# ArroyoSystems/arroyo

Measured on NVIDIA H100. Metric: rows/sec sliding-window SUM (1M keys), higher is better.
Workload: dtype int64

## Files before the change

arroyo_b200/csrc/abi.cu:

```cuda
#include <algorithm>
#include <chrono>
#include <memory>
#include <new>

#include "op.h"
#include "planner.h"

using namespace ab;

struct ArroyoB200Op {
  OpBase* impl;
  double host_process_ms = 0, host_watermark_ms = 0;
};

namespace {
struct WallTimer {
  double& acc;
  std::chrono::steady_clock::time_point t0 = std::chrono::steady_clock::now();
  explicit WallTimer(double& a) : acc(a) {}
  ~WallTimer() { acc += std::chrono::duration<double, std::milli>(std::chrono::steady_clock::now() - t0).count(); }
};
}

namespace {

template <class F>
int32_t guarded(ArroyoB200Op* op, F&& f) {
  if (!op || !op->impl) return ARROYO_B200_INVALID_ARGUMENT;
  try {
    f(op->impl);
    return ARROYO_B200_OK;
  } catch (const Error& e) {
    op->impl->last_error = e.what();
    return e.status;
  } catch (const std::bad_alloc&) {
    op->impl->last_error = "out of host memory";
    return ARROYO_B200_RUNTIME;
  } catch (const std::exception& e) {
    op->impl->last_error = e.what();
    return ARROYO_B200_RUNTIME;
  } catch (...) {
    op->impl->last_error = "unknown C++ exception";
    return ARROYO_B200_RUNTIME;
  }
}

template <class F>
int32_t emit_batches(ArroyoB200Op* op, ArroyoB200Batches* out, F&& f, double ArroyoB200Op::*timer = nullptr,
                     bool null_out_ok = false) {
  if (out) memset(out, 0, sizeof *out);
  if (!op) return ARROYO_B200_INVALID_ARGUMENT;
  double untimed = 0;
  WallTimer wt(timer ? op->*timer : untimed);
  return guarded(op, [&](OpBase* o) {
    AB_REQUIRE(out != nullptr || null_out_ok, ARROYO_B200_INVALID_ARGUMENT, "null out");
    std::unique_ptr<BatchesPriv, void (*)(BatchesPriv*)> priv(new BatchesPriv(), discard);
    f(o, priv.get());
    if (out) batches_finish(priv.release(), out);
  });
}

void begin_emission(OpBase* o, int64_t watermark_ns) {
  o->pending_out = new BatchesPriv();
  try {
    o->begin_watermark(watermark_ns);
  } catch (...) {
    o->poll_watermark(true);
    discard(o->pending_out);
    o->pending_out = nullptr;
    throw;
  }
}

void set_err(char* err, uint64_t len, const char* msg) {
  if (err && len) {
    snprintf(err, (size_t)len, "%s", msg);
  }
}

int64_t hand_out(OpBase* o, std::vector<ArroyoB200DeviceBatch>& v, ArroyoB200DeviceBatch* out, int64_t max_out) {
  const size_t n = (size_t)std::min<int64_t>((int64_t)v.size(), std::max<int64_t>(max_out, 0));
  for (size_t i = 0; i < n; ++i) out[i] = v[i];
  o->pending_dev.assign(v.begin() + n, v.end());
  return (int64_t)n;
}

}

extern "C" {

int32_t arroyo_b200_abi_version(void) { return 1; }

int32_t arroyo_b200_device_count(void) {
  int n = 0;
  if (cudaGetDeviceCount(&n) != cudaSuccess) {
    cudaGetLastError();
    return 0;
  }
  return n;
}

void* arroyo_b200_host_alloc(uint64_t bytes) {
  void* p = nullptr;
  if (cudaHostAlloc(&p, (size_t)bytes, cudaHostAllocDefault) != cudaSuccess) {
    cudaGetLastError();
    return nullptr;
  }
  return p;
}

void arroyo_b200_host_free(void* p) {
  if (p) cudaFreeHost(p);
}

int32_t arroyo_b200_op_create(const ArroyoB200OpConfig* config, ArroyoB200Op** out, char* err, uint64_t err_len) {
  if (!config || !out) {
    set_err(err, err_len, "null config or out pointer");
    return ARROYO_B200_INVALID_ARGUMENT;
  }
  *out = nullptr;
  try {
    OpBase* impl = nullptr;
    switch (config->kind) {
      case ARROYO_B200_TUMBLING_AGGREGATE:
      case ARROYO_B200_SLIDING_AGGREGATE:
        impl = make_window_agg_op(*config);
        break;
      case ARROYO_B200_SESSION_AGGREGATE:
        impl = make_session_op(*config);
        break;
      case ARROYO_B200_INSTANT_JOIN:
        impl = make_instant_join_op(*config);
        break;
      case ARROYO_B200_UPDATING_AGGREGATE:
        impl = make_updating_agg_op(*config);
        break;
      case ARROYO_B200_TTL_JOIN:
        impl = make_ttl_join_op(*config);
        break;
      case ARROYO_B200_INSTANT_AGGREGATE:
        impl = make_instant_agg_op(*config);
        break;
      case ARROYO_B200_WINDOW_FUNCTION:
        impl = make_window_fn_op(*config);
        break;
      default:
        set_err(err, err_len, "unknown operator kind");
        return ARROYO_B200_INVALID_ARGUMENT;
    }
    auto* h = new ArroyoB200Op();
    h->impl = impl;
    *out = h;
    return ARROYO_B200_OK;
  } catch (const Error& e) {
    set_err(err, err_len, e.what());
    return e.status;
  } catch (const std::exception& e) {
    set_err(err, err_len, e.what());
    return ARROYO_B200_RUNTIME;
  } catch (...) {
    set_err(err, err_len, "unknown C++ exception");
    return ARROYO_B200_RUNTIME;
  }
}

void arroyo_b200_op_destroy(ArroyoB200Op* op) {
  if (!op) return;
  try {
    if (op->impl && op->impl->pending_out) {
      op->impl->poll_watermark(true);
      discard(op->impl->pending_out);
      op->impl->pending_out = nullptr;
    }
    delete op->impl;
  } catch (...) {
  }
  delete op;
}

const char* arroyo_b200_op_last_error(const ArroyoB200Op* op) {
  if (!op || !op->impl) return "invalid handle";
  return op->impl->last_error.c_str();
}

const char* arroyo_b200_op_name(const ArroyoB200Op* op) {
  if (!op || !op->impl) return "";
  return op->impl->name.c_str();
}

int32_t arroyo_b200_op_on_start(ArroyoB200Op* op, struct ArrowArray* state, struct ArrowSchema* schemas, int64_t n,
                                int64_t watermark_ns, int64_t table_min_time_ns) {
  return guarded(op, [&](OpBase* o) { o->on_start(state, schemas, n, watermark_ns, table_min_time_ns); });
}

int32_t arroyo_b200_op_process_batch(ArroyoB200Op* op, uint32_t input_index, uint32_t in_partitions,
                                     struct ArrowArray* batch, const struct ArrowSchema* schema) {
  if (!op) return ARROYO_B200_INVALID_ARGUMENT;
  WallTimer wt(op->host_process_ms);
  return guarded(op, [&](OpBase* o) { o->process_batch(input_index, in_partitions, batch, schema); });
}

int32_t arroyo_b200_op_process_batch_emit(ArroyoB200Op* op, uint32_t input_index, uint32_t in_partitions,
                                          struct ArrowArray* batch, const struct ArrowSchema* schema, ArroyoB200Batches* out) {
  return emit_batches(
      op, out, [&](OpBase* o, BatchesPriv* b) { o->process_batch_emit(input_index, in_partitions, batch, schema, b); },
      &ArroyoB200Op::host_process_ms);
}

int32_t arroyo_b200_op_process_device_batch(ArroyoB200Op* op, uint32_t input_index, uint32_t in_partitions,
                                            const uint64_t* cols, int32_t n_cols, int64_t n_rows) {
  return guarded(op, [&](OpBase* o) {
    AB_REQUIRE(cols != nullptr && n_cols > 0, ARROYO_B200_INVALID_ARGUMENT, "null column list");
    o->process_device_batch(input_index, in_partitions, cols, n_cols, n_rows);
  });
}

int32_t arroyo_b200_op_process_device_batches(ArroyoB200Op* op, uint32_t input_index, uint32_t in_partitions,
                                              const uint64_t* cols, int32_t n_cols, const int64_t* n_rows,
                                              int64_t n_batches) {
  if (!op) return ARROYO_B200_INVALID_ARGUMENT;
  WallTimer wt(op->host_process_ms);
  return guarded(op, [&](OpBase* o) {
    AB_REQUIRE(cols != nullptr && n_rows != nullptr && n_cols > 0 && n_batches >= 0, ARROYO_B200_INVALID_ARGUMENT,
               "null batch list");
    for (int64_t b = 0; b < n_batches; ++b)
      o->process_device_batch(input_index, in_partitions, cols + b * n_cols, n_cols, n_rows[b]);
  });
}

int32_t arroyo_b200_op_handle_watermark(ArroyoB200Op* op, int64_t watermark_ns, ArroyoB200Batches* out) {
  return emit_batches(
      op, out, [&](OpBase* o, BatchesPriv* b) { o->handle_watermark(watermark_ns, b, nullptr); },
      &ArroyoB200Op::host_watermark_ms);
}

int32_t arroyo_b200_op_handle_tick(ArroyoB200Op* op, ArroyoB200Batches* out) {
  return emit_batches(op, out, [&](OpBase* o, BatchesPriv* b) { o->handle_tick(b); });
}

int32_t arroyo_b200_op_handle_watermark_begin(ArroyoB200Op* op, int64_t watermark_ns) {
  if (!op) return ARROYO_B200_INVALID_ARGUMENT;
  WallTimer wt(op->host_watermark_ms);
  return guarded(op, [&](OpBase* o) {
    AB_REQUIRE(o->pending_out == nullptr, ARROYO_B200_INVALID_ARGUMENT,
               "the previous emission has not been collected (handle_watermark_poll)");
    begin_emission(o, watermark_ns);
  });
}

int32_t arroyo_b200_op_handle_watermark_poll(ArroyoB200Op* op, int32_t block, ArroyoB200Batches* out, int32_t* ready) {
  if (out) memset(out, 0, sizeof *out);
  if (ready) *ready = 0;
  if (!op) return ARROYO_B200_INVALID_ARGUMENT;
  WallTimer wt(op->host_watermark_ms);
  return guarded(op, [&](OpBase* o) {
    AB_REQUIRE(out != nullptr && ready != nullptr, ARROYO_B200_INVALID_ARGUMENT, "null out");
    if (!o->pending_out) {
      *ready = 1;
      return;
    }
    if (!o->poll_watermark(block != 0)) return;
    batches_finish(o->pending_out, out);
    o->pending_out = nullptr;
    *ready = 1;
  });
}

int32_t arroyo_b200_op_run_batches(ArroyoB200Op* op, struct ArrowArray* batches, const struct ArrowSchema* schema,
                                    int64_t n_batches, const int64_t* watermarks, int32_t async_emit,
                                    ArroyoB200Batches* out, int64_t* n_consumed) {
  if (out) memset(out, 0, sizeof *out);
  if (n_consumed) *n_consumed = 0;
  if (!op) return ARROYO_B200_INVALID_ARGUMENT;
  auto* acc = new BatchesPriv();
  int32_t st = guarded(op, [&](OpBase* o) {
    AB_REQUIRE(out != nullptr && n_consumed != nullptr && (n_batches == 0 || (batches != nullptr && schema != nullptr)),
               ARROYO_B200_INVALID_ARGUMENT, "null argument");
    auto collect = [&](bool block) {
      if (!o->pending_out || !o->poll_watermark(block)) return;
      for (auto& a : o->pending_out->arrays) acc->arrays.push_back(a);
      for (auto& s : o->pending_out->schemas) acc->schemas.push_back(s);
      delete o->pending_out;
      o->pending_out = nullptr;
    };
    for (int64_t i = 0; i < n_batches; ++i) {
      {
        WallTimer wt(op->host_process_ms);
        o->process_batch(0, 1, &batches[i], schema);
      }
      ++*n_consumed;
      const int64_t wm = watermarks ? watermarks[i] : INT64_MIN;
      WallTimer wt(op->host_watermark_ms);
      if (wm == INT64_MIN) {
        if (async_emit && (i & 7) == 0) collect(false);
        continue;
      }
      if (async_emit) {
        collect(true);
        begin_emission(o, wm);
      } else {
        o->handle_watermark(wm, acc, nullptr);
      }
    }
    if (async_emit) collect(false);
  });
  if (out) batches_finish(acc, out);
  else discard(acc);
  return st;
}

int32_t arroyo_b200_op_handle_watermark_device(ArroyoB200Op* op, int64_t watermark_ns, ArroyoB200DeviceBatch* out,
                                               int64_t max_out, int64_t* n_out) {
  if (n_out) *n_out = 0;
  if (!op) return ARROYO_B200_INVALID_ARGUMENT;
  WallTimer wt(op->host_watermark_ms);
  return guarded(op, [&](OpBase* o) {
    AB_REQUIRE(n_out != nullptr && (out != nullptr || max_out <= 0), ARROYO_B200_INVALID_ARGUMENT, "null out");
    AB_REQUIRE(o->pending_dev.empty(), ARROYO_B200_INVALID_ARGUMENT,
               "windows of the previous emission are still queued (handle_watermark_device_poll)");
    std::vector<ArroyoB200DeviceBatch> v;
    o->handle_watermark(watermark_ns, nullptr, &v);
    *n_out = hand_out(o, v, out, max_out);
  });
}

int32_t arroyo_b200_op_handle_watermark_device_begin(ArroyoB200Op* op, int64_t watermark_ns) {
  if (!op) return ARROYO_B200_INVALID_ARGUMENT;
  WallTimer wt(op->host_watermark_ms);
  return guarded(op, [&](OpBase* o) {
    AB_REQUIRE(o->pending_dev.empty(), ARROYO_B200_INVALID_ARGUMENT,
               "windows of the previous emission are still queued (handle_watermark_device_poll)");
    o->begin_watermark_device(watermark_ns);
  });
}

int32_t arroyo_b200_op_handle_watermark_device_poll(ArroyoB200Op* op, ArroyoB200DeviceBatch* out, int64_t max_out,
                                                    int64_t* n_out) {
  if (n_out) *n_out = 0;
  if (!op) return ARROYO_B200_INVALID_ARGUMENT;
  WallTimer wt(op->host_watermark_ms);
  return guarded(op, [&](OpBase* o) {
    AB_REQUIRE(n_out != nullptr && (out != nullptr || max_out <= 0), ARROYO_B200_INVALID_ARGUMENT, "null out");
    std::vector<ArroyoB200DeviceBatch> v;
    o->poll_watermark_device(&v);
    *n_out = hand_out(o, v, out, max_out);
  });
}

int32_t arroyo_b200_op_handle_checkpoint(ArroyoB200Op* op, int64_t watermark_ns, ArroyoB200Batches* state_out) {
  return emit_batches(op, state_out, [&](OpBase* o, BatchesPriv* b) { o->handle_checkpoint(watermark_ns, b); });
}

int32_t arroyo_b200_op_checkpoint_state(ArroyoB200Op* op, ArroyoB200Batches* state_out) {
  return emit_batches(op, state_out, [&](OpBase* o, BatchesPriv* b) { o->checkpoint_state(b); });
}

int32_t arroyo_b200_op_restore_side(ArroyoB200Op* op, uint32_t side, struct ArrowArray* batches,
                                    struct ArrowSchema* schemas, int64_t n) {
  return guarded(op, [&](OpBase* o) { o->restore_side(side, batches, schemas, n); });
}

int32_t arroyo_b200_op_set_clock(ArroyoB200Op* op, int64_t now_ns) {
  return guarded(op, [&](OpBase* o) { o->set_clock(now_ns); });
}

int32_t arroyo_b200_op_on_close(ArroyoB200Op* op, int32_t end_of_data, ArroyoB200Batches* out) {
  return emit_batches(op, out, [&](OpBase* o, BatchesPriv* b) { o->on_close(end_of_data, b); }, nullptr, true);
}

int32_t arroyo_b200_op_flush(ArroyoB200Op* op) {
  return guarded(op, [&](OpBase* o) { o->flush(); });
}

int32_t arroyo_b200_op_submit(ArroyoB200Op* op) {
  return guarded(op, [&](OpBase* o) { o->submit(); });
}

void arroyo_b200_release_batches(ArroyoB200Batches* batches) { batches_release(batches); }

int32_t arroyo_b200_op_stats(ArroyoB200Op* op, ArroyoB200Stats* out) {
  return guarded(op, [&](OpBase* o) {
    AB_REQUIRE(out != nullptr, ARROYO_B200_INVALID_ARGUMENT, "null out");
    o->stats(out);
    out->host_process_ms = op->host_process_ms;
    out->host_watermark_ms = op->host_watermark_ms;
  });
}

uint64_t arroyo_b200_hash_key(int64_t key) { return mix64((uint64_t)key); }

uint32_t arroyo_b200_server_for_hash(uint64_t h, uint32_t n) {
  if (n == 0) return 0;
  uint64_t range = UINT64_MAX / (uint64_t)n;
  return (uint32_t)((h / range) % (uint64_t)n);
}

int64_t arroyo_b200_bin_start(int64_t ts_ns, int64_t width_ns) {
  if (width_ns < 2 || ts_ns < 0) return width_ns <= 0 ? ts_ns : ts_ns - ts_ns % width_ns;
  FastDivU64 d = FastDivU64::make((uint64_t)width_ns);
  return (int64_t)(d.div_host((uint64_t)ts_ns) * (uint64_t)width_ns);
}

static int64_t write_steps(const std::vector<PlanStep>& steps, int64_t* out, int64_t cap) {
  if ((int64_t)steps.size() * 4 > cap) return -1;
  for (size_t i = 0; i < steps.size(); ++i) {
    out[4 * i + 0] = steps[i].kind;
    out[4 * i + 1] = steps[i].a;
    out[4 * i + 2] = steps[i].b;
    out[4 * i + 3] = steps[i].c;
  }
  return (int64_t)steps.size();
}

int64_t arroyo_b200_plan_sliding(int64_t width_ns, int64_t slide_ns, const int64_t* events, int64_t n_events,
                                 int64_t* out, int64_t out_cap) {
  if (slide_ns <= 0 || width_ns <= 0 || width_ns % slide_ns) return -2;
  SlidingPlanner pl(width_ns, slide_ns);
  std::vector<PlanStep> steps;
  bool has_wm = false;
  int64_t wm = 0;
  for (int64_t i = 0; i < n_events; ++i) {
    int64_t kind = events[2 * i], v = events[2 * i + 1];
    if (kind == 0) {
      if (has_wm && v < bin_start(wm, slide_ns)) continue;
      pl.touch(v);
    } else if (kind == 1) {
      has_wm = true;
      wm = v;
      pl.watermark(v, steps);
    } else if (kind == 2) {
      pl.checkpoint(has_wm, wm, steps);
    }
  }
  return write_steps(steps, out, out_cap);
}

int64_t arroyo_b200_plan_tumbling(int64_t width_ns, const int64_t* events, int64_t n_events, int64_t* out,
                                  int64_t out_cap) {
  if (width_ns <= 0) return -2;
  TumblingPlanner pl(width_ns);
  std::vector<PlanStep> steps;
  bool has_wm = false;
  int64_t wm = 0;
  for (int64_t i = 0; i < n_events; ++i) {
    int64_t kind = events[2 * i], v = events[2 * i + 1];
    if (kind == 0) {
      if (has_wm && v < bin_start(wm, width_ns)) continue;
      pl.touch(v);
    } else if (kind == 1) {
      has_wm = true;
      wm = v;
      pl.watermark(v, steps);
    } else if (kind == 2) {
      pl.checkpoint(steps);
    }
  }
  return write_steps(steps, out, out_cap);
}

}
```

arroyo_b200/csrc/op.h:

```cpp
#pragma once

#include <string>
#include <vector>

#include "arrow_io.h"
#include "common.cuh"

namespace ab {

class OpBase {
 public:
  ArroyoB200OpConfig cfg{};
  std::string last_error;
  std::string name;

  virtual ~OpBase() {
    if (own_stream_) cudaStreamDestroy(stream_);
  }
  virtual void on_start(ArrowArray* state, ArrowSchema* schemas, int64_t n, int64_t watermark, int64_t table_min) = 0;
  virtual void process_batch(uint32_t index, uint32_t in_partitions, ArrowArray* batch, const ArrowSchema* schema) = 0;
  virtual void process_batch_emit(uint32_t index, uint32_t in_partitions, ArrowArray* batch, const ArrowSchema* schema,
                                  BatchesPriv* ) {
    process_batch(index, in_partitions, batch, schema);
  }
  virtual void process_device_batch(uint32_t index, uint32_t in_partitions, const uint64_t* cols, int32_t n_cols,
                                    int64_t n_rows) = 0;
  virtual void handle_watermark(int64_t watermark, BatchesPriv* out_host, std::vector<ArroyoB200DeviceBatch>* out_dev) = 0;
  virtual void handle_checkpoint(int64_t watermark, BatchesPriv* out) = 0;
  virtual void on_close(int end_of_data, BatchesPriv* out) = 0;
  virtual void handle_tick(BatchesPriv* ) {}
  virtual void checkpoint_state(BatchesPriv* ) {}
  virtual void restore_side(uint32_t , ArrowArray* , ArrowSchema* , int64_t ) {
    throw Error(ARROYO_B200_UNSUPPORTED, name + ": restore_side is only for the join with expiration");
  }
  virtual void set_clock(int64_t ) {
    throw Error(ARROYO_B200_UNSUPPORTED, name + ": set_clock is only for the updating aggregate");
  }
  virtual void flush() = 0;
  virtual void submit() {}
  BatchesPriv* pending_out = nullptr;
  virtual void begin_watermark(int64_t watermark) { handle_watermark(watermark, pending_out, nullptr); }
  virtual bool poll_watermark(bool ) { return true; }
  std::vector<ArroyoB200DeviceBatch> pending_dev;
  virtual void begin_watermark_device(int64_t watermark) {
    pending_dev.clear();
    handle_watermark(watermark, nullptr, &pending_dev);
  }
  virtual void poll_watermark_device(std::vector<ArroyoB200DeviceBatch>* out) {
    out->swap(pending_dev);
    pending_dev.clear();
  }
  virtual void stats(ArroyoB200Stats* out) = 0;

 protected:
  int device_ = 0;
  cudaStream_t stream_ = nullptr;
  bool own_stream_ = false;
  int num_sms_ = 132;

  void open_device(const ArroyoB200OpConfig& c) {
    int count = 0;
    if (cudaGetDeviceCount(&count) != cudaSuccess || count <= 0)
      throw Error(ARROYO_B200_FATAL, "no CUDA device available: libarroyo_b200 has no CPU fallback");
    AB_REQUIRE(c.device >= 0 && c.device < count, ARROYO_B200_INVALID_ARGUMENT, "bad device ordinal");
    device_ = c.device;
    set_device();
    cudaDeviceProp prop{};
    AB_CUDA(cudaGetDeviceProperties(&prop, device_));
    num_sms_ = prop.multiProcessorCount;
    if (c.stream) {
      stream_ = (cudaStream_t)c.stream;
    } else {
      AB_CUDA(cudaStreamCreateWithFlags(&stream_, cudaStreamNonBlocking));
      own_stream_ = true;
    }
  }
  void set_device() const { AB_CUDA(cudaSetDevice(device_)); }
  void drain_stream() const {
    cudaSetDevice(device_);
    cudaStreamSynchronize(stream_);
  }
};

OpBase* make_window_agg_op(const ArroyoB200OpConfig& cfg);
OpBase* make_instant_join_op(const ArroyoB200OpConfig& cfg);
OpBase* make_session_op(const ArroyoB200OpConfig& cfg);
OpBase* make_updating_agg_op(const ArroyoB200OpConfig& cfg);
OpBase* make_ttl_join_op(const ArroyoB200OpConfig& cfg);
OpBase* make_instant_agg_op(const ArroyoB200OpConfig& cfg);
OpBase* make_window_fn_op(const ArroyoB200OpConfig& cfg);

}
```

arroyo_b200/csrc/window_agg.cu:

```cuda
#include <algorithm>
#include <climits>
#include <deque>
#include <map>
#include <memory>
#include <set>

#include "agg_plan.h"
#include "bdict.cuh"
#include "op.h"
#include "planner.h"

namespace ab {
namespace {

constexpr int MAX_SEGS = 512;
constexpr int MAX_RING = 4096;
constexpr int RING_INLINE = 64;
constexpr int MAX_MERGE = 4096;
constexpr long long FREE_BIN = LLONG_MIN;

constexpr int THREADS = 256;
constexpr int PAIRS = 2;
constexpr int TILE = THREADS * PAIRS * 2;

struct Counters {
  unsigned long long late_rows;
  unsigned long long deferred;
  unsigned long long lost;
  unsigned long long neg_ts;
  unsigned long long max_q;
  unsigned long long big_vals;
  unsigned int n_keys;
  unsigned int dict_full;
  unsigned long long part_overflow;
};

struct Segment {
  const long long* key;
  const long long* ts;
  const long long* val[MAX_VALS];
  long long n;
  long long tile_start;
  int vec_ok;
  int pad;
};

struct IngestParams {
  const Segment* segs;
  int n_segs;
  int keyed;
  long long n_tiles;
  BDict dict;
  FastDivU64 slide_div;
  long long slide;
  long long late_bin;
  unsigned long long late_q;
  unsigned int guard_vals;
  int combine;
  int rows_slot;
  int pad2;
  uint32_t ring_mask;
  int n_acc;
  const long long* pane_bins;
  unsigned long long* const* pane_ptrs;
  unsigned long long id_cap;
  int ring_inline;
  int pad1;
  long long ring_bins[RING_INLINE];
  unsigned long long* ring_ptrs[RING_INLINE];
  int acc_kind[MAX_ACC];
  int acc_val[MAX_ACC];
  Counters* counters;
  unsigned long long* slot_rows;
  long long* d_key;
  long long* d_ts;
  long long* d_val[MAX_VALS];
  unsigned long long defer_cap;
};

struct InitParams {
  unsigned long long* pane;
  unsigned long long id_cap;
  unsigned long long n;
  int n_acc;
  int acc_kind[MAX_ACC];
};

__global__ void pane_init_kernel(const __grid_constant__ InitParams p) {
  uint64_t i = (uint64_t)blockIdx.x * blockDim.x + threadIdx.x;
  uint64_t stride = (uint64_t)gridDim.x * blockDim.x;
  for (; i < p.n; i += stride) {
    for (int a = 0; a < p.n_acc; ++a) p.pane[a * p.id_cap + i] = acc_identity(p.acc_kind[a]);
  }
}

__device__ __forceinline__ const long long* ldg_ptr(const long long* const* pp) {
  return reinterpret_cast<const long long*>(__ldg(reinterpret_cast<const unsigned long long*>(pp)));
}

__device__ __forceinline__ void red_add_u64(unsigned long long* a, unsigned long long v) {
  asm volatile("red.global.add.u64 [%0], %1;" ::"l"(__cvta_generic_to_global(a)), "l"(v) : "memory");
}
__device__ __forceinline__ void red_add_f64(unsigned long long* a, double v) {
  asm volatile("red.global.add.f64 [%0], %1;" ::"l"(__cvta_generic_to_global(a)), "d"(v) : "memory");
}
__device__ __forceinline__ void red_min_s64(unsigned long long* a, long long v) {
  asm volatile("red.global.min.s64 [%0], %1;" ::"l"(__cvta_generic_to_global(a)), "l"(v) : "memory");
}
__device__ __forceinline__ void red_max_s64(unsigned long long* a, long long v) {
  asm volatile("red.global.max.s64 [%0], %1;" ::"l"(__cvta_generic_to_global(a)), "l"(v) : "memory");
}

__device__ __forceinline__ long long ring_bin(const IngestParams& p, uint32_t slot) {
  return p.ring_inline ? p.ring_bins[slot] : __ldg(p.pane_bins + slot);
}
__device__ __forceinline__ unsigned long long* ring_ptr(const IngestParams& p, uint32_t slot) {
  return p.ring_inline ? p.ring_ptrs[slot]
                       : reinterpret_cast<unsigned long long*>(__ldg(reinterpret_cast<const unsigned long long*>(p.pane_ptrs + slot)));
}

struct Vals {
  long long v0, v1, v2, v3;
};
template <int NV>
__device__ __forceinline__ Vals pack_vals(const long long (&v)[NV > 0 ? NV : 1]) {
  Vals o{0, 0, 0, 0};
  if (NV > 0) o.v0 = v[0];
  if (NV > 1) o.v1 = v[NV > 1 ? 1 : 0];
  if (NV > 2) o.v2 = v[NV > 2 ? 2 : 0];
  if (NV > 3) o.v3 = v[NV > 3 ? 3 : 0];
  return o;
}

__device__ __noinline__ void defer_row(const IngestParams& p, long long key, long long ts, long long v0, long long v1,
                                       long long v2, long long v3) {
  unsigned long long idx = atomicAdd(&p.counters->deferred, 1ull);
  if (idx < p.defer_cap) {
    p.d_key[idx] = key;
    p.d_ts[idx] = ts;
    if (p.d_val[0]) p.d_val[0][idx] = v0;
    if (p.d_val[1]) p.d_val[1][idx] = v1;
    if (p.d_val[2]) p.d_val[2][idx] = v2;
    if (p.d_val[3]) p.d_val[3][idx] = v3;
  } else {
    atomicAdd(&p.counters->lost, 1ull);
  }
}

constexpr int GENERIC_SIG = -1;
constexpr int sig_of(int k1, int k2 = 0, int k3 = 0) { return k1 | (k2 << 3) | (k3 << 6); }

__device__ __forceinline__ void red_kind(int kind, unsigned long long* dst, long long v) {
  switch (kind) {
    case ACC_SUM_I64: red_add_u64(dst, (unsigned long long)v); break;
    case ACC_SUM_F64: red_add_f64(dst, (double)v); break;
    case ACC_MIN_I64: red_min_s64(dst, v); break;
    case ACC_MAX_I64: red_max_s64(dst, v); break;
    default: break;
  }
}

__device__ __forceinline__ unsigned long long rows_of(const IngestParams& p, const Vals& v) {
  const int x = p.rows_slot;
  if (x < 0) return 1ull;
  return (unsigned long long)(x == 0 ? v.v0 : x == 1 ? v.v1 : x == 2 ? v.v2 : v.v3);
}

template <int NV, int SIG>
__device__ __forceinline__ void accumulate(const IngestParams& p, const Vals& v, unsigned long long* pane, uint32_t id) {
  red_add_u64(pane + id, rows_of(p, v));
  if (SIG == GENERIC_SIG) {
#pragma unroll
    for (int a = 1; a < MAX_ACC; ++a) {
      if (a < p.n_acc) {
        const int x = p.acc_val[a];
        const long long val = x == 0 ? v.v0 : x == 1 ? v.v1 : x == 2 ? v.v2 : v.v3;
        red_kind(p.acc_kind[a], pane + (unsigned long long)a * p.id_cap + id, val);
      }
    }
  } else {
    constexpr int k1 = SIG & 7, k2 = (SIG >> 3) & 7, k3 = (SIG >> 6) & 7;
    if (k1) red_kind(k1, pane + p.id_cap + id, v.v0);
    if (k2) red_kind(k2, pane + 2 * p.id_cap + id, v.v0);
    if (k3) red_kind(k3, pane + 3 * p.id_cap + id, v.v0);
  }
}

__device__ __forceinline__ bool big_one(long long v) { return (unsigned long long)(v + (1ll << 31)) >= (1ull << 32); }
__device__ __forceinline__ bool big_value(unsigned int mask, const Vals& v) {
  return ((mask & 1u) && big_one(v.v0)) || ((mask & 2u) && big_one(v.v1)) || ((mask & 4u) && big_one(v.v2)) ||
         ((mask & 8u) && big_one(v.v3));
}

template <int NV, int SIG>
__device__ __noinline__ void slow_row(const IngestParams& p, long long key, long long ts, uint64_t q, long long v0,
                                      long long v1, long long v2, long long v3) {
  const uint32_t slot = (uint32_t)q & p.ring_mask;
  uint32_t id = 0;
  bool ok = ring_bin(p, slot) == (long long)(q * (uint64_t)p.slide);
  if (ok && p.keyed) {
    const uint64_t h = bd_hash(key);
    const ulonglong2* hp = reinterpret_cast<const ulonglong2*>(bd_home(p.dict, key, h));
    const ulonglong2 raw = __ldcg(hp), raw1 = __ldcg(hp + 1);
    id = bd_resolve(p.dict, key, h, raw.x, (uint32_t)raw.y, raw1.x, (uint32_t)raw1.y);
    ok = id < ID_OVERFLOW;
    if (!ok) atomicAdd(&p.counters->dict_full, 1u);
  }
  const Vals v{v0, v1, v2, v3};
  if (ok && NV > 0 && p.guard_vals && big_value(p.guard_vals, v)) {
    atomicAdd(&p.counters->big_vals, 1ull);
    ok = false;
  }
  if (!ok) {
    defer_row(p, key, ts, v0, v1, v2, v3);
    return;
  }
  unsigned long long* pane = ring_ptr(p, slot);
  atomicAdd(p.slot_rows + slot, 1ull);
  accumulate<NV, SIG>(p, v, pane, id);
}

struct PaneCache {
  uint64_t q = ~0ull;
  unsigned long long* ptr = nullptr;
  uint32_t cnt = 0;
};

__device__ __forceinline__ void flush_counts(const IngestParams& p, PaneCache& pc, int lane) {
  const unsigned int peers = __match_any_sync(0xffffffffu, pc.q);
  const unsigned int total = __reduce_add_sync(peers, pc.cnt);
  if (total && (__ffs(peers) - 1) == lane)
    atomicAdd(p.slot_rows + ((uint32_t)pc.q & p.ring_mask), (unsigned long long)total);
  pc.cnt = 0;
}

template <int NV, int SIG>
__device__ __forceinline__ uint32_t hot_resolve(const IngestParams& p, const PaneCache& pc, uint64_t& maxq, bool keyed,
                                                long long key, long long ts, uint64_t q, const Vals& v, uint64_t h,
                                                unsigned long long k0, uint32_t id0, unsigned long long k1, uint32_t id1) {
  uint32_t id = ID_OVERFLOW;
  if (q == pc.q && pc.ptr != nullptr) id = keyed ? bd_resolve(p.dict, key, h, k0, id0, k1, id1) : 0u;
  if (NV > 0 && p.guard_vals && big_value(p.guard_vals, v)) {
    atomicAdd(&p.counters->big_vals, 1ull);
    defer_row(p, key, ts, v.v0, v.v1, v.v2, v.v3);
    return ID_OVERFLOW;
  }
  if (id >= ID_OVERFLOW) {
    maxq = max(maxq, q);
    slow_row<NV, SIG>(p, key, ts, q, v.v0, v.v1, v.v2, v.v3);
  }
  return id;
}

__device__ __forceinline__ long long shfl_ll(unsigned mask, long long v, int src) {
  return (long long)__shfl_sync(mask, (unsigned long long)v, src);
}

__device__ __forceinline__ long long group_reduce(int kind, unsigned peers, long long v) {
  long long r = v;
  bool first = true;
  for (unsigned m = peers; m; m &= m - 1) {
    const long long x = shfl_ll(peers, v, __ffs(m) - 1);
    if (first) {
      r = x;
      first = false;
      continue;
    }
    switch (kind) {
      case ACC_SUM_I64: r = (long long)((unsigned long long)r + (unsigned long long)x); break;
      case ACC_SUM_F64: r = __double_as_longlong(__longlong_as_double(r) + __longlong_as_double(x)); break;
      case ACC_MIN_I64: r = min(r, x); break;
      case ACC_MAX_I64: r = max(r, x); break;
      default: break;
    }
  }
  return r;
}

__device__ __forceinline__ void red_kind_combined(int kind, unsigned long long* dst, long long v) {
  if (kind == ACC_SUM_F64) red_add_f64(dst, __longlong_as_double(v));
  else red_kind(kind, dst, v);
}

template <int NV, int SIG>
__device__ __forceinline__ void combine_accumulate(const IngestParams& p, const PaneCache& pc, bool fast, uint32_t id,
                                                   const Vals& v, int lane) {
  const unsigned long long gkey = fast ? ((unsigned long long)id | (pc.q << 32)) : (0xFFFFFFFF00000000ull | (unsigned)lane);
  const unsigned long long nb = __shfl_xor_sync(0xffffffffu, gkey, 1);
  if (!__any_sync(0xffffffffu, fast && nb == gkey)) {
    if (fast) accumulate<NV, SIG>(p, v, pc.ptr, id);
    return;
  }
  const unsigned peers = __match_any_sync(0xffffffffu, gkey);
  const bool leader = (__ffs(peers) - 1) == lane;
  unsigned long long* pane = pc.ptr;
  if (p.rows_slot < 0) {
    if (fast && leader) red_add_u64(pane + id, (unsigned long long)__popc(peers));
  } else {
    const long long r = group_reduce(ACC_SUM_I64, peers, (long long)rows_of(p, v));
    if (fast && leader) red_add_u64(pane + id, (unsigned long long)r);
  }
  if (SIG == GENERIC_SIG) {
#pragma unroll
    for (int a = 1; a < MAX_ACC; ++a) {
      if (a < p.n_acc) {
        const int x = p.acc_val[a];
        long long val = x == 0 ? v.v0 : x == 1 ? v.v1 : x == 2 ? v.v2 : v.v3;
        const int kind = p.acc_kind[a];
        if (kind == ACC_SUM_F64) val = __double_as_longlong((double)val);
        const long long r = group_reduce(kind, peers, val);
        if (fast && leader) red_kind_combined(kind, pane + (unsigned long long)a * p.id_cap + id, r);
      }
    }
  } else {
    constexpr int k1 = SIG & 7, k2 = (SIG >> 3) & 7, k3 = (SIG >> 6) & 7;
    if (k1) {
      const long long r = group_reduce(k1, peers, k1 == ACC_SUM_F64 ? __double_as_longlong((double)v.v0) : v.v0);
      if (fast && leader) red_kind_combined(k1, pane + p.id_cap + id, r);
    }
    if (k2) {
      const long long r = group_reduce(k2, peers, k2 == ACC_SUM_F64 ? __double_as_longlong((double)v.v0) : v.v0);
      if (fast && leader) red_kind_combined(k2, pane + 2 * p.id_cap + id, r);
    }
    if (k3) {
      const long long r = group_reduce(k3, peers, k3 == ACC_SUM_F64 ? __double_as_longlong((double)v.v0) : v.v0);
      if (fast && leader) red_kind_combined(k3, pane + 3 * p.id_cap + id, r);
    }
  }
}

#ifndef AB_INGEST_PREFETCH
#define AB_INGEST_PREFETCH 1
#endif
#ifndef AB_INGEST_MIN_BLOCKS
#define AB_INGEST_MIN_BLOCKS 4
#endif
template <int NV, int SIG>
__global__ void __launch_bounds__(THREADS, AB_INGEST_MIN_BLOCKS) ingest_kernel(const __grid_constant__ IngestParams p) {
  __shared__ unsigned long long s_late, s_maxq;
  __shared__ unsigned int s_done;
  const int tid = threadIdx.x;
  const int lane = tid & 31;
  if (tid == 0) {
    s_late = 0;
    s_maxq = 0;
    s_done = 0;
  }
  __syncthreads();

  PaneCache pc;
  uint32_t late = 0;
  uint64_t maxq = 0;
  const FastDivU64 sd = p.slide_div;
  const bool keyed = p.keyed != 0;

  for (long long tile = blockIdx.x; tile < p.n_tiles; tile += gridDim.x) {
    int lo = 0, hi = p.n_segs - 1;
    while (lo < hi) {
      int mid = (lo + hi + 1) >> 1;
      if (__ldg(&p.segs[mid].tile_start) <= tile) lo = mid; else hi = mid - 1;
    }
    const Segment* sg = p.segs + lo;
    const long long base = (tile - __ldg(&sg->tile_start)) * TILE;
    const long long nrem = __ldg(&sg->n) - base;
    const int cnt = nrem < TILE ? (int)nrem : TILE;

    long long nkey = 0, nts = 0;
    long long nv[NV > 0 ? NV : 1] = {0};
    if (tid < cnt) {
      if (keyed) nkey = __ldcs(ldg_ptr(&sg->key) + base + tid);
      nts = __ldcs(ldg_ptr(&sg->ts) + base + tid);
#pragma unroll
      for (int x = 0; x < NV; ++x) nv[x] = __ldcs(ldg_ptr(&sg->val[x]) + base + tid);
    }
#pragma unroll 1
    for (int i = tid; i < TILE; i += THREADS) {
      const bool valid = i < cnt;
      const long long key = nkey, ts = nts;
      long long v[NV > 0 ? NV : 1];
#pragma unroll
      for (int x = 0; x < (NV > 0 ? NV : 1); ++x) v[x] = nv[x];
      ulonglong2 raw = {0, 0}, raw1 = {0, 0};
      const uint64_t h = keyed ? bd_hash(key) : 0ull;
      if (valid && keyed) {
        const ulonglong2* hp = reinterpret_cast<const ulonglong2*>(bd_home(p.dict, key, h));
        raw = __ldcg(hp);
        raw1 = __ldcg(hp + 1);
      }
#if AB_INGEST_PREFETCH
      if (i + THREADS < cnt) {
        if (keyed) nkey = __ldcs(ldg_ptr(&sg->key) + base + i + THREADS);
        nts = __ldcs(ldg_ptr(&sg->ts) + base + i + THREADS);
#pragma unroll
        for (int x = 0; x < NV; ++x) nv[x] = __ldcs(ldg_ptr(&sg->val[x]) + base + i + THREADS);
      }
#endif
      const uint64_t q = sd.div((uint64_t)ts);
      if (valid && ts < 0) atomicAdd(&p.counters->neg_ts, 1ull);
      const bool live = valid && ts >= 0 && q >= p.late_q;
      late += (valid && !live) ? 1u : 0u;
      if (__any_sync(0xffffffffu, live && q != pc.q)) {
        flush_counts(p, pc, lane);
        if (live) {
          const uint32_t slot = (uint32_t)q & p.ring_mask;
          const bool resident = ring_bin(p, slot) == (long long)(q * (uint64_t)p.slide);
          pc.q = q;
          pc.ptr = resident ? ring_ptr(p, slot) : nullptr;
          maxq = max(maxq, q);
        }
      }
      const Vals pv = pack_vals<NV>(v);
      uint32_t id = ID_OVERFLOW;
      if (live) id = hot_resolve<NV, SIG>(p, pc, maxq, keyed, key, ts, q, pv, h, raw.x, (uint32_t)raw.y, raw1.x, (uint32_t)raw1.y);
      const bool fast = id < ID_OVERFLOW;
      if (fast) ++pc.cnt;
      if (p.combine) combine_accumulate<NV, SIG>(p, pc, fast, id, pv, lane);
      else if (fast) accumulate<NV, SIG>(p, pv, pc.ptr, id);
#if !AB_INGEST_PREFETCH
      if (i + THREADS < cnt) {
        if (keyed) nkey = __ldcs(ldg_ptr(&sg->key) + base + i + THREADS);
        nts = __ldcs(ldg_ptr(&sg->ts) + base + i + THREADS);
#pragma unroll
        for (int x = 0; x < NV; ++x) nv[x] = __ldcs(ldg_ptr(&sg->val[x]) + base + i + THREADS);
      }
#endif
    }
  }

  __syncwarp();
  flush_counts(p, pc, lane);
  unsigned long long wl = late;
#pragma unroll
  for (int o = 16; o > 0; o >>= 1) {
    wl += __shfl_xor_sync(0xffffffffu, wl, o);
    maxq = max(maxq, __shfl_xor_sync(0xffffffffu, maxq, o));
  }
  if (lane == 0) {
    if (wl) atomicAdd(&s_late, wl);
    if (maxq) atomicMax(&s_maxq, (unsigned long long)maxq);
    __threadfence_block();
    if (atomicAdd(&s_done, 1u) == THREADS / 32 - 1) {
      __threadfence_block();
      const unsigned long long bl = *(volatile unsigned long long*)&s_late;
      const unsigned long long mq = *(volatile unsigned long long*)&s_maxq;
      if (bl) atomicAdd(&p.counters->late_rows, bl);
      if (mq) atomicMax(&p.counters->max_q, mq);
    }
  }
}

#include "ingest_two_pass.cuh"

struct PartialParams {
  const uint32_t* ids;
  const unsigned long long* state[MAX_ACC];
  long long n;
  int n_acc;
  int acc_kind[MAX_ACC];
  unsigned long long* pane;
  unsigned long long id_cap;
};

__global__ void ingest_partial_kernel(const __grid_constant__ PartialParams p) {
  long long i = (long long)blockIdx.x * blockDim.x + threadIdx.x;
  long long stride = (long long)gridDim.x * blockDim.x;
  for (; i < p.n; i += stride) {
    const uint32_t id = p.ids[i];
    for (int a = 0; a < p.n_acc; ++a)
      acc_atomic_merge(p.acc_kind[a], p.pane + (unsigned long long)a * p.id_cap + id, p.state[a] ? p.state[a][i] : 1ull);
  }
}

constexpr int EMIT_INLINE = 16;
struct EmitParams {
  const unsigned long long* const* panes;
  const unsigned long long* inline_panes[EMIT_INLINE];
  int panes_inline;
  int n_panes;
  int n_acc;
  unsigned long long id_cap;
  uint32_t n_ids;
  int keyed;
  int acc_kind[MAX_ACC];
  unsigned long long* out_raw[MAX_ACC];
  unsigned long long* out_avg[MAX_ACC];
  const long long* id_keys;
  long long* out_key;
  long long* out_wstart;
  long long* out_wend;
  long long* out_ts;
  long long wstart, wend, ts;
  unsigned int* out_count;
  unsigned int out_base;
  unsigned long long* running;
  int n_add;
  int partial;
  unsigned long long* out_state[MAX_ACC];
};

constexpr int EMIT_THREADS = 256;

__device__ __forceinline__ unsigned long long unmerge_acc(int kind, unsigned long long a, unsigned long long v) {
  if (kind == ACC_SUM_F64)
    return (unsigned long long)__double_as_longlong(__longlong_as_double((long long)a) - __longlong_as_double((long long)v));
  return a - v;
}

template <int NACC>
__device__ __forceinline__ void emit_row(const EmitParams& p, unsigned int o, const unsigned long long (&acc)[NACC],
                                         long long key) {
  const unsigned long long rows = acc[0];
  if (p.keyed) p.out_key[o] = key;
  if (p.partial) {
#pragma unroll
    for (int a = 0; a < NACC; ++a)
      p.out_state[a][o] = acc[a];
    p.out_ts[o] = p.ts;
    return;
  }
#pragma unroll
  for (int a = 0; a < NACC; ++a) {
    if (p.out_raw[a]) p.out_raw[a][o] = acc[a];
    if (p.out_avg[a]) {
      const double num = p.acc_kind[a] == ACC_SUM_F64 ? __longlong_as_double((long long)acc[a]) : (double)(long long)acc[a];
      p.out_avg[a][o] = (unsigned long long)__double_as_longlong(num / (double)rows);
    }
  }
  if (p.out_wstart) {
    p.out_wstart[o] = p.wstart;
    p.out_wend[o] = p.wend;
  }
  p.out_ts[o] = p.ts;
}

template <bool RUNNING, int NACC>
__global__ void __launch_bounds__(EMIT_THREADS) emit_kernel(const __grid_constant__ EmitParams p) {
  __shared__ unsigned int s_warp[EMIT_THREADS / 32];
  __shared__ unsigned int s_base;
  const int tid = threadIdx.x;
  const int lane = tid & 31, w = tid >> 5;
  const uint32_t n_pairs = (p.n_ids + 1) / 2;
  const uint32_t n_iter = (n_pairs + EMIT_THREADS - 1) / EMIT_THREADS;
  for (uint32_t it = blockIdx.x; it < n_iter; it += gridDim.x) {
    const uint32_t pair = it * EMIT_THREADS + tid;
    const uint32_t id = pair * 2;
    unsigned long long acc0[NACC], acc1[NACC];
#pragma unroll
    for (int a = 0; a < NACC; ++a) {
      acc0[a] = 0;
      acc1[a] = 0;
    }
    const bool in0 = id < p.n_ids, in1 = id + 1 < p.n_ids;
    if (in0) {
      if (RUNNING) {
#pragma unroll
        for (int a = 0; a < NACC; ++a)
          {
            const ulonglong2 v = *reinterpret_cast<const ulonglong2*>(p.running + (unsigned long long)a * p.id_cap + id);
            acc0[a] = v.x;
            acc1[a] = v.y;
          }
        for (int k = 0; k < p.n_panes; ++k) {
          const unsigned long long* pane = p.panes_inline ? p.inline_panes[k] : p.panes[k];
          const bool add = k < p.n_add;
#pragma unroll
          for (int a = 0; a < NACC; ++a)
            {
              const ulonglong2 v = __ldcs(reinterpret_cast<const ulonglong2*>(pane + (unsigned long long)a * p.id_cap + id));
              const int kind = p.acc_kind[a];
              acc0[a] = add ? acc_merge(kind, acc0[a], v.x) : unmerge_acc(kind, acc0[a], v.x);
              acc1[a] = add ? acc_merge(kind, acc1[a], v.y) : unmerge_acc(kind, acc1[a], v.y);
            }
        }
        const bool z0 = acc0[0] == 0, z1 = acc1[0] == 0;
#pragma unroll
        for (int a = 0; a < NACC; ++a)
          {
            if (z0) acc0[a] = 0;
            if (z1) acc1[a] = 0;
            *reinterpret_cast<ulonglong2*>(p.running + (unsigned long long)a * p.id_cap + id) = make_ulonglong2(acc0[a], acc1[a]);
          }
      } else {
#pragma unroll
        for (int a = 0; a < NACC; ++a)
          {
            const unsigned long long ident = acc_identity(p.acc_kind[a]);
            acc0[a] = ident;
            acc1[a] = ident;
          }
        for (int k = 0; k < p.n_panes; ++k) {
          const unsigned long long* pane = p.panes_inline ? p.inline_panes[k] : p.panes[k];
#pragma unroll
          for (int a = 0; a < NACC; ++a)
            {
              const ulonglong2 v = __ldcs(reinterpret_cast<const ulonglong2*>(pane + (unsigned long long)a * p.id_cap + id));
              const int kind = p.acc_kind[a];
              acc0[a] = acc_merge(kind, acc0[a], v.x);
              acc1[a] = acc_merge(kind, acc1[a], v.y);
            }
        }
      }
    }
    const bool v0 = in0 && acc0[0] != 0, v1 = in1 && acc1[0] != 0;
    const unsigned int b0 = __ballot_sync(0xffffffffu, v0), b1 = __ballot_sync(0xffffffffu, v1);
    if (lane == 0) s_warp[w] = __popc(b0) + __popc(b1);
    __syncthreads();
    if (tid == 0) {
      unsigned int total = 0;
      for (int i = 0; i < EMIT_THREADS / 32; ++i) {
        unsigned int c = s_warp[i];
        s_warp[i] = total;
        total += c;
      }
      s_base = total ? atomicAdd(p.out_count, total) - p.out_base : 0u;
    }
    __syncthreads();
    const unsigned int lt = (1u << lane) - 1u;
    const unsigned int o0 = s_base + s_warp[w] + __popc(b0 & lt) + __popc(b1 & lt);
    ulonglong2 keys = make_ulonglong2(0, 0);
    if ((v0 || v1) && p.keyed) keys = *reinterpret_cast<const ulonglong2*>(p.id_keys + id);
    if (v0) emit_row<NACC>(p, o0, acc0, (long long)keys.x);
    if (v1) emit_row<NACC>(p, o0 + (v0 ? 1u : 0u), acc1, (long long)keys.y);
    __syncthreads();
  }
}

struct Pane {
  int64_t bin = 0;
  unsigned long long* dev = nullptr;
  unsigned long long* frozen = nullptr;
  int slot = -1;
  bool in_tier = false;
  uint64_t rows = 0;
  bool exported = false;
  bool delta_exported = false;
};

struct LaunchRec {
  cudaEvent_t done = nullptr;
  cudaEvent_t t0 = nullptr, t1 = nullptr;
  Counters* h_counters = nullptr;
  unsigned long long* h_slot_rows = nullptr;
  uint64_t rows = 0;
  bool in_flight = false;
  int chunk = -1;
};

constexpr size_t RELEASE_GROUP = 16;
struct PendingRelease {
  cudaEvent_t ev;
  std::vector<ArrowArray> arrs;
};

class WindowAggOp final : public OpBase {
 public:
  explicit WindowAggOp(const ArroyoB200OpConfig& c);
  ~WindowAggOp() override;

  void on_start(ArrowArray* state, ArrowSchema* schemas, int64_t n, int64_t watermark, int64_t table_min) override;
  void process_batch(uint32_t, uint32_t, ArrowArray* batch, const ArrowSchema* schema) override;
  void process_device_batch(uint32_t, uint32_t, const uint64_t* cols, int32_t n_cols, int64_t n_rows) override;
  void handle_watermark(int64_t wm, BatchesPriv* out_host, std::vector<ArroyoB200DeviceBatch>* out_dev) override;
  void handle_checkpoint(int64_t wm, BatchesPriv* out) override;
  void on_close(int, BatchesPriv*) override { flush(); }
  void flush() override;
  void submit() override;
  void begin_watermark(int64_t wm) override;
  bool poll_watermark(bool block) override;
  void begin_watermark_device(int64_t wm) override;
  void poll_watermark_device(std::vector<ArroyoB200DeviceBatch>* out) override;
  void stats(ArroyoB200Stats* out) override;

 private:
  bool sliding_;
  int64_t width_, slide_;
  AggPlan plan_;
  bool invertible_ = true;
  bool avg_exact_ = true;
  unsigned int guard_vals_ = 0;
  int rows_slot_ = -1;
  bool running_mode_ = false;
  bool profile_;
  std::string key_format_ = "l";

  BucketDict dict_;
  DevBuf book_;
  static constexpr size_t BOOK_SLOT_OFF = (sizeof(Counters) + 15) / 16 * 16;
  Counters* d_counters() const { return reinterpret_cast<Counters*>(book_.p); }
  unsigned long long* d_slot_rows() const { return reinterpret_cast<unsigned long long*>((char*)book_.p + BOOK_SLOT_OFF); }
  std::vector<unsigned long long> slot_rows_seen_;
  uint32_t total_keys_host_ = 0;
  uint32_t dict_full_seen_ = 0;
  DevBuf part_, part_cursor_;
  uint32_t part_cap_ = 0;
  int part_flip_ = 0;
  bool two_pass_attr_set_ = false;
  bool two_pass_enabled_ = true;
  uint64_t part_overflow_seen_ = 0;
  mutable int two_pass_pause_ = 0;
  bool two_pass_eligible(uint64_t rows) const;
  void launch_two_pass(IngestParams& p, uint64_t rows, long long tiles_direct);
  cudaStream_t out_stream_ = nullptr;
  cudaEvent_t emit_done_ = nullptr, out_done_ = nullptr;
  bool async_out_ = false, out_inflight_ = false;
  void wait_outputs();
  static constexpr size_t COPY_GROUP = 48;
  std::vector<void*> copy_dst_, copy_src_;
  std::vector<size_t> copy_size_;
  bool batch_copy_ok_ = true;
  void queue_copy(void* dst, const void* src, size_t bytes);
  void flush_copies();
  std::vector<ArrowArray> open_release_;
  std::vector<cudaEvent_t> ev_pool_;
  void seal_release();

  uint32_t ring_ = 16;
  std::vector<long long> h_pane_bins_;
  std::vector<unsigned long long*> h_pane_ptrs_;
  DevBuf d_pane_bins_, d_pane_ptrs_;
  bool ring_dirty_ = true;
  std::map<int64_t, Pane> panes_;
  std::vector<std::pair<unsigned long long*, uint64_t>> free_panes_;
  std::vector<DevBuf> pane_storage_;
  int64_t late_bin_ = LLONG_MIN;
  int64_t max_bin_seen_ = LLONG_MIN;

  unsigned long long* running_ = nullptr;
  std::set<int64_t> in_running_;
  std::map<int64_t, Pane> zombies_;

  std::unique_ptr<TumblingPlanner> tumbling_;
  std::unique_ptr<SlidingPlanner> sliding_planner_;

  static constexpr int NCHUNK = 3;
  static constexpr int NLAUNCH = 3;
  int64_t chunk_rows_ = 1 << 24;
  int64_t launch_rows_ = (1 << 24) + (1 << 22);
  DevBuf chunk_[NCHUNK];
  cudaEvent_t chunk_free_[NCHUNK] = {nullptr, nullptr, nullptr};
  cudaStream_t copy_stream_ = nullptr;
  cudaEvent_t copied_ = nullptr;
  int cur_chunk_ = 0;
  int64_t cur_rows_ = 0;
  std::vector<Segment> segs_;
  int64_t pending_rows_ = 0;
  bool pending_uses_chunk_ = false;
  PinnedBuf h_segs_[NLAUNCH];
  DevBuf d_segs_[NLAUNCH];
  LaunchRec launches_[NLAUNCH];
  PinnedBuf h_book_[NLAUNCH];
  int next_launch_ = 0;
  std::deque<int> in_flight_;
  std::deque<PendingRelease> releases_;
  std::vector<ArrowArray> zero_copy_inputs_;

  uint64_t defer_cap_ = 0;
  DevBuf defer_[2][2 + MAX_VALS];
  int defer_cur_ = 0;
  Counters last_counters_{};
  bool have_counters_ = false;
  bool draining_ = false;
  bool need_promote_ = false;

  struct OutSet {
    DevBuf key, wstart, wend, ts;
    DevBuf agg[ARROYO_B200_MAX_AGGS];
    DevBuf state[MAX_ACC];
    uint64_t cap = 0;
  };
  std::vector<std::unique_ptr<OutSet>> out_sets_;
  DevBuf d_emit_panes_, d_out_count_;
  unsigned int out_count_base_ = 0;
  PinnedBuf h_out_count_;
  static constexpr int COUNT_SLOTS = 64;
  PinnedBuf h_out_counts_;
  bool defer_counts_ = false;
  int count_slots_used_ = 0;
  int last_count_slot_ = -1;
  bool counts_pending_ = false;
  cudaEvent_t counts_done_ = nullptr;
  void resolve_deferred();

  ArroyoB200Stats st_{};
  std::vector<std::pair<cudaEvent_t, cudaEvent_t>> emit_events_;
  size_t emit_events_used_ = 0;

  void preallocate();
  template <class Fill>
  void rebuild_blocks(Fill fill);
  void grow_ids();
  void promote_avg();
  unsigned long long* acquire_block();
  void release_block(unsigned long long* blk);
  void init_block(unsigned long long* blk, uint64_t n_ids);
  void ensure_pane(int64_t bin);
  void drop_pane(int64_t bin);
  void upload_ring();
  void add_segment(const long long* key, const long long* ts, const long long* const* vals, int64_t n);
  void launch_pending();
  void launch_segments(const std::vector<Segment>& segs, int chunk);
  void absorb(int li);
  void sync_all();
  void drain_deferred();
  void poll_releases(bool wait);
  void rotate_chunk();
  void touch(int64_t bin);
  OutSet* out_set(size_t i, uint64_t cap);
  int64_t run_emit(const std::vector<const unsigned long long*>& blocks, int n_add, bool use_running, bool partial,
                   int64_t wstart, int64_t wend, int64_t ts, OutSet* os);
  void emit_window(int64_t a, int64_t b, size_t out_index, BatchesPriv* out_host,
                   std::vector<ArroyoB200DeviceBatch>* out_dev);
  void export_window(OutSet* os, int64_t n, BatchesPriv* out_host);
  void export_partial(OutSet* os, int64_t n, BatchesPriv* out);
  void collect_emit_times();
  void lookahead();
};

WindowAggOp::WindowAggOp(const ArroyoB200OpConfig& c) {
  cfg = c;
  sliding_ = c.kind == ARROYO_B200_SLIDING_AGGREGATE;
  name = sliding_ ? "sliding_window" : "tumbling_window";
  AB_REQUIRE(c.width_ns > 0, ARROYO_B200_UNSUPPORTED, "width_micros == 0 (instant window) is not supported");
  width_ = c.width_ns;
  slide_ = sliding_ ? c.slide_ns : c.width_ns;
  AB_REQUIRE(slide_ >= 2, ARROYO_B200_INVALID_ARGUMENT, "slide must be >= 2 ns");
  if (sliding_)
    AB_REQUIRE(width_ % slide_ == 0, ARROYO_B200_INVALID_ARGUMENT,
               "hop width must be a multiple of the slide (arroyo-planner/src/lib.rs:640-655)");
  plan_ = AggPlan(c, ACC_SUM_I64);
  std::set<int> avg_slots;
  for (int g = 0; g < plan_.n_aggs; ++g)
    if (plan_.agg_kind[g] == ARROYO_B200_AGG_AVG_I64) avg_slots.insert(plan_.acc_val[plan_.agg_acc[g]]);
  avg_exact_ = !(c.flags & ARROYO_B200_FLAG_AVG_F64) && plan_.n_acc + avg_slots.size() <= (size_t)MAX_ACC;
  if (!avg_exact_) plan_ = AggPlan(c, ACC_SUM_F64);
  if (avg_exact_)
    for (int v : avg_slots) guard_vals_ |= 1u << v;
  for (int g = 0; g < plan_.n_aggs; ++g)
    if (plan_.agg_kind[g] == ARROYO_B200_AGG_MIN_I64 || plan_.agg_kind[g] == ARROYO_B200_AGG_MAX_I64) invertible_ = false;
  if (c.partial_count_col_plus1 > 0) {
    const int col = c.partial_count_col_plus1 - 1;
    AB_REQUIRE(col < c.n_cols, ARROYO_B200_INVALID_ARGUMENT, "partial count column out of range");
    rows_slot_ = plan_.value_slot(col);
    guard_vals_ = 0;
  }
  profile_ = (c.flags & ARROYO_B200_FLAG_PROFILE) != 0;
  bool has_f64 = false;
  for (int a = 1; a < plan_.n_acc; ++a) has_f64 = has_f64 || plan_.acc_kind[a] == ACC_SUM_F64;
  running_mode_ = sliding_ && invertible_ && !has_f64 && !(c.flags & ARROYO_B200_FLAG_REMERGE_ONLY) && width_ > slide_;

  open_device(c);

  if (sliding_) sliding_planner_.reset(new SlidingPlanner(width_, slide_));
  else tumbling_.reset(new TumblingPlanner(width_));

  book_.alloc(BOOK_SLOT_OFF + MAX_RING * sizeof(unsigned long long));
  AB_CUDA(cudaMemsetAsync(book_.p, 0, book_.bytes, stream_));
  slot_rows_seen_.assign(MAX_RING, 0);
  Counters init{};
  init.max_q = 0;
  init.n_keys = 0;
  AB_CUDA(cudaMemcpyAsync(book_.p, &init, sizeof init, cudaMemcpyHostToDevice, stream_));
  last_counters_ = init;

  uint64_t want = c.expected_keys ? c.expected_keys : (1ull << 16);
  dict_.init(stream_, num_sms_, plan_.keyed, (unsigned int*)((char*)book_.p + offsetof(Counters, n_keys)),
             &st_.kernel_launches);
  dict_.alloc(plan_.keyed ? bd_buckets_for(want) : 1);
  {
    const char* e = getenv("ARROYO_B200_NO_TWO_PASS");
    two_pass_enabled_ = !(e && atoi(e) != 0) && !(c.flags & ARROYO_B200_FLAG_NO_TWO_PASS);
  }

  h_pane_bins_.assign(MAX_RING, FREE_BIN);
  h_pane_ptrs_.assign(MAX_RING, nullptr);
  d_pane_bins_.alloc(MAX_RING * sizeof(long long));
  d_pane_ptrs_.alloc(MAX_RING * sizeof(void*));
  if (sliding_) {
    uint64_t need = (uint64_t)(width_ / slide_) + 8;
    while (ring_ < need && ring_ < MAX_RING) ring_ <<= 1;
  }

  const int n_used = 2 + plan_.n_vals;
  for (int i = 0; i < NCHUNK; ++i) {
    AB_CUDA(cudaEventCreateWithFlags(&chunk_free_[i], cudaEventDisableTiming));
    if (i == 0) {
      AB_CUDA(cudaStreamCreateWithFlags(&copy_stream_, cudaStreamNonBlocking));
      AB_CUDA(cudaEventCreateWithFlags(&copied_, cudaEventDisableTiming));
    }
  }
  (void)n_used;
  for (int i = 0; i < NLAUNCH; ++i) {
    h_segs_[i].alloc(MAX_SEGS * sizeof(Segment));
    d_segs_[i].alloc(MAX_SEGS * sizeof(Segment));
    h_book_[i].alloc(BOOK_SLOT_OFF + MAX_RING * sizeof(unsigned long long));
    launches_[i].h_counters = h_book_[i].as<Counters>();
    launches_[i].h_slot_rows = reinterpret_cast<unsigned long long*>((char*)h_book_[i].p + BOOK_SLOT_OFF);
    AB_CUDA(cudaEventCreateWithFlags(&launches_[i].done, cudaEventDisableTiming));
    if (profile_) {
      AB_CUDA(cudaEventCreate(&launches_[i].t0));
      AB_CUDA(cudaEventCreate(&launches_[i].t1));
    }
  }
  if (c.reserved >= 16 && c.reserved <= 26) chunk_rows_ = 1ll << c.reserved;
  launch_rows_ = chunk_rows_ + chunk_rows_ / 4;
  defer_cap_ = (uint64_t)launch_rows_ * 2;
  d_emit_panes_.alloc(MAX_MERGE * sizeof(void*));
  d_out_count_.alloc(sizeof(unsigned int));
  AB_CUDA(cudaMemsetAsync(d_out_count_.p, 0, sizeof(unsigned int), stream_));
  h_out_count_.alloc(sizeof(unsigned int));
  h_out_counts_.alloc(COUNT_SLOTS * sizeof(unsigned int));
  preallocate();
  AB_CUDA(cudaStreamSynchronize(stream_));
}

void WindowAggOp::preallocate() {
  const size_t block_bytes = (size_t)plan_.n_acc * dict_.id_cap() * sizeof(unsigned long long);
  size_t want = (sliding_ ? (size_t)(width_ / slide_) : 1) + 4 + (running_mode_ ? 1 : 0);
  const size_t budget = (size_t)4 << 30;
  want = std::min<size_t>(std::min<size_t>(want, 64), std::max<size_t>(budget / std::max<size_t>(block_bytes, 1), 4));
  for (size_t i = 0; i < want; ++i) {
    pane_storage_.emplace_back(block_bytes);
    auto* blk = pane_storage_.back().as<unsigned long long>();
    init_block(blk, dict_.id_cap());
    free_panes_.emplace_back(blk, 0);
  }
  for (int c = 0; c < 2 + plan_.n_vals; ++c) defer_[0][c].alloc(defer_cap_ * 8);
  out_set(0, dict_.id_cap());
  out_set(1, dict_.id_cap());
}

WindowAggOp::~WindowAggOp() {
  cudaSetDevice(device_);
  if (counts_done_) cudaEventDestroy(counts_done_);
  if (copy_stream_) cudaStreamSynchronize(copy_stream_);
  if (out_stream_) cudaStreamSynchronize(out_stream_);
  cudaStreamSynchronize(stream_);
  for (auto& r : releases_) {
    for (auto& a : r.arrs)
      if (a.release) a.release(&a);
    cudaEventDestroy(r.ev);
  }
  for (auto& a : zero_copy_inputs_)
    if (a.release) a.release(&a);
  for (auto& a : open_release_)
    if (a.release) a.release(&a);
  for (auto e : ev_pool_) cudaEventDestroy(e);
  for (int i = 0; i < NCHUNK; ++i)
    if (chunk_free_[i]) cudaEventDestroy(chunk_free_[i]);
  if (copy_stream_) {
    cudaStreamSynchronize(copy_stream_);
    cudaStreamDestroy(copy_stream_);
    cudaEventDestroy(copied_);
  }
  for (int i = 0; i < NLAUNCH; ++i) {
    if (launches_[i].done) cudaEventDestroy(launches_[i].done);
    if (launches_[i].t0) cudaEventDestroy(launches_[i].t0);
    if (launches_[i].t1) cudaEventDestroy(launches_[i].t1);
  }
  for (auto& e : emit_events_) {
    cudaEventDestroy(e.first);
    cudaEventDestroy(e.second);
  }
  if (out_stream_) {
    cudaStreamSynchronize(out_stream_);
    cudaStreamDestroy(out_stream_);
    cudaEventDestroy(emit_done_);
    cudaEventDestroy(out_done_);
  }
}

void WindowAggOp::init_block(unsigned long long* blk, uint64_t n_ids) {
  if (n_ids == 0) return;
  InitParams ip{};
  ip.pane = blk;
  ip.id_cap = dict_.id_cap();
  ip.n = n_ids;
  ip.n_acc = plan_.n_acc;
  for (int a = 0; a < plan_.n_acc; ++a) ip.acc_kind[a] = plan_.acc_kind[a];
  int blocks = (int)std::min<uint64_t>((n_ids + 255) / 256, (uint64_t)num_sms_ * 8);
  pane_init_kernel<<<blocks, 256, 0, stream_>>>(ip);
  AB_CUDA(cudaGetLastError());
  ++st_.kernel_launches;
}

unsigned long long* WindowAggOp::acquire_block() {
  if (!free_panes_.empty()) {
    auto pr = free_panes_.back();
    free_panes_.pop_back();
    init_block(pr.first, pr.second);
    return pr.first;
  }
  pane_storage_.emplace_back((size_t)plan_.n_acc * dict_.id_cap() * sizeof(unsigned long long));
  auto* blk = pane_storage_.back().as<unsigned long long>();
  init_block(blk, dict_.id_cap());
  return blk;
}

void WindowAggOp::release_block(unsigned long long* blk) {
  if (!blk) return;
  free_panes_.emplace_back(blk, std::min<uint64_t>(dict_.id_cap(), (uint64_t)dict_.n_ids() + 1));
}

__global__ void permute_block_kernel(const unsigned long long* __restrict__ old_blk, unsigned long long* __restrict__ new_blk,
                                     const uint32_t* __restrict__ map, uint32_t old_ids, uint64_t old_cap, uint64_t new_cap,
                                     int n_acc) {
  uint32_t i = blockIdx.x * blockDim.x + threadIdx.x;
  const uint32_t stride = gridDim.x * blockDim.x;
  for (; i < old_ids; i += stride) {
    const uint32_t m = map[i];
    if (m == ID_UNSET || m >= ID_OVERFLOW) continue;
    for (int a = 0; a < n_acc; ++a) new_blk[(uint64_t)a * new_cap + m] = old_blk[(uint64_t)a * old_cap + i];
  }
}

template <class Fill>
void WindowAggOp::rebuild_blocks(Fill fill) {
  std::vector<DevBuf> new_storage;
  auto rebuild = [&](unsigned long long*& blk) {
    if (!blk) return;
    new_storage.emplace_back((size_t)plan_.n_acc * dict_.id_cap() * sizeof(unsigned long long));
    auto* nb = new_storage.back().as<unsigned long long>();
    init_block(nb, dict_.id_cap());
    fill(blk, nb);
    blk = nb;
  };
  for (auto& kv : panes_) {
    rebuild(kv.second.dev);
    rebuild(kv.second.frozen);
    if (kv.second.slot >= 0) h_pane_ptrs_[kv.second.slot] = kv.second.dev;
  }
  for (auto& kv : zombies_) {
    rebuild(kv.second.dev);
    rebuild(kv.second.frozen);
  }
  rebuild(running_);
  AB_CUDA(cudaStreamSynchronize(stream_));
  free_panes_.clear();
  pane_storage_ = std::move(new_storage);
  ring_dirty_ = true;
}

void WindowAggOp::grow_ids() {
  const BdGrowth g = dict_.grow();
  const uint64_t new_cap = dict_.id_cap();
  const int grid = (int)std::min<uint64_t>((g.old_ids + 255) / 256, (uint64_t)num_sms_ * 8);
  rebuild_blocks([&](const unsigned long long* old_blk, unsigned long long* nb) {
    permute_block_kernel<<<std::max(grid, 1), 256, 0, stream_>>>(old_blk, nb, g.map.as<uint32_t>(), g.old_ids, g.old_cap,
                                                               new_cap, plan_.n_acc);
    AB_CUDA(cudaGetLastError());
    ++st_.kernel_launches;
  });
  Counters c{};
  AB_CUDA(cudaMemcpyAsync(&c, book_.p, sizeof c, cudaMemcpyDeviceToHost, stream_));
  AB_CUDA(cudaStreamSynchronize(stream_));
  total_keys_host_ = c.n_keys;
  part_cap_ = 0;
}

__global__ void i64_to_f64_kernel(const unsigned long long* __restrict__ src, unsigned long long* __restrict__ dst, uint64_t n) {
  uint64_t i = (uint64_t)blockIdx.x * blockDim.x + threadIdx.x;
  uint64_t stride = (uint64_t)gridDim.x * blockDim.x;
  for (; i < n; i += stride) dst[i] = (unsigned long long)__double_as_longlong((double)(long long)src[i]);
}

void WindowAggOp::promote_avg() {
  if (!avg_exact_) return;
  AB_REQUIRE(in_flight_.empty(), ARROYO_B200_RUNTIME, "promote with launches in flight");
  const int old_n_acc = plan_.n_acc;
  std::set<int> avg_srcs;
  for (int g = 0; g < plan_.n_aggs; ++g)
    if (plan_.agg_kind[g] == ARROYO_B200_AGG_AVG_I64) avg_srcs.insert(plan_.agg_acc[g]);
  AB_REQUIRE(old_n_acc + (int)avg_srcs.size() <= MAX_ACC, ARROYO_B200_RUNTIME, "too many accumulators after AVG promotion");
  std::vector<std::pair<int, int>> f64_from;
  for (int g = 0; g < plan_.n_aggs; ++g) {
    if (plan_.agg_kind[g] != ARROYO_B200_AGG_AVG_I64) continue;
    const int src = plan_.agg_acc[g];
    int found = -1;
    for (auto& pr : f64_from)
      if (pr.second == src) found = pr.first;
    if (found < 0) {
      found = plan_.n_acc;
      plan_.acc_kind[plan_.n_acc] = ACC_SUM_F64;
      plan_.acc_val[plan_.n_acc] = plan_.acc_val[src];
      ++plan_.n_acc;
      f64_from.emplace_back(found, src);
    }
    plan_.agg_acc[g] = found;
  }
  avg_exact_ = false;
  if (running_mode_) {
    running_mode_ = false;
    in_running_.clear();
    for (auto& z : zombies_) {
      release_block(z.second.dev);
      release_block(z.second.frozen);
    }
    zombies_.clear();
    release_block(running_);
    running_ = nullptr;
  }
  const uint64_t cap = dict_.id_cap();
  const uint32_t n_valid = (uint32_t)std::min<uint64_t>(dict_.n_ids(), cap);
  rebuild_blocks([&](const unsigned long long* old_blk, unsigned long long* nb) {
    for (int a = 0; a < old_n_acc; ++a)
      AB_CUDA(cudaMemcpyAsync(nb + (size_t)a * cap, old_blk + (size_t)a * cap, (size_t)n_valid * sizeof(unsigned long long),
                              cudaMemcpyDeviceToDevice, stream_));
    for (auto& pr : f64_from) {
      const int grid = (int)std::min<uint64_t>((n_valid + 255) / 256 + 1, (uint64_t)num_sms_ * 8);
      i64_to_f64_kernel<<<grid, 256, 0, stream_>>>(old_blk + (size_t)pr.second * cap, nb + (size_t)pr.first * cap, n_valid);
      AB_CUDA(cudaGetLastError());
      ++st_.kernel_launches;
    }
  });
}

void WindowAggOp::ensure_pane(int64_t bin) {
  auto it = panes_.find(bin);
  if (it != panes_.end() && it->second.slot >= 0) return;
  const uint64_t q = (uint64_t)bin / (uint64_t)slide_;
  uint32_t slot;
  while (true) {
    slot = (uint32_t)q & (ring_ - 1);
    if (h_pane_bins_[slot] == FREE_BIN) break;
    if (ring_ == MAX_RING) {
      auto old = panes_.find(h_pane_bins_[slot]);
      AB_REQUIRE(old != panes_.end(), ARROYO_B200_RUNTIME, "ring slot of an unknown pane");
      old->second.slot = -1;
      h_pane_bins_[slot] = FREE_BIN;
      h_pane_ptrs_[slot] = nullptr;
      ring_dirty_ = true;
      break;
    }
    ring_ *= 2;
    std::fill(h_pane_bins_.begin(), h_pane_bins_.end(), FREE_BIN);
    std::fill(h_pane_ptrs_.begin(), h_pane_ptrs_.end(), nullptr);
    for (auto& kv : panes_) {
      if (kv.second.slot < 0) continue;
      uint32_t s = (uint32_t)((uint64_t)kv.first / (uint64_t)slide_) & (ring_ - 1);
      kv.second.slot = (int)s;
      h_pane_bins_[s] = kv.first;
      h_pane_ptrs_[s] = kv.second.dev;
    }
    ring_dirty_ = true;
  }
  if (it == panes_.end()) {
    Pane p;
    p.bin = bin;
    p.dev = acquire_block();
    it = panes_.emplace(bin, p).first;
  }
  it->second.slot = (int)slot;
  h_pane_bins_[slot] = bin;
  h_pane_ptrs_[slot] = it->second.dev;
  ring_dirty_ = true;
}

void WindowAggOp::drop_pane(int64_t bin) {
  auto it = panes_.find(bin);
  if (it == panes_.end()) return;
  Pane& p = it->second;
  if (p.slot >= 0) {
    h_pane_bins_[p.slot] = FREE_BIN;
    h_pane_ptrs_[p.slot] = nullptr;
    ring_dirty_ = true;
  }
  release_block(p.dev);
  release_block(p.frozen);
  panes_.erase(it);
}

void WindowAggOp::upload_ring() {
  if (!ring_dirty_) return;
  AB_CUDA(cudaMemcpyAsync(d_pane_bins_.p, h_pane_bins_.data(), ring_ * sizeof(long long), cudaMemcpyHostToDevice, stream_));
  AB_CUDA(cudaMemcpyAsync(d_pane_ptrs_.p, h_pane_ptrs_.data(), ring_ * sizeof(void*), cudaMemcpyHostToDevice, stream_));
  ring_dirty_ = false;
}

void WindowAggOp::queue_copy(void* dst, const void* src, size_t bytes) {
  if (bytes == 0) return;
  copy_dst_.push_back(dst);
  copy_src_.push_back(const_cast<void*>(src));
  copy_size_.push_back(bytes);
  if (copy_dst_.size() >= COPY_GROUP) flush_copies();
}

void WindowAggOp::flush_copies() {
  const size_t n = copy_dst_.size();
  if (n == 0) return;
  bool done = false;
#if CUDART_VERSION >= 12080 && CUDART_VERSION < 13000
  if (batch_copy_ok_ && n > 1) {
    cudaMemcpyAttributes at{};
    at.srcAccessOrder = cudaMemcpySrcAccessOrderStream;
    at.flags = cudaMemcpyFlagPreferOverlapWithCompute;
    size_t idx = 0, fail = 0;
    cudaError_t e = cudaMemcpyBatchAsync(copy_dst_.data(), copy_src_.data(), copy_size_.data(), n, &at, &idx, 1, &fail,
                                         copy_stream_);
    if (e == cudaSuccess) {
      done = true;
    } else if (e == cudaErrorNotSupported || e == cudaErrorInvalidValue) {
      cudaGetLastError();
      batch_copy_ok_ = false;
    } else {
      AB_CUDA(e);
    }
  }
#endif
  if (!done)
    for (size_t i = 0; i < n; ++i)
      AB_CUDA(cudaMemcpyAsync(copy_dst_[i], copy_src_[i], copy_size_[i], cudaMemcpyHostToDevice, copy_stream_));
  copy_dst_.clear();
  copy_src_.clear();
  copy_size_.clear();
}

void WindowAggOp::seal_release() {
  flush_copies();
  if (open_release_.empty()) return;
  PendingRelease r;
  if (!ev_pool_.empty()) {
    r.ev = ev_pool_.back();
    ev_pool_.pop_back();
  } else {
    AB_CUDA(cudaEventCreateWithFlags(&r.ev, cudaEventDisableTiming));
  }
  AB_CUDA(cudaEventRecord(r.ev, copy_stream_));
  r.arrs.swap(open_release_);
  releases_.push_back(std::move(r));
}

void WindowAggOp::poll_releases(bool wait) {
  if (wait) seal_release();
  while (!releases_.empty()) {
    PendingRelease& r = releases_.front();
    if (wait) {
      AB_CUDA(cudaEventSynchronize(r.ev));
    } else {
      cudaError_t e = cudaEventQuery(r.ev);
      if (e == cudaErrorNotReady) break;
      AB_CUDA(e);
    }
    for (auto& a : r.arrs)
      if (a.release) a.release(&a);
    ev_pool_.push_back(r.ev);
    releases_.pop_front();
  }
}

void WindowAggOp::add_segment(const long long* key, const long long* ts, const long long* const* vals, int64_t n) {
  if (n <= 0) return;
  if (!segs_.empty()) {
    Segment& l = segs_.back();
    bool contig = l.ts + l.n == ts && (!plan_.keyed || l.key + l.n == key);
    for (int v = 0; v < plan_.n_vals; ++v) contig = contig && (l.val[v] + l.n == vals[v]);
    if (contig) {
      l.n += n;
      pending_rows_ += n;
      return;
    }
  }
  if ((int)segs_.size() == MAX_SEGS) launch_pending();
  Segment s{};
  s.key = key;
  s.ts = ts;
  for (int v = 0; v < plan_.n_vals; ++v) s.val[v] = vals[v];
  s.n = n;
  segs_.push_back(s);
  pending_rows_ += n;
}

void WindowAggOp::rotate_chunk() {
  cur_chunk_ = (cur_chunk_ + 1) % NCHUNK;
  cur_rows_ = 0;
  AB_CUDA(cudaStreamWaitEvent(copy_stream_, chunk_free_[cur_chunk_], 0));
}

void WindowAggOp::process_batch(uint32_t, uint32_t, ArrowArray* batch, const ArrowSchema* schema) {
  set_device();
  int64_t n = 0;
  std::vector<InColumn> cols = import_batch(batch, schema, &n);
  AB_REQUIRE((int)cols.size() == cfg.n_cols, ARROYO_B200_INVALID_ARGUMENT, "batch has the wrong number of columns");
  require_aggregate_input_types(cols, plan_.keyed ? plan_.key_col : -1, plan_.val_cols, plan_.n_vals);
  if (plan_.keyed) key_format_ = cols[plan_.key_col].format;
  poll_releases(false);
  st_.rows_in += (uint64_t)n;
  if (n > 0 && panes_.empty() && max_bin_seen_ == LLONG_MIN) {
    int64_t b0 = bin_start((int64_t)cols[plan_.ts_col].data[0], slide_);
    if (b0 >= late_bin_) {
      ensure_pane(b0);
      max_bin_seen_ = b0;
      lookahead();
    }
  }
  if (n > 0 && (cfg.flags & ARROYO_B200_FLAG_ZERO_COPY)) {
    bool pinned = true;
    const uint64_t* devp[ARROYO_B200_MAX_COLS] = {nullptr};
    auto probe = [&](int c) {
      cudaPointerAttributes at{};
      if (cudaPointerGetAttributes(&at, cols[c].data) != cudaSuccess) {
        cudaGetLastError();
        pinned = false;
        return;
      }
      if (at.type != cudaMemoryTypeHost || at.devicePointer == nullptr) pinned = false;
      else devp[c] = (const uint64_t*)at.devicePointer;
    };
    if (plan_.keyed) probe(plan_.key_col);
    probe(plan_.ts_col);
    for (int v = 0; v < plan_.n_vals; ++v) probe(plan_.val_cols[v]);
    if (pinned) {
      int64_t done = 0;
      while (done < n) {
        int64_t take = std::min<int64_t>(n - done, launch_rows_ - pending_rows_);
        const long long* vals[MAX_VALS];
        for (int v = 0; v < plan_.n_vals; ++v) vals[v] = (const long long*)devp[plan_.val_cols[v]] + done;
        add_segment(plan_.keyed ? (const long long*)devp[plan_.key_col] + done : nullptr, (const long long*)devp[plan_.ts_col] + done,
                    vals, take);
        done += take;
        if (done < n && pending_rows_ >= launch_rows_) launch_pending();
      }
      st_.h2d_bytes += (uint64_t)n * 8 * (uint64_t)((plan_.keyed ? 1 : 0) + 1 + plan_.n_vals);
      zero_copy_inputs_.push_back(*batch);
      batch->release = nullptr;
      if (pending_rows_ >= launch_rows_) launch_pending();
      return;
    }
  }
  const int n_used = 2 + plan_.n_vals;
  int64_t done = 0;
  while (done < n) {
    if (!chunk_[cur_chunk_].p) chunk_[cur_chunk_].alloc((size_t)n_used * chunk_rows_ * 8);
    int64_t room = chunk_rows_ - cur_rows_;
    if (room == 0) {
      launch_pending();
      rotate_chunk();
      continue;
    }
    int64_t take = std::min(room, n - done);
    long long* base = chunk_[cur_chunk_].as<long long>();
    long long* d_key = base + 0 * chunk_rows_ + cur_rows_;
    long long* d_ts = base + 1 * chunk_rows_ + cur_rows_;
    const long long* d_vals[MAX_VALS];
    if (plan_.keyed) queue_copy(d_key, cols[plan_.key_col].data + done, (size_t)take * 8);
    queue_copy(d_ts, cols[plan_.ts_col].data + done, (size_t)take * 8);
    for (int v = 0; v < plan_.n_vals; ++v) {
      long long* dv = base + (size_t)(2 + v) * chunk_rows_ + cur_rows_;
      queue_copy(dv, cols[plan_.val_cols[v]].data + done, (size_t)take * 8);
      d_vals[v] = dv;
    }
    st_.h2d_bytes += (uint64_t)take * 8 * (uint64_t)((plan_.keyed ? 1 : 0) + 1 + plan_.n_vals);
    add_segment(d_key, d_ts, d_vals, take);
    pending_uses_chunk_ = true;
    cur_rows_ += take;
    done += take;
  }
  open_release_.push_back(*batch);
  batch->release = nullptr;
  if (open_release_.size() >= RELEASE_GROUP) seal_release();
  if (cur_rows_ == chunk_rows_) {
    launch_pending();
    rotate_chunk();
  }
}

void WindowAggOp::process_device_batch(uint32_t, uint32_t, const uint64_t* cols, int32_t n_cols, int64_t n_rows) {
  set_device();
  const AggCols d = plan_.columns(cols, n_cols);
  if (n_rows <= 0) return;
  st_.rows_in += (uint64_t)n_rows;
  int64_t done = 0;
  while (done < n_rows) {
    int64_t take = std::min<int64_t>(n_rows - done, launch_rows_ - pending_rows_);
    const long long* vals[MAX_VALS];
    for (int v = 0; v < plan_.n_vals; ++v) vals[v] = d.val[v] + done;
    add_segment(d.key ? d.key + done : nullptr, d.ts + done, vals, take);
    done += take;
    if (pending_rows_ >= launch_rows_) launch_pending();
  }
}

bool WindowAggOp::two_pass_eligible(uint64_t rows) const {
  if (!two_pass_enabled_ || !plan_.keyed || rows_slot_ >= 0 || plan_.n_vals > 1 || plan_.n_acc > 2) return false;
  if (plan_.n_acc == 2 && plan_.acc_kind[1] != ACC_SUM_I64) return false;
  if (dict_.n_buckets() > (uint64_t)P1_NR) return false;
  if (max_bin_seen_ == LLONG_MIN) return false;
  if (two_pass_pause_ > 0) {
    --two_pass_pause_;
    return false;
  }
  static const uint64_t min_rows = [] {
    const char* e = getenv("ARROYO_B200_TWO_PASS_MIN_ROWS");
    return e ? strtoull(e, nullptr, 10) : (1ull << 19);
  }();
  return rows >= min_rows || (cfg.flags & ARROYO_B200_FLAG_TWO_PASS_ALWAYS);
}

void WindowAggOp::launch_two_pass(IngestParams& p, uint64_t rows, long long tiles) {
  const uint64_t n_buckets = dict_.n_buckets();
  TwoPassParams tp{};
  int nf = 0;
  for (int k = 0; k < 3 && nf < TP_NP; ++k) {
    const int64_t b = max_bin_seen_ + (int64_t)(k == 2 ? -1 : k) * slide_;
    auto it = panes_.find(b);
    if (b < late_bin_ || it == panes_.end() || it->second.slot < 0) continue;
    tp.fast_q[nf] = (unsigned long long)b / (unsigned long long)slide_;
    tp.fast_ptr[nf] = it->second.dev;
    tp.fast_slot[nf] = (uint32_t)it->second.slot;
    ++nf;
  }
  for (int f = nf; f < TP_NP; ++f) {
    tp.fast_q[f] = ~0ull;
    tp.fast_ptr[f] = nullptr;
    tp.fast_slot[f] = 0;
  }
  const uint32_t n_regions = (uint32_t)(TP_NP * n_buckets);
  const uint64_t mean = (uint64_t)launch_rows_ / n_buckets + 1;
  const uint32_t cap = (uint32_t)std::min<uint64_t>(((mean + mean / 4 + 2048 + 63) / 64) * 64, 1u << 30);
  if (part_cap_ != cap || !part_.p) {
    AB_CUDA(cudaStreamSynchronize(stream_));
    part_.alloc((size_t)n_regions * cap * sizeof(Rec));
    part_cursor_.alloc((size_t)2 * n_regions * sizeof(unsigned int));
    AB_CUDA(cudaMemsetAsync(part_cursor_.p, 0, (size_t)2 * n_regions * sizeof(unsigned int), stream_));
    part_cap_ = cap;
  }
  tp.part = part_.as<Rec>();
  tp.cursor = part_cursor_.as<unsigned int>() + (size_t)part_flip_ * n_regions;
  tp.cursor_next = part_cursor_.as<unsigned int>() + (size_t)(part_flip_ ^ 1) * n_regions;
  part_flip_ ^= 1;
  tp.cap = cap;
  const uint32_t want_blocks = (uint32_t)num_sms_ * 2;
  tp.slices = (uint32_t)std::max<uint64_t>(1, std::min<uint64_t>((want_blocks + n_buckets - 1) / n_buckets,
                                                                 std::max<uint64_t>(1, rows / n_buckets / 4096)));
  if (!two_pass_attr_set_) {
    AB_CUDA(cudaFuncSetAttribute(part_kernel<0, 0>, cudaFuncAttributeMaxDynamicSharedMemorySize, (int)P1_SMEM));
    AB_CUDA(cudaFuncSetAttribute(part_kernel<1, sig_of(ACC_SUM_I64)>, cudaFuncAttributeMaxDynamicSharedMemorySize, (int)P1_SMEM));
    AB_CUDA(cudaFuncSetAttribute(agg_kernel<0>, cudaFuncAttributeMaxDynamicSharedMemorySize, (int)P2_SMEM));
    AB_CUDA(cudaFuncSetAttribute(agg_kernel<1>, cudaFuncAttributeMaxDynamicSharedMemorySize, (int)P2_SMEM));
    two_pass_attr_set_ = true;
  }
  const int grid1 = (int)std::max<long long>(1, std::min<long long>(tiles, (long long)num_sms_ * P1_BLOCKS_PER_SM));
  const uint32_t max_blocks = (uint32_t)num_sms_ * P2_BLOCKS_PER_SM;
  tp.tail_first = (uint32_t)n_buckets;
  tp.tail_slices = 1;
  if (tp.slices == 1 && n_buckets > max_blocks && rows / n_buckets >= 2048) {
    const uint32_t rest = (uint32_t)(n_buckets % max_blocks);
    if (rest && max_blocks / rest >= 2) {
      tp.tail_first = (uint32_t)n_buckets - rest;
      tp.tail_slices = std::min<uint32_t>(max_blocks / rest, 4);
    }
  }
  const uint32_t n_work = tp.tail_first * tp.slices + ((uint32_t)n_buckets - tp.tail_first) * tp.tail_slices;
  const int grid2 = (int)std::max<uint32_t>(1, std::min<uint32_t>(n_work, max_blocks));
  if (plan_.n_vals == 0) {
    part_kernel<0, 0><<<grid1, P1_THREADS, P1_SMEM, stream_>>>(p, tp);
    AB_CUDA(cudaGetLastError());
    agg_kernel<0><<<grid2, P2_NW * 32, P2_SMEM, stream_>>>(p, tp);
  } else {
    part_kernel<1, sig_of(ACC_SUM_I64)><<<grid1, P1_THREADS, P1_SMEM, stream_>>>(p, tp);
    AB_CUDA(cudaGetLastError());
    agg_kernel<1><<<grid2, P2_NW * 32, P2_SMEM, stream_>>>(p, tp);
  }
  ++st_.kernel_launches;
}

void WindowAggOp::launch_segments(const std::vector<Segment>& segs_in, int chunk) {
  while (in_flight_.size() >= 2) absorb(in_flight_.front());
  if (!draining_ && have_counters_ && last_counters_.deferred > 0) {
    while (!in_flight_.empty()) absorb(in_flight_.front());
    drain_deferred();
  }
  const int li = next_launch_;
  next_launch_ = (next_launch_ + 1) % NLAUNCH;
  LaunchRec& L = launches_[li];
  AB_REQUIRE(!L.in_flight, ARROYO_B200_RUNTIME, "launch record still in flight");
  Segment* hs = h_segs_[li].as<Segment>();
  long long tiles = 0;
  uint64_t rows = 0;
  for (size_t i = 0; i < segs_in.size(); ++i) {
    hs[i] = segs_in[i];
    hs[i].tile_start = tiles;
    uintptr_t al = (uintptr_t)hs[i].ts;
    if (plan_.keyed) al |= (uintptr_t)hs[i].key;
    for (int v = 0; v < plan_.n_vals; ++v) al |= (uintptr_t)hs[i].val[v];
    hs[i].vec_ok = (al & 15) == 0;
    tiles += (hs[i].n + TILE - 1) / TILE;
    rows += (uint64_t)hs[i].n;
  }
  AB_CUDA(cudaMemcpyAsync(d_segs_[li].p, hs, segs_in.size() * sizeof(Segment), cudaMemcpyHostToDevice, stream_));
  if (ring_ > RING_INLINE) upload_ring();
  if (!defer_[defer_cur_][0].p) {
    for (int c = 0; c < 2 + plan_.n_vals; ++c) defer_[defer_cur_][c].alloc(defer_cap_ * 8);
  }

  IngestParams p{};
  p.segs = d_segs_[li].as<Segment>();
  p.n_segs = (int)segs_in.size();
  p.keyed = plan_.keyed ? 1 : 0;
  p.n_tiles = tiles;
  p.dict = dict_.view();
  p.slide_div = FastDivU64::make((uint64_t)slide_);
  p.slide = slide_;
  p.late_bin = late_bin_;
  p.late_q = late_bin_ <= 0 ? 0ull : (unsigned long long)late_bin_ / (unsigned long long)slide_;
  p.guard_vals = avg_exact_ ? guard_vals_ : 0u;
  p.combine = (cfg.flags & ARROYO_B200_FLAG_NO_COMBINE) ? 0 : 1;
  p.rows_slot = rows_slot_;
  p.ring_mask = ring_ - 1;
  p.n_acc = plan_.n_acc;
  p.pane_bins = d_pane_bins_.as<long long>();
  p.pane_ptrs = d_pane_ptrs_.as<unsigned long long*>();
  p.id_cap = dict_.id_cap();
  p.ring_inline = ring_ <= RING_INLINE ? 1 : 0;
  if (p.ring_inline)
    for (uint32_t i = 0; i < ring_; ++i) {
      p.ring_bins[i] = h_pane_bins_[i];
      p.ring_ptrs[i] = h_pane_ptrs_[i];
    }
  for (int a = 0; a < plan_.n_acc; ++a) {
    p.acc_kind[a] = plan_.acc_kind[a];
    p.acc_val[a] = plan_.acc_val[a];
  }
  p.counters = d_counters();
  p.slot_rows = d_slot_rows();
  p.d_key = defer_[defer_cur_][0].as<long long>();
  p.d_ts = defer_[defer_cur_][1].as<long long>();
  for (int v = 0; v < plan_.n_vals; ++v) p.d_val[v] = defer_[defer_cur_][2 + v].as<long long>();
  p.defer_cap = defer_cap_;

  int grid = (int)std::min<long long>(tiles, (long long)num_sms_ * 8);
  if (grid < 1) grid = 1;
  if (profile_) AB_CUDA(cudaEventRecord(L.t0, stream_));
  const bool two_pass = two_pass_eligible(rows);
  if (two_pass) {
    long long t2 = 0;
    for (size_t i = 0; i < segs_in.size(); ++i) {
      hs[i].tile_start = t2;
      t2 += (hs[i].n + P1_TILE - 1) / P1_TILE;
    }
    AB_CUDA(cudaMemcpyAsync(d_segs_[li].p, hs, segs_in.size() * sizeof(Segment), cudaMemcpyHostToDevice, stream_));
    p.n_tiles = t2;
    launch_two_pass(p, rows, t2);
  }
  int sig = GENERIC_SIG;
  if (plan_.n_vals <= 1 && plan_.n_acc <= 4) {
    int k[3] = {0, 0, 0};
    for (int a = 1; a < plan_.n_acc; ++a) k[a - 1] = plan_.acc_kind[a];
    sig = sig_of(k[0], k[1], k[2]);
  }
#define AB_LAUNCH(NV, SIG) ingest_kernel<NV, SIG><<<grid, THREADS, 0, stream_>>>(p)
  if (two_pass) {
  } else if (plan_.n_vals == 0) AB_LAUNCH(0, 0);
  else if (plan_.n_vals == 1 && sig == sig_of(ACC_SUM_I64)) AB_LAUNCH(1, sig_of(ACC_SUM_I64));
  else if (plan_.n_vals == 1 && sig == sig_of(ACC_SUM_F64)) AB_LAUNCH(1, sig_of(ACC_SUM_F64));
  else if (plan_.n_vals == 1 && sig == sig_of(ACC_SUM_I64, ACC_SUM_F64)) AB_LAUNCH(1, sig_of(ACC_SUM_I64, ACC_SUM_F64));
  else if (plan_.n_vals == 1 && sig == sig_of(ACC_MIN_I64, ACC_MAX_I64)) AB_LAUNCH(1, sig_of(ACC_MIN_I64, ACC_MAX_I64));
  else if (plan_.n_vals == 1) AB_LAUNCH(1, GENERIC_SIG);
  else if (plan_.n_vals == 2) AB_LAUNCH(2, GENERIC_SIG);
  else if (plan_.n_vals == 3) AB_LAUNCH(3, GENERIC_SIG);
  else AB_LAUNCH(4, GENERIC_SIG);
#undef AB_LAUNCH
  AB_CUDA(cudaGetLastError());
  if (profile_) AB_CUDA(cudaEventRecord(L.t1, stream_));
  ++st_.kernel_launches;
  ++st_.ingest_launches;
  AB_CUDA(cudaMemcpyAsync(L.h_counters, book_.p, BOOK_SLOT_OFF + ring_ * sizeof(unsigned long long), cudaMemcpyDeviceToHost,
                          stream_));
  AB_CUDA(cudaEventRecord(L.done, stream_));
  if (chunk >= 0) AB_CUDA(cudaEventRecord(chunk_free_[chunk], stream_));
  L.rows = rows;
  L.in_flight = true;
  L.chunk = chunk;
  in_flight_.push_back(li);
}

void WindowAggOp::launch_pending() {
  seal_release();
  if (segs_.empty()) return;
  std::vector<Segment> segs;
  segs.swap(segs_);
  pending_rows_ = 0;
  int chunk = pending_uses_chunk_ ? cur_chunk_ : -1;
  pending_uses_chunk_ = false;
  if (chunk >= 0) {
    AB_CUDA(cudaEventRecord(copied_, copy_stream_));
    AB_CUDA(cudaStreamWaitEvent(stream_, copied_, 0));
  }
  launch_segments(segs, chunk);
  if (!zero_copy_inputs_.empty()) {
    PendingRelease r;
    if (!ev_pool_.empty()) {
      r.ev = ev_pool_.back();
      ev_pool_.pop_back();
    } else {
      AB_CUDA(cudaEventCreateWithFlags(&r.ev, cudaEventDisableTiming));
    }
    AB_CUDA(cudaEventRecord(r.ev, stream_));
    r.arrs.swap(zero_copy_inputs_);
    releases_.push_back(std::move(r));
  }
}

void WindowAggOp::touch(int64_t bin) {
  if (sliding_) sliding_planner_->touch(bin);
  else tumbling_->touch(bin);
}

void WindowAggOp::absorb(int li) {
  LaunchRec& L = launches_[li];
  AB_REQUIRE(L.in_flight, ARROYO_B200_RUNTIME, "absorb of an idle launch");
  AB_CUDA(cudaEventSynchronize(L.done));
  L.in_flight = false;
  AB_REQUIRE(!in_flight_.empty() && in_flight_.front() == li, ARROYO_B200_RUNTIME, "launch order violated");
  in_flight_.pop_front();
  if (profile_) {
    float ms = 0;
    AB_CUDA(cudaEventElapsedTime(&ms, L.t0, L.t1));
    st_.ingest_ms += ms;
    st_.ingest_rows_timed += L.rows;
  }
  const Counters& c = *L.h_counters;
  last_counters_ = c;
  have_counters_ = true;
  total_keys_host_ = c.n_keys;
  if (c.part_overflow != part_overflow_seen_) {
    if (c.part_overflow - part_overflow_seen_ > L.rows / 64) two_pass_pause_ = 64;
    part_overflow_seen_ = c.part_overflow;
  }
  if (c.max_q) max_bin_seen_ = std::max<int64_t>(max_bin_seen_, (int64_t)(c.max_q * (uint64_t)slide_));
  for (uint32_t s = 0; s < ring_; ++s) {
    const unsigned long long fresh = L.h_slot_rows[s] - slot_rows_seen_[s];
    slot_rows_seen_[s] = L.h_slot_rows[s];
    if (fresh) {
      AB_REQUIRE(h_pane_bins_[s] != FREE_BIN, ARROYO_B200_RUNTIME, "touched a free ring slot");
      Pane& tp = panes_.at(h_pane_bins_[s]);
      tp.rows += fresh;
      if (tp.rows >= (1ull << 31)) need_promote_ = true;
      touch(h_pane_bins_[s]);
    }
  }
  if (c.lost) throw Error(ARROYO_B200_RUNTIME, "deferred-row buffer overflowed; rows were lost");
  if (c.neg_ts)
    throw Error(ARROYO_B200_PANIC, "batch holds a negative _timestamp (before the Unix epoch): the reference panics on it");
  lookahead();
}

void WindowAggOp::lookahead() {
  if (max_bin_seen_ == LLONG_MIN) return;
  for (int k = 0; k <= 2; ++k) {
    int64_t b = max_bin_seen_ + (int64_t)k * slide_;
    if (b >= late_bin_ && !panes_.count(b)) {
      uint32_t slot = (uint32_t)((uint64_t)b / (uint64_t)slide_) & (ring_ - 1);
      if (h_pane_bins_[slot] == FREE_BIN) ensure_pane(b);
    }
  }
}

void WindowAggOp::sync_all() {
  while (!in_flight_.empty()) absorb(in_flight_.front());
  if (need_promote_ && avg_exact_) promote_avg();
  drain_deferred();
}

void WindowAggOp::drain_deferred() {
  struct Guard {
    bool& f;
    explicit Guard(bool& x) : f(x) { f = true; }
    ~Guard() { f = false; }
  } guard(draining_);
  uint64_t prev = UINT64_MAX;
  for (int stalls = 0; stalls < 64;) {
    if (!have_counters_ || last_counters_.deferred == 0) return;
    AB_REQUIRE(in_flight_.empty(), ARROYO_B200_RUNTIME, "drain with launches in flight");
    const uint64_t n = last_counters_.deferred;
    stalls = n < prev ? 0 : stalls + 1;
    prev = n;
    AB_REQUIRE(n <= defer_cap_, ARROYO_B200_RUNTIME, "deferred overflow");
    st_.rows_deferred += n;
    std::vector<long long> ts(n);
    AB_CUDA(cudaMemcpyAsync(ts.data(), defer_[defer_cur_][1].p, n * 8, cudaMemcpyDeviceToHost, stream_));
    AB_CUDA(cudaStreamSynchronize(stream_));
    std::set<int64_t> bins;
    for (uint64_t i = 0; i < n; ++i) {
      int64_t b = (int64_t)((uint64_t)ts[i] / (uint64_t)slide_ * (uint64_t)slide_);
      if (b >= late_bin_) bins.insert(b);
    }
    for (int64_t b : bins) ensure_pane(b);
    if (last_counters_.big_vals && avg_exact_) promote_avg();
    if (plan_.keyed && (last_counters_.dict_full != dict_full_seen_ ||
                   (uint64_t)last_counters_.n_keys > dict_.n_buckets() * (uint64_t)(BD_MEAN + BD_MEAN / 8))) {
      dict_full_seen_ = last_counters_.dict_full;
      grow_ids();
      last_counters_.n_keys = total_keys_host_;
    }
    const int full = defer_cur_;
    defer_cur_ ^= 1;
    unsigned long long zero = 0;
    AB_CUDA(cudaMemcpyAsync((char*)book_.p + offsetof(Counters, deferred), &zero, sizeof zero,
                            cudaMemcpyHostToDevice, stream_));
    Segment s{};
    s.key = defer_[full][0].as<long long>();
    s.ts = defer_[full][1].as<long long>();
    for (int v = 0; v < plan_.n_vals; ++v) s.val[v] = defer_[full][2 + v].as<long long>();
    s.n = (long long)n;
    launch_segments({s}, -1);
    while (!in_flight_.empty()) absorb(in_flight_.front());
  }
  throw Error(ARROYO_B200_RUNTIME, "deferred rows did not converge");
}

void WindowAggOp::flush() {
  set_device();
  resolve_deferred();
  launch_pending();
  sync_all();
  poll_releases(true);
}

void WindowAggOp::submit() {
  set_device();
  launch_pending();
}

void WindowAggOp::wait_outputs() {
  if (!out_inflight_) return;
  AB_CUDA(cudaEventSynchronize(out_done_));
  out_inflight_ = false;
}

void WindowAggOp::begin_watermark(int64_t wm) {
  set_device();
  if (!out_stream_) {
    AB_CUDA(cudaStreamCreateWithFlags(&out_stream_, cudaStreamNonBlocking));
    AB_CUDA(cudaEventCreateWithFlags(&emit_done_, cudaEventDisableTiming));
    AB_CUDA(cudaEventCreateWithFlags(&out_done_, cudaEventDisableTiming));
  }
  struct Flag {
    bool& f;
    explicit Flag(bool& x) : f(x) { f = true; }
    ~Flag() { f = false; }
  } flag(async_out_);
  handle_watermark(wm, pending_out, nullptr);
  AB_CUDA(cudaEventRecord(out_done_, out_stream_));
  out_inflight_ = true;
}

bool WindowAggOp::poll_watermark(bool block) {
  if (!out_inflight_) return true;
  set_device();
  if (block) {
    wait_outputs();
    return true;
  }
  cudaError_t e = cudaEventQuery(out_done_);
  if (e == cudaErrorNotReady) return false;
  AB_CUDA(e);
  out_inflight_ = false;
  return true;
}

WindowAggOp::OutSet* WindowAggOp::out_set(size_t i, uint64_t cap) {
  while (out_sets_.size() <= i) out_sets_.emplace_back(new OutSet());
  OutSet* os = out_sets_[i].get();
  if (os->cap < cap) {
    uint64_t c = std::max<uint64_t>(std::max<uint64_t>(cap, dict_.id_cap()), 1024);
    os->key.alloc(c * 8);
    os->wstart.alloc(c * 8);
    os->wend.alloc(c * 8);
    os->ts.alloc(c * 8);
    for (int g = 0; g < plan_.n_aggs; ++g) os->agg[g].alloc(c * 8);
    os->cap = c;
    for (int a = 0; a < MAX_ACC; ++a) os->state[a].release();
  }
  return os;
}

int64_t WindowAggOp::run_emit(const std::vector<const unsigned long long*>& blocks, int n_add, bool use_running,
                              bool partial, int64_t wstart, int64_t wend, int64_t ts, OutSet* os) {
  AB_REQUIRE(blocks.size() <= (size_t)INT_MAX, ARROYO_B200_RUNTIME, "too many panes in one window");
  const uint32_t n_ids = dict_.n_ids();
  EmitParams p{};
  p.panes_inline = blocks.size() <= (size_t)EMIT_INLINE ? 1 : 0;
  if (p.panes_inline) {
    for (size_t i = 0; i < blocks.size(); ++i) p.inline_panes[i] = blocks[i];
  } else {
    if (blocks.size() * sizeof(void*) > d_emit_panes_.bytes) {
      AB_CUDA(cudaStreamSynchronize(stream_));
      d_emit_panes_.alloc(std::max(blocks.size(), d_emit_panes_.bytes / sizeof(void*) * 2) * sizeof(void*));
    }
    AB_CUDA(cudaMemcpyAsync(d_emit_panes_.p, blocks.data(), blocks.size() * sizeof(void*), cudaMemcpyHostToDevice, stream_));
  }
  p.panes = d_emit_panes_.as<const unsigned long long*>();
  p.n_panes = (int)blocks.size();
  p.n_acc = plan_.n_acc;
  p.id_cap = dict_.id_cap();
  p.n_ids = n_ids;
  p.keyed = plan_.keyed ? 1 : 0;
  for (int a = 0; a < plan_.n_acc; ++a) p.acc_kind[a] = plan_.acc_kind[a];
  std::vector<std::pair<unsigned long long*, unsigned long long*>> dup_cols;
  for (int a = 0; a < MAX_ACC; ++a) {
    p.out_raw[a] = nullptr;
    p.out_avg[a] = nullptr;
  }
  if (!partial) {
    for (int g = 0; g < plan_.n_aggs; ++g) {
      unsigned long long* col = os->agg[g].as<unsigned long long>();
      const bool avg = plan_.agg_kind[g] == ARROYO_B200_AGG_AVG_I64;
      const int a = plan_.agg_kind[g] == ARROYO_B200_AGG_COUNT_STAR ? 0 : plan_.agg_acc[g];
      unsigned long long*& slot = avg ? p.out_avg[a] : p.out_raw[a];
      if (slot) dup_cols.emplace_back(slot, col);
      else slot = col;
    }
  }
  p.id_keys = dict_.id_keys();
  p.out_key = os->key.as<long long>();
  const bool proj = cfg.final_projection != 0 && !partial;
  p.out_wstart = proj ? os->wstart.as<long long>() : nullptr;
  p.out_wend = proj ? os->wend.as<long long>() : nullptr;
  p.out_ts = os->ts.as<long long>();
  p.wstart = wstart;
  p.wend = wend;
  p.ts = ts;
  p.out_count = d_out_count_.as<unsigned int>();
  const bool deferred = defer_counts_ && count_slots_used_ < COUNT_SLOTS;
  if (defer_counts_) {
    AB_CUDA(cudaMemsetAsync(d_out_count_.p, 0, sizeof(unsigned int), stream_));
    out_count_base_ = 0;
  }
  p.out_base = out_count_base_;
  p.running = use_running ? running_ : nullptr;
  p.n_add = n_add;
  p.partial = partial ? 1 : 0;
  if (partial) {
    for (int a = 0; a < plan_.n_acc; ++a) {
      if (!os->state[a].p) os->state[a].alloc(os->cap * 8);
      p.out_state[a] = os->state[a].as<unsigned long long>();
    }
  }
  const uint32_t n_iter = ((n_ids + 1) / 2 + EMIT_THREADS - 1) / EMIT_THREADS;
  int grid = (int)std::min<uint32_t>(std::max<uint32_t>(n_iter, 1u), (uint32_t)num_sms_ * 8);
  if (profile_) {
    if (emit_events_used_ == emit_events_.size()) {
      cudaEvent_t e0 = nullptr, e1 = nullptr;
      AB_CUDA(cudaEventCreate(&e0));
      AB_CUDA(cudaEventCreate(&e1));
      emit_events_.emplace_back(e0, e1);
    }
    AB_CUDA(cudaEventRecord(emit_events_[emit_events_used_].first, stream_));
  }
#define AB_EMIT(N)                                                               \
  do {                                                                          \
    if (use_running) emit_kernel<true, N><<<grid, EMIT_THREADS, 0, stream_>>>(p); \
    else emit_kernel<false, N><<<grid, EMIT_THREADS, 0, stream_>>>(p);            \
  } while (0)
  switch (plan_.n_acc) {
    case 1: AB_EMIT(1); break;
    case 2: AB_EMIT(2); break;
    case 3: AB_EMIT(3); break;
    case 4: AB_EMIT(4); break;
    case 5: AB_EMIT(5); break;
    case 6: AB_EMIT(6); break;
    case 7: AB_EMIT(7); break;
    case 8: AB_EMIT(8); break;
    default: AB_EMIT(9); break;
  }
  static_assert(MAX_ACC == 9, "emit_kernel instantiations cover 1..MAX_ACC accumulators");
#undef AB_EMIT
  AB_CUDA(cudaGetLastError());
  if (profile_) {
    AB_CUDA(cudaEventRecord(emit_events_[emit_events_used_].second, stream_));
    ++emit_events_used_;
    st_.emit_rows_timed += n_ids;
  }
  ++st_.kernel_launches;
  ++st_.emit_launches;
  if (deferred) {
    const int slot = count_slots_used_++;
    last_count_slot_ = slot;
    AB_CUDA(cudaMemcpyAsync(h_out_counts_.as<unsigned int>() + slot, d_out_count_.p, sizeof(unsigned int),
                            cudaMemcpyDeviceToHost, stream_));
    counts_pending_ = true;
    for (auto& d : dup_cols)
      if (n_ids) AB_CUDA(cudaMemcpyAsync(d.second, d.first, (size_t)n_ids * 8, cudaMemcpyDeviceToDevice, stream_));
    return -(int64_t)(slot + 1);
  }
  AB_CUDA(cudaMemcpyAsync(h_out_count_.p, d_out_count_.p, sizeof(unsigned int), cudaMemcpyDeviceToHost, stream_));
  AB_CUDA(cudaStreamSynchronize(stream_));
  const unsigned int out_now = *h_out_count_.as<unsigned int>();
  const int64_t n_out = (int64_t)(unsigned int)(out_now - out_count_base_);
  out_count_base_ = out_now;
  last_count_slot_ = -1;
  for (auto& d : dup_cols)
    if (n_out) AB_CUDA(cudaMemcpyAsync(d.second, d.first, (size_t)n_out * 8, cudaMemcpyDeviceToDevice, stream_));
  return n_out;
}

void WindowAggOp::export_window(OutSet* os, int64_t n, BatchesPriv* out_host) {
  cudaStream_t cs = stream_;
  if (async_out_) {
    AB_CUDA(cudaEventRecord(emit_done_, stream_));
    AB_CUDA(cudaStreamWaitEvent(out_stream_, emit_done_, 0));
    cs = out_stream_;
  }
  const int wi = std::min<int>(std::max<int>(cfg.window_index, 0), (plan_.keyed ? 1 : 0) + plan_.n_aggs);
  export_window_batch(out_host, n, cs, &st_.d2h_bytes, plan_.keyed ? os->key.p : nullptr, key_format_, os->agg,
                      plan_.agg_format, cfg.final_projection ? os->wstart.p : nullptr, os->wend.p, wi, os->ts.p);
  if (!async_out_) AB_CUDA(cudaStreamSynchronize(stream_));
}

void WindowAggOp::export_partial(OutSet* os, int64_t n, BatchesPriv* out) {
  const std::vector<StateCol> layout = plan_.state_layout(false);
  std::vector<OutColumn> cols = state_columns(layout, n, plan_.keyed ? os->key.p : nullptr, key_format_, os->state,
                                              os->ts.p, stream_, &st_.d2h_bytes);
  AB_CUDA(cudaStreamSynchronize(stream_));
  for (size_t j = 0; j < layout.size(); ++j) {
    if (layout[j].role != S_ACC || plan_.acc_kind[layout[j].acc] != ACC_SUM_I64 || strcmp(layout[j].format, "g")) continue;
    long long* raw = (long long*)cols[(plan_.keyed ? 1 : 0) + j].data;
    double* d = (double*)raw;
    for (int64_t i = 0; i < n; ++i) d[i] = (double)raw[i];
  }
  out->arrays.emplace_back();
  out->schemas.emplace_back();
  export_batch(cols, n, &out->arrays.back(), &out->schemas.back());
}

void WindowAggOp::emit_window(int64_t a, int64_t b, size_t out_index, BatchesPriv* out_host,
                              std::vector<ArroyoB200DeviceBatch>* out_dev) {
  std::vector<int64_t> members;
  for (auto it = panes_.lower_bound(a); it != panes_.end() && it->first < b; ++it)
    if (it->second.in_tier) members.push_back(it->first);
  if (avg_exact_ && guard_vals_) {
    uint64_t window_rows = 0;
    for (int64_t m : members) window_rows += panes_.at(m).rows;
    if (window_rows >= (1ull << 32)) promote_avg();
  }
  std::vector<const unsigned long long*> blocks;
  int n_add = 0;
  bool use_running = false;
  if (running_mode_) {
    if (!running_) {
      running_ = acquire_block();
    }
    std::set<int64_t> target(members.begin(), members.end());
    std::vector<const unsigned long long*> add, sub;
    for (int64_t m : target)
      if (!in_running_.count(m)) {
        const Pane& p = panes_.at(m);
        add.push_back(p.dev);
        if (p.frozen) add.push_back(p.frozen);
      }
    for (int64_t m : in_running_)
      if (!target.count(m)) {
        auto zi = zombies_.find(m);
        const Pane& p = zi != zombies_.end() ? zi->second : panes_.at(m);
        sub.push_back(p.dev);
        if (p.frozen) sub.push_back(p.frozen);
      }
    blocks = add;
    n_add = (int)add.size();
    blocks.insert(blocks.end(), sub.begin(), sub.end());
    in_running_ = target;
    use_running = true;
    if (target.empty()) {
      if (blocks.empty()) return;
    }
  } else {
    for (int64_t m : members) {
      const Pane& p = panes_.at(m);
      blocks.push_back(p.dev);
      if (p.frozen) blocks.push_back(p.frozen);
    }
    if (blocks.empty()) return;
  }
  OutSet* os = out_set(out_dev || async_out_ ? out_index : 0, std::max<uint64_t>(dict_.n_ids(), 1));
  const int64_t ts = cfg.final_projection ? b - 1 : a;
  int64_t n = run_emit(blocks, n_add, use_running, false, a, b, ts, os);
  for (auto& z : zombies_) {
    release_block(z.second.dev);
    release_block(z.second.frozen);
  }
  zombies_.clear();
  if (n == 0) return;
  if (n > 0) {
    st_.rows_out += (uint64_t)n;
    ++st_.windows_out;
  }
  if (out_host) {
    export_window(os, n, out_host);
  } else {
    ArroyoB200DeviceBatch d{};
    d.n_rows = n;
    int c = 0;
    std::vector<uint64_t> cols;
    if (plan_.keyed) cols.push_back((uint64_t)os->key.p);
    for (int g = 0; g < plan_.n_aggs; ++g) cols.push_back((uint64_t)os->agg[g].p);
    if (cfg.final_projection) {
      int wi = std::min<int>(std::max<int>(cfg.window_index, 0), (int)cols.size());
      cols.insert(cols.begin() + wi, (uint64_t)os->wend.p);
      cols.insert(cols.begin() + wi, (uint64_t)os->wstart.p);
    }
    cols.push_back((uint64_t)os->ts.p);
    for (uint64_t v : cols) d.cols[c++] = v;
    d.n_cols = c;
    out_dev->push_back(d);
  }
}

void WindowAggOp::handle_watermark(int64_t wm, BatchesPriv* out_host, std::vector<ArroyoB200DeviceBatch>* out_dev) {
  set_device();
  if (!defer_counts_) resolve_deferred();
  wait_outputs();
  launch_pending();
  sync_all();
  poll_releases(false);
  std::vector<PlanStep> steps;
  if (sliding_) sliding_planner_->watermark(wm, steps);
  else tumbling_->watermark(wm, steps);
  size_t out_index = 0;
  for (const PlanStep& s : steps) {
    switch (s.kind) {
      case PlanStep::JOIN: {
        auto it = panes_.find(s.a);
        AB_REQUIRE(it != panes_.end(), ARROYO_B200_RUNTIME, "closing a pane that is not resident");
        it->second.in_tier = true;
        break;
      }
      case PlanStep::EMIT: {
        if (!sliding_) {
          auto it = panes_.find(s.c);
          AB_REQUIRE(it != panes_.end(), ARROYO_B200_RUNTIME, "emitting a pane that is not resident");
          it->second.in_tier = true;
          emit_window(s.a, s.b, out_index++, out_host, out_dev);
          drop_pane(s.c);
        } else {
          emit_window(s.a, s.b, out_index++, out_host, out_dev);
        }
        break;
      }
      case PlanStep::LEAVE: {
        if (running_mode_ && in_running_.count(s.a)) {
          auto it = panes_.find(s.a);
          Pane z = it->second;
          it->second.dev = nullptr;
          it->second.frozen = nullptr;
          z.slot = -1;
          zombies_[s.a] = z;
        }
        drop_pane(s.a);
        break;
      }
      default:
        break;
    }
  }
  int64_t new_late = bin_start(wm, slide_);
  if (new_late > late_bin_) late_bin_ = new_late;
  std::vector<int64_t> dead;
  const auto& execs = sliding_ ? sliding_planner_->execs() : tumbling_->execs();
  for (auto& kv : panes_)
    if (kv.first < late_bin_ && !kv.second.in_tier && !execs.count(kv.first)) dead.push_back(kv.first);
  for (int64_t b : dead) drop_pane(b);
  for (auto& kv : panes_) {
    if (kv.first >= late_bin_) break;
    Pane& p = kv.second;
    if (p.slot < 0) continue;
    h_pane_bins_[p.slot] = FREE_BIN;
    h_pane_ptrs_[p.slot] = nullptr;
    p.slot = -1;
    ring_dirty_ = true;
  }
  if (wm != INT64_MAX && max_bin_seen_ != LLONG_MIN && late_bin_ >= 0) {
    if (!panes_.count(late_bin_)) {
      uint32_t slot = (uint32_t)((uint64_t)late_bin_ / (uint64_t)slide_) & (ring_ - 1);
      if (h_pane_bins_[slot] == FREE_BIN && late_bin_ <= max_bin_seen_ + 2 * slide_) ensure_pane(late_bin_);
    }
  }
  if (!defer_counts_) collect_emit_times();
}

void WindowAggOp::begin_watermark_device(int64_t wm) {
  set_device();
  resolve_deferred();
  AB_REQUIRE(pending_dev.empty(), ARROYO_B200_INVALID_ARGUMENT,
             "the previous emission has not been collected (handle_watermark_device_poll)");
  if (!counts_done_) AB_CUDA(cudaEventCreateWithFlags(&counts_done_, cudaEventDisableTiming));
  struct Flag {
    bool& f;
    explicit Flag(bool& x) : f(x) { f = true; }
    ~Flag() { f = false; }
  } flag(defer_counts_);
  count_slots_used_ = 0;
  try {
    handle_watermark(wm, nullptr, &pending_dev);
  } catch (...) {
    if (counts_pending_) cudaEventRecord(counts_done_, stream_);
    throw;
  }
  if (counts_pending_) AB_CUDA(cudaEventRecord(counts_done_, stream_));
}

void WindowAggOp::resolve_deferred() {
  if (!counts_pending_) return;
  AB_CUDA(cudaEventSynchronize(counts_done_));
  counts_pending_ = false;
  const unsigned int* h = h_out_counts_.as<unsigned int>();
  std::vector<ArroyoB200DeviceBatch> kept;
  for (ArroyoB200DeviceBatch& d : pending_dev) {
    if (d.n_rows < 0) {
      const int slot = (int)(-d.n_rows - 1);
      d.n_rows = (int64_t)h[slot];
      if (d.n_rows) {
        st_.rows_out += (uint64_t)d.n_rows;
        ++st_.windows_out;
      }
    }
    if (d.n_rows) kept.push_back(d);
  }
  pending_dev.swap(kept);
  if (last_count_slot_ >= 0) out_count_base_ = h[last_count_slot_];
  last_count_slot_ = -1;
  count_slots_used_ = 0;
  collect_emit_times();
}

void WindowAggOp::poll_watermark_device(std::vector<ArroyoB200DeviceBatch>* out) {
  set_device();
  resolve_deferred();
  out->swap(pending_dev);
  pending_dev.clear();
}

void WindowAggOp::collect_emit_times() {
  if (!profile_ || emit_events_used_ == 0) return;
  AB_CUDA(cudaEventSynchronize(emit_events_[emit_events_used_ - 1].second));
  for (size_t i = 0; i < emit_events_used_; ++i) {
    float ms = 0;
    AB_CUDA(cudaEventElapsedTime(&ms, emit_events_[i].first, emit_events_[i].second));
    st_.emit_ms += ms;
  }
  emit_events_used_ = 0;
}

void WindowAggOp::handle_checkpoint(int64_t wm, BatchesPriv* out) {
  set_device();
  resolve_deferred();
  wait_outputs();
  launch_pending();
  sync_all();
  std::vector<PlanStep> steps;
  if (sliding_) sliding_planner_->checkpoint(wm != INT64_MIN, wm, steps);
  else tumbling_->checkpoint(steps);
  for (const PlanStep& s : steps) {
    if (s.kind != PlanStep::CHECKPOINT_PANE) continue;
    auto it = panes_.find(s.a);
    AB_REQUIRE(it != panes_.end(), ARROYO_B200_RUNTIME, "checkpointing a pane that is not resident");
    Pane& p = it->second;
    OutSet* os = out_set(0, std::max<uint64_t>(dict_.n_ids(), 1));
    int64_t n = run_emit({p.dev}, 1, false, true, 0, 0, s.a, os);
    if (n > 0) export_partial(os, n, out);
    p.delta_exported = true;
    if (!p.frozen) p.frozen = acquire_block();
    FoldParams fp{};
    fp.base = p.frozen;
    fp.delta = p.dev;
    fp.cap = dict_.id_cap();
    fp.n = dict_.n_ids();
    fp.n_acc = plan_.n_acc;
    for (int a = 0; a < plan_.n_acc; ++a) fp.acc_kind[a] = plan_.acc_kind[a];
    int grid = (int)std::min<uint32_t>((dict_.n_ids() + 255) / 256, (uint32_t)num_sms_ * 8);
    acc_fold_kernel<<<std::max(grid, 1), 256, 0, stream_>>>(fp);
    AB_CUDA(cudaGetLastError());
    ++st_.kernel_launches;
  }
  for (auto& kv : panes_) {
    Pane& p = kv.second;
    if (!p.in_tier || p.exported) continue;
    std::vector<const unsigned long long*> blocks{p.dev};
    if (p.frozen && !p.delta_exported) blocks.push_back(p.frozen);
    OutSet* os = out_set(0, std::max<uint64_t>(dict_.n_ids(), 1));
    int64_t n = run_emit(blocks, (int)blocks.size(), false, true, 0, 0, kv.first, os);
    if (n > 0) export_partial(os, n, out);
    p.exported = true;
  }
  AB_CUDA(cudaStreamSynchronize(stream_));
  collect_emit_times();
}

void WindowAggOp::on_start(ArrowArray* state, ArrowSchema* schemas, int64_t n, int64_t watermark, int64_t table_min) {
  set_device();
  const StateBatches sb(plan_, false, state, schemas, n);
  const bool has_wm = watermark != INT64_MIN;
  if (has_wm) late_bin_ = std::max<int64_t>(late_bin_, bin_start(watermark, slide_));
  if (sliding_) sliding_planner_->restore_begin(has_wm, watermark);
  for (int64_t bi = 0; bi < n; ++bi) {
    const int64_t rows = sb.rows[bi];
    if (rows == 0) continue;
    const std::vector<InColumn>& cols = sb.cols[bi];
    if (plan_.keyed) key_format_ = cols[0].format;
    const int64_t ts = (int64_t)cols[sb.ts_col].data[0];
    const int64_t bin = bin_start(ts, slide_);
    ensure_pane(bin);
    Pane& p = panes_.at(bin);
    if (!p.frozen) p.frozen = acquire_block();
    bool to_tier = false;
    if (sliding_) to_tier = sliding_planner_->restore_pane(ts);
    else tumbling_->restore(bin);
    if (to_tier) p.in_tier = true;
    p.exported = to_tier;
    p.delta_exported = true;
    PartialParams pp{};
    pp.n = rows;
    pp.n_acc = plan_.n_acc;
    for (int a = 0; a < plan_.n_acc; ++a) pp.acc_kind[a] = plan_.acc_kind[a];
    DevBuf d_key, d_acc[MAX_ACC];
    std::vector<long long> conv[MAX_ACC];
    const long long* keys =
        plan_.keyed ? (const long long*)sb.upload(0, bi, bi + 1, d_key, stream_, &st_.h2d_bytes) : nullptr;
    for (int a = 0; a < plan_.n_acc; ++a) {
      const int c = sb.seed[a];
      if (c < 0) continue;
      if (plan_.acc_kind[a] == ACC_SUM_I64 && !strcmp(sb.layout[c - sb.kc].format, "g")) {
        conv[a].resize((size_t)rows);
        const double* d = (const double*)cols[c].data;
        for (int64_t i = 0; i < rows; ++i) conv[a][(size_t)i] = (long long)__builtin_llround(d[i]);
        d_acc[a].alloc((size_t)rows * 8);
        AB_CUDA(cudaMemcpyAsync(d_acc[a].p, conv[a].data(), (size_t)rows * 8, cudaMemcpyHostToDevice, stream_));
        st_.h2d_bytes += (uint64_t)rows * 8;
        pp.state[a] = d_acc[a].as<unsigned long long>();
      } else {
        pp.state[a] = sb.upload(c, bi, bi + 1, d_acc[a], stream_, &st_.h2d_bytes);
      }
    }
    while (plan_.keyed && (uint64_t)total_keys_host_ + (uint64_t)rows > dict_.n_buckets() * (uint64_t)BD_MEAN) {
      AB_CUDA(cudaStreamSynchronize(stream_));
      grow_ids();
    }
    DevBuf ids((size_t)rows * sizeof(uint32_t));
    dict_.place(keys, rows, ids.as<uint32_t>(), [&] { grow_ids(); });
    pp.ids = ids.as<uint32_t>();
    pp.pane = panes_.at(bin).frozen;
    pp.id_cap = dict_.id_cap();
    int grid = (int)std::min<int64_t>((rows + 255) / 256, (int64_t)num_sms_ * 8);
    ingest_partial_kernel<<<std::max(grid, 1), 256, 0, stream_>>>(pp);
    AB_CUDA(cudaGetLastError());
    ++st_.kernel_launches;
    Counters c{};
    AB_CUDA(cudaMemcpyAsync(&c, book_.p, sizeof c, cudaMemcpyDeviceToHost, stream_));
    AB_CUDA(cudaStreamSynchronize(stream_));
    total_keys_host_ = c.n_keys;
    last_counters_ = c;
    max_bin_seen_ = std::max<int64_t>(max_bin_seen_, bin);
  }
  if (sliding_) sliding_planner_->restore_end(table_min != INT64_MIN, table_min);
  AB_CUDA(cudaStreamSynchronize(stream_));
  take_batches(state, n);
}

void WindowAggOp::stats(ArroyoB200Stats* out) {
  set_device();
  resolve_deferred();
  st_.n_keys = plan_.keyed ? total_keys_host_ : 0;
  st_.rows_late = last_counters_.late_rows;
  *out = st_;
}

}

OpBase* make_window_agg_op(const ArroyoB200OpConfig& cfg) { return new WindowAggOp(cfg); }

}
```

arroyo_b200/ffi.py:

```python
import ctypes as C
import os

from . import build as _build

ABI_VERSION = 1
MAX_AGGS = 8
MAX_COLS = 16

OK, INVALID_ARGUMENT, UNSUPPORTED, RUNTIME, FATAL, PANIC = 0, 1, 2, 3, 4, 5
TUMBLING_AGGREGATE, SLIDING_AGGREGATE, SESSION_AGGREGATE, INSTANT_JOIN, UPDATING_AGGREGATE, TTL_JOIN = 1, 2, 3, 4, 5, 6
INSTANT_AGGREGATE = 7
WINDOW_FUNCTION = 8
FN_ROW_NUMBER, FN_RANK, FN_DENSE_RANK, FN_AGGREGATE = 1, 2, 3, 4
FN_LAG, FN_LEAD, FN_FIRST_VALUE, FN_LAST_VALUE, FN_NTH_VALUE, FN_PERCENT_RANK, FN_CUME_DIST = 5, 6, 7, 8, 9, 10, 11
ORDER_ASC, ORDER_DESC = 16, 17
FN_ARGUMENT = 18
MAX_ORDER_KEYS = 4
AGG_COUNT_STAR, AGG_SUM_I64, AGG_AVG_I64, AGG_MIN_I64, AGG_MAX_I64 = 1, 2, 3, 4, 5
JOIN_INNER, JOIN_LEFT, JOIN_RIGHT, JOIN_FULL = 0, 1, 2, 3
FLAG_PROFILE, FLAG_REMERGE_ONLY, FLAG_COMBINE, FLAG_AVG_F64, FLAG_NO_COMBINE, FLAG_ZERO_COPY = 1, 2, 4, 8, 16, 32
FLAG_NO_DIRECT = 64
FLAG_NO_TWO_PASS = 128
FLAG_TWO_PASS_ALWAYS = 256
FLAG_UPDATING_INPUT = 512
FLAG_FN_DEFAULT = 1024
NO_WATERMARK = -(1 << 63)
INT64_MIN = -(1 << 63)
INT64_MAX = (1 << 63) - 1


class ArrowSchema(C.Structure):
    pass


class ArrowArray(C.Structure):
    pass


ArrowSchema._fields_ = [
    ("format", C.c_char_p), ("name", C.c_char_p), ("metadata", C.c_char_p), ("flags", C.c_int64),
    ("n_children", C.c_int64), ("children", C.POINTER(C.POINTER(ArrowSchema))),
    ("dictionary", C.POINTER(ArrowSchema)), ("release", C.c_void_p), ("private_data", C.c_void_p),
]
ArrowArray._fields_ = [
    ("length", C.c_int64), ("null_count", C.c_int64), ("offset", C.c_int64), ("n_buffers", C.c_int64),
    ("n_children", C.c_int64), ("buffers", C.POINTER(C.c_void_p)),
    ("children", C.POINTER(C.POINTER(ArrowArray))), ("dictionary", C.POINTER(ArrowArray)),
    ("release", C.c_void_p), ("private_data", C.c_void_p),
]


class Agg(C.Structure):
    _fields_ = [("kind", C.c_int32), ("input_col", C.c_int32)]


class OpConfig(C.Structure):
    _fields_ = [
        ("kind", C.c_int32), ("device", C.c_int32), ("stream", C.c_uint64),
        ("task_index", C.c_uint32), ("parallelism", C.c_uint32),
        ("width_ns", C.c_int64), ("slide_ns", C.c_int64), ("gap_ns", C.c_int64),
        ("n_cols", C.c_int32), ("timestamp_col", C.c_int32), ("n_key_cols", C.c_int32), ("key_col", C.c_int32),
        ("n_aggs", C.c_int32), ("aggs", Agg * MAX_AGGS),
        ("final_projection", C.c_int32), ("window_index", C.c_int32),
        ("join_type", C.c_int32), ("right_n_cols", C.c_int32), ("right_timestamp_col", C.c_int32),
        ("left_key_col", C.c_int32), ("right_key_col", C.c_int32),
        ("left_n_routing", C.c_int32), ("right_n_routing", C.c_int32),
        ("partial_count_col_plus1", C.c_int32), ("window_fn", C.c_int32),
        ("expected_keys", C.c_uint64), ("flags", C.c_uint32), ("reserved", C.c_uint32),
    ]


class Batches(C.Structure):
    _fields_ = [("n_batches", C.c_int64), ("arrays", C.POINTER(ArrowArray)), ("schemas", C.POINTER(ArrowSchema)),
                ("private_data", C.c_void_p)]


class DeviceBatch(C.Structure):
    _fields_ = [("n_rows", C.c_int64), ("n_cols", C.c_int32), ("reserved", C.c_int32),
                ("cols", C.c_uint64 * MAX_COLS)]


class Stats(C.Structure):
    _fields_ = [
        ("rows_in", C.c_uint64), ("rows_late", C.c_uint64), ("rows_deferred", C.c_uint64), ("rows_out", C.c_uint64),
        ("windows_out", C.c_uint64), ("n_keys", C.c_uint64), ("kernel_launches", C.c_uint64),
        ("ingest_launches", C.c_uint64), ("emit_launches", C.c_uint64), ("h2d_bytes", C.c_uint64),
        ("d2h_bytes", C.c_uint64), ("ingest_ms", C.c_double), ("emit_ms", C.c_double),
        ("ingest_rows_timed", C.c_uint64), ("emit_rows_timed", C.c_uint64),
        ("host_process_ms", C.c_double), ("host_watermark_ms", C.c_double),
    ]

    def as_dict(self):
        return {f: getattr(self, f) for f, _ in self._fields_}


_VP = C.c_void_p
SYMBOLS = [
    ("arroyo_b200_abi_version", C.c_int32, []),
    ("arroyo_b200_device_count", C.c_int32, []),
    ("arroyo_b200_host_alloc", _VP, [C.c_uint64]),
    ("arroyo_b200_host_free", None, [_VP]),
    ("arroyo_b200_op_create", C.c_int32, [C.POINTER(OpConfig), C.POINTER(_VP), C.c_char_p, C.c_uint64]),
    ("arroyo_b200_op_destroy", None, [_VP]),
    ("arroyo_b200_op_last_error", C.c_char_p, [_VP]),
    ("arroyo_b200_op_name", C.c_char_p, [_VP]),
    ("arroyo_b200_op_on_start", C.c_int32, [_VP, C.POINTER(ArrowArray), C.POINTER(ArrowSchema), C.c_int64,
                                            C.c_int64, C.c_int64]),
    ("arroyo_b200_op_process_batch", C.c_int32, [_VP, C.c_uint32, C.c_uint32, C.POINTER(ArrowArray),
                                                 C.POINTER(ArrowSchema)]),
    ("arroyo_b200_op_process_device_batch", C.c_int32, [_VP, C.c_uint32, C.c_uint32, C.POINTER(C.c_uint64),
                                                        C.c_int32, C.c_int64]),
    ("arroyo_b200_op_process_device_batches", C.c_int32, [_VP, C.c_uint32, C.c_uint32, C.POINTER(C.c_uint64),
                                                          C.c_int32, C.POINTER(C.c_int64), C.c_int64]),
    ("arroyo_b200_op_handle_watermark", C.c_int32, [_VP, C.c_int64, C.POINTER(Batches)]),
    ("arroyo_b200_op_handle_watermark_begin", C.c_int32, [_VP, C.c_int64]),
    ("arroyo_b200_op_handle_watermark_poll", C.c_int32, [_VP, C.c_int32, C.POINTER(Batches), C.POINTER(C.c_int32)]),
    ("arroyo_b200_op_run_batches", C.c_int32, [_VP, C.c_void_p, C.c_void_p, C.c_int64, C.POINTER(C.c_int64), C.c_int32,
                                               C.POINTER(Batches), C.POINTER(C.c_int64)]),
    ("arroyo_b200_op_handle_watermark_device", C.c_int32, [_VP, C.c_int64, C.POINTER(DeviceBatch), C.c_int64,
                                                           C.POINTER(C.c_int64)]),
    ("arroyo_b200_op_handle_watermark_device_begin", C.c_int32, [_VP, C.c_int64]),
    ("arroyo_b200_op_handle_watermark_device_poll", C.c_int32, [_VP, C.POINTER(DeviceBatch), C.c_int64,
                                                                C.POINTER(C.c_int64)]),
    ("arroyo_b200_op_handle_checkpoint", C.c_int32, [_VP, C.c_int64, C.POINTER(Batches)]),
    ("arroyo_b200_op_checkpoint_state", C.c_int32, [_VP, C.POINTER(Batches)]),
    ("arroyo_b200_op_set_clock", C.c_int32, [_VP, C.c_int64]),
    ("arroyo_b200_op_on_close", C.c_int32, [_VP, C.c_int32, C.POINTER(Batches)]),
    ("arroyo_b200_op_handle_tick", C.c_int32, [_VP, C.POINTER(Batches)]),
    ("arroyo_b200_op_process_batch_emit", C.c_int32, [_VP, C.c_uint32, C.c_uint32, C.POINTER(ArrowArray), C.POINTER(ArrowSchema),
                                                      C.POINTER(Batches)]),
    ("arroyo_b200_op_restore_side", C.c_int32, [_VP, C.c_uint32, C.POINTER(ArrowArray), C.POINTER(ArrowSchema),
                                                C.c_int64]),
    ("arroyo_b200_op_flush", C.c_int32, [_VP]),
    ("arroyo_b200_op_submit", C.c_int32, [_VP]),
    ("arroyo_b200_release_batches", None, [C.POINTER(Batches)]),
    ("arroyo_b200_op_stats", C.c_int32, [_VP, C.POINTER(Stats)]),
    ("arroyo_b200_partitioner_create", C.c_int32, [C.c_int32, C.c_uint64, C.c_int32, C.c_int32, C.c_int32,
                                                   C.c_int64, C.POINTER(_VP)]),
    ("arroyo_b200_partitioner_destroy", None, [_VP]),
    ("arroyo_b200_partition", C.c_int32, [_VP, C.POINTER(C.c_uint64), C.c_int64, C.POINTER(C.c_uint64),
                                          C.c_uint64, C.c_uint64]),
    ("arroyo_b200_partition_packed", C.c_int32, [_VP, C.POINTER(C.c_uint64), C.c_int64, C.c_uint64, C.c_uint64,
                                                 C.c_uint64]),
    ("arroyo_b200_ts_minmax", C.c_int32, [C.c_int32, C.c_uint64, C.c_uint64, C.c_int64, C.POINTER(C.c_int64),
                                          C.POINTER(C.c_int64)]),
    ("arroyo_b200_hash_key", C.c_uint64, [C.c_int64]),
    ("arroyo_b200_server_for_hash", C.c_uint32, [C.c_uint64, C.c_uint32]),
    ("arroyo_b200_bin_start", C.c_int64, [C.c_int64, C.c_int64]),
    ("arroyo_b200_plan_sliding", C.c_int64, [C.c_int64, C.c_int64, C.POINTER(C.c_int64), C.c_int64,
                                             C.POINTER(C.c_int64), C.c_int64]),
    ("arroyo_b200_plan_tumbling", C.c_int64, [C.c_int64, C.POINTER(C.c_int64), C.c_int64, C.POINTER(C.c_int64),
                                              C.c_int64]),
]

_lib = None


def lib_path() -> str:
    return _build.LIB


def load():
    global _lib
    if _lib is not None:
        return _lib
    path = lib_path()
    if not os.path.exists(path):
        raise ImportError(
            f"{path} is missing: run `python -c 'import __graft_entry__ as g; g.build()'` "
            "(arroyo_b200 has no CPU fallback)")
    lib = C.CDLL(path)
    for name, res, args in SYMBOLS:
        fn = getattr(lib, name)
        fn.restype = res
        fn.argtypes = args
    v = lib.arroyo_b200_abi_version()
    if v != ABI_VERSION:
        raise ImportError(f"libarroyo_b200 ABI {v} != binding {ABI_VERSION}")
    _lib = lib
    return lib


class ArroyoB200Error(RuntimeError):
    def __init__(self, status: int, message: str):
        super().__init__(f"[status {status}] {message}")
        self.status = status
        self.message = message


class UnsupportedPlan(ArroyoB200Error):
    """The plan is outside the supported subset: fall through to the stock operator."""
```

arroyo_b200/operators.py:

```python
import ctypes as C
import functools
import struct
import time
from typing import List, Optional

import pyarrow as pa

from . import ffi
from .context import Collector, OperatorContext, clamp_watermark

TIMESTAMP = "_timestamp"
_AGG_KINDS = {"count": ffi.AGG_COUNT_STAR, "sum": ffi.AGG_SUM_I64, "avg": ffi.AGG_AVG_I64,
              "min": ffi.AGG_MIN_I64, "max": ffi.AGG_MAX_I64}


def _check(lib, handle, status):
    if status == ffi.OK:
        return
    msg = lib.arroyo_b200_op_last_error(handle)
    msg = msg.decode() if msg else ""
    if status == ffi.UNSUPPORTED:
        raise ffi.UnsupportedPlan(status, msg)
    raise ffi.ArroyoB200Error(status, msg)


def export_batch(batch: pa.RecordBatch):
    arr, sch = ffi.ArrowArray(), ffi.ArrowSchema()
    batch._export_to_c(C.addressof(arr), C.addressof(sch))
    return arr, sch


def _release(s):
    if s.release:
        C.CFUNCTYPE(None, C.c_void_p)(s.release)(C.addressof(s))


def _agg_config(kind: int, c, names: List[str]) -> ffi.OpConfig:
    cfg = ffi.OpConfig()
    cfg.kind = kind
    cfg.n_cols = len(names)
    cfg.timestamp_col = names.index(TIMESTAMP)
    if len(c.key_names) > 1:
        raise ffi.UnsupportedPlan(ffi.UNSUPPORTED, "more than one group-by key column")
    cfg.n_key_cols = len(c.key_names)
    cfg.key_col = names.index(c.key_names[0]) if c.key_names else 0
    cfg.n_aggs = len(c.aggs)
    for i, a in enumerate(c.aggs):
        if a.kind not in _AGG_KINDS:
            raise ffi.UnsupportedPlan(ffi.UNSUPPORTED, f"aggregate {a.kind}")
        cfg.aggs[i].kind = _AGG_KINDS[a.kind]
        cfg.aggs[i].input_col = names.index(a.col) if a.col is not None else 0
    return cfg


class ExportedBatches:

    def __init__(self, batches: List[pa.RecordBatch]):
        self.n = len(batches)
        self.names = list(batches[0].schema.names) if batches else []
        self.arrays = (ffi.ArrowArray * max(self.n, 1))()
        self.schema = ffi.ArrowSchema()
        step = C.sizeof(ffi.ArrowArray)
        base = C.addressof(self.arrays)
        for i, b in enumerate(batches):
            if i == 0:
                b._export_to_c(base, C.addressof(self.schema))
            else:
                b._export_to_c(base + i * step)

    def release_unconsumed(self, first: int):
        for i in range(first, self.n):
            a = self.arrays[i]
            if a.release:
                C.CFUNCTYPE(None, C.c_void_p)(a.release)(C.addressof(a))

    def __del__(self):
        try:
            if self.schema.release:
                C.CFUNCTYPE(None, C.c_void_p)(self.schema.release)(C.addressof(self.schema))
        except Exception:
            pass


def import_batches(lib, out: ffi.Batches) -> List[pa.RecordBatch]:
    res = []
    try:
        for i in range(out.n_batches):
            res.append(pa.RecordBatch._import_from_c(C.addressof(out.arrays[i]), C.addressof(out.schemas[i])))
    finally:
        lib.arroyo_b200_release_batches(C.byref(out))
    return res


class _NativeOperator:

    kind = 0

    def __init__(self, device: int = 0, stream: int = 0, flags: int = 0, expected_keys: int = 0,
                 task_index: int = 0, parallelism: int = 1, chunk_log2: int = 0):
        self._lib = ffi.load()
        self._h = C.c_void_p()
        self._device = device
        self._stream = stream
        self._flags = flags
        self._expected_keys = expected_keys
        self._task_index = task_index
        self._parallelism = parallelism
        self._chunk_log2 = chunk_log2

    def _create(self, cfg: ffi.OpConfig):
        cfg.device = self._device
        cfg.stream = self._stream
        cfg.flags |= self._flags
        cfg.expected_keys = self._expected_keys
        cfg.task_index = self._task_index
        cfg.parallelism = self._parallelism
        cfg.reserved = self._chunk_log2
        err = C.create_string_buffer(1024)
        st = self._lib.arroyo_b200_op_create(C.byref(cfg), C.byref(self._h), err, 1024)
        if st != ffi.OK:
            msg = err.value.decode()
            if st == ffi.UNSUPPORTED:
                raise ffi.UnsupportedPlan(st, msg)
            raise ffi.ArroyoB200Error(st, msg)

    @property
    def created(self) -> bool:
        return bool(self._h)

    def close(self):
        if self._h:
            self._lib.arroyo_b200_op_destroy(self._h)
            self._h = C.c_void_p()

    def __del__(self):
        try:
            self.close()
        except Exception:
            pass

    def flush(self):
        _check(self._lib, self._h, self._lib.arroyo_b200_op_flush(self._h))

    def submit(self):
        if self.created:
            _check(self._lib, self._h, self._lib.arroyo_b200_op_submit(self._h))

    def stats(self) -> dict:
        s = ffi.Stats()
        _check(self._lib, self._h, self._lib.arroyo_b200_op_stats(self._h, C.byref(s)))
        return s.as_dict()

    def _process_batch(self, entry, index: int, parts: int, batch: pa.RecordBatch, out: Optional[ffi.Batches] = None):
        arr, sch = export_batch(batch)
        extra = () if out is None else (C.byref(out),)
        try:
            st = entry(self._h, index, parts, C.byref(arr), C.byref(sch), *extra)
        finally:
            _release(arr)
            _release(sch)
        _check(self._lib, self._h, st)

    def _hand_over_state(self, call, batches: List[pa.RecordBatch]):
        n = len(batches)
        arrs = (ffi.ArrowArray * max(n, 1))()
        schs = (ffi.ArrowSchema * max(n, 1))()
        for i, b in enumerate(batches):
            b._export_to_c(C.addressof(arrs[i]), C.addressof(schs[i]))
        try:
            st = call(arrs, schs, n)
        finally:
            for s in list(arrs) + list(schs):
                _release(s)
        _check(self._lib, self._h, st)

    def _on_start(self, batches: List[pa.RecordBatch], wm: int, t: int):
        self._hand_over_state(lambda a, s, n: self._lib.arroyo_b200_op_on_start(self._h, a, s, n, wm, t), batches)

    def _collect(self, out: ffi.Batches, collector: Optional[Collector]):
        names = self.output_names()
        for b in import_batches(self._lib, out):
            if collector is not None:
                collector.collect(pa.RecordBatch.from_arrays(b.columns, names=names))

    def _device_windows(self, call, max_out: int, drain: bool = True):
        out = getattr(self, "_dev_out", None)
        if out is None or len(out) < max_out:
            out = self._dev_out = (ffi.DeviceBatch * max_out)()
        n = C.c_int64(0)
        got = []
        while True:
            _check(self._lib, self._h, call(out, max_out, C.byref(n)))
            got += [(out[i].n_rows, [out[i].cols[c] for c in range(out[i].n_cols)]) for i in range(n.value)]
            if not drain or n.value != max_out or max_out <= 0:
                return got
            call = functools.partial(self._lib.arroyo_b200_op_handle_watermark_device_poll, self._h)


class _WindowAggregate(_NativeOperator):
    def __init__(self, config, input_schema: Optional[pa.Schema] = None, **kw):
        super().__init__(**kw)
        self.config = config
        self._names: Optional[List[str]] = None
        if input_schema is not None:
            self._build(input_schema.names)

    def _build(self, names: List[str]):
        c = self.config
        if len(c.aggs) > ffi.MAX_AGGS:
            raise ffi.UnsupportedPlan(ffi.UNSUPPORTED, "too many aggregates")
        cfg = _agg_config(self.kind, c, names)
        cfg.width_ns = self._width_ns()
        cfg.slide_ns = int(getattr(c, "slide", 0) or 0)
        pc = getattr(c, "partial_count_col", None)
        cfg.partial_count_col_plus1 = names.index(pc) + 1 if pc else 0
        cfg.final_projection = 1 if c.final_projection else 0
        cfg.window_index = int(c.window_index)
        self._create(cfg)
        self._names = list(names)

    def _width_ns(self) -> int:
        return int(self.config.width)

    def output_names(self) -> List[str]:
        c = self.config
        names = list(c.key_names) + [a.name for a in c.aggs]
        if c.final_projection:
            names.insert(min(max(c.window_index, 0), len(names)), "window")
        return names + [TIMESTAMP]

    def partial_names(self) -> List[str]:
        c = self.config
        names = list(c.key_names)
        for a in c.aggs:
            if a.kind == "avg":
                names += [f"{a.name}[count]", f"{a.name}[sum]"]
            else:
                names.append(f"{a.name}[{a.kind}]")
        return names + [TIMESTAMP]

    def tables(self):
        return {"t": int(self.config.width)}

    def on_start(self, ctx: OperatorContext):
        wm = ctx.last_present_watermark()
        table = ctx.table("t", int(self.config.width))
        batches = [b for _, b in table.all_batches_for_watermark(wm)]
        if not batches and not self.created:
            return
        if not self.created:
            raise ffi.ArroyoB200Error(ffi.INVALID_ARGUMENT, "restore needs input_schema at construction")
        mt = table.get_min_time()
        self._on_start(batches, ffi.INT64_MIN if wm is None else clamp_watermark(wm), ffi.INT64_MIN if mt is None else mt)

    def process_batch(self, batch: pa.RecordBatch, ctx: OperatorContext, collector: Collector):
        if not self.created:
            self._build(batch.schema.names)
        self._process_batch(self._lib.arroyo_b200_op_process_batch, 0, 1, batch)

    def process_device_batch(self, cols: List[int], n_rows: int):
        arr = (C.c_uint64 * len(cols))(*cols)
        st = self._lib.arroyo_b200_op_process_device_batch(self._h, 0, 1, arr, len(cols), n_rows)
        _check(self._lib, self._h, st)

    def process_device_batches(self, cols_flat, n_rows, n_cols: int):
        st = self._lib.arroyo_b200_op_process_device_batches(self._h, 0, 1, cols_flat, n_cols, n_rows, len(n_rows))
        _check(self._lib, self._h, st)

    def handle_watermark(self, watermark, ctx: OperatorContext, collector: Collector):
        wm = ctx.last_present_watermark()
        if wm is None or not self.created:
            return None if self.kind == ffi.SLIDING_AGGREGATE and wm is None else watermark
        out = ffi.Batches()
        _check(self._lib, self._h, self._lib.arroyo_b200_op_handle_watermark(self._h, clamp_watermark(wm), C.byref(out)))
        self._collect(out, collector)
        return watermark

    def handle_watermark_begin(self, watermark, ctx: OperatorContext) -> bool:
        wm = ctx.last_present_watermark()
        if wm is None or not self.created:
            return False
        _check(self._lib, self._h, self._lib.arroyo_b200_op_handle_watermark_begin(self._h, clamp_watermark(wm)))
        return True

    def handle_watermark_poll(self, collector: Collector, block: bool = True) -> bool:
        out = ffi.Batches()
        ready = C.c_int32(0)
        st = self._lib.arroyo_b200_op_handle_watermark_poll(self._h, 1 if block else 0, C.byref(out), C.byref(ready))
        _check(self._lib, self._h, st)
        if not ready.value:
            return False
        self._collect(out, collector)
        return True

    def run_batches(self, exported: "ExportedBatches", watermarks, collector: Collector, first: int = 0,
                    count: Optional[int] = None, async_emit: bool = True):
        if not self.created:
            self._build(exported.names)
        count = exported.n - first if count is None else count
        out, taken = ffi.Batches(), C.c_int64(0)
        step = C.sizeof(ffi.ArrowArray)
        st = self._lib.arroyo_b200_op_run_batches(
            self._h, C.addressof(exported.arrays) + first * step, C.addressof(exported.schema), count,
            C.cast(C.addressof(watermarks) + 8 * first, C.POINTER(C.c_int64)), 1 if async_emit else 0, C.byref(out),
            C.byref(taken))
        self._collect(out, collector)
        _check(self._lib, self._h, st)

    def handle_watermark_device(self, wm: int, max_out: int = 64):
        return self._device_windows(
            functools.partial(self._lib.arroyo_b200_op_handle_watermark_device, self._h, clamp_watermark(wm)), max_out)

    def handle_watermark_device_begin(self, wm: int):
        _check(self._lib, self._h, self._lib.arroyo_b200_op_handle_watermark_device_begin(self._h, clamp_watermark(wm)))

    def handle_watermark_device_poll(self, max_out: int = 64, drain: bool = True):
        return self._device_windows(
            functools.partial(self._lib.arroyo_b200_op_handle_watermark_device_poll, self._h), max_out, drain)

    def handle_checkpoint(self, barrier, ctx: OperatorContext, collector: Collector):
        if not self.created:
            return
        w = ctx.watermark()
        wm = ffi.INT64_MIN if (w is None or w == "idle") else clamp_watermark(w)
        out = ffi.Batches()
        st = self._lib.arroyo_b200_op_handle_checkpoint(self._h, wm, C.byref(out))
        _check(self._lib, self._h, st)
        table = ctx.table("t", int(self.config.width))
        names = self.partial_names()
        for b in import_batches(self._lib, out):
            b = pa.RecordBatch.from_arrays(b.columns, names=names)
            table.insert(int(b.column(len(names) - 1)[0].value), b)

    def on_close(self, final_message, ctx: OperatorContext, collector: Collector):
        if self.created:
            self.flush()


class TumblingAggregatingWindowFunc(_WindowAggregate):
    kind = ffi.TUMBLING_AGGREGATE

    def name(self):
        return "tumbling_window"


class SlidingAggregatingWindowFunc(_WindowAggregate):
    kind = ffi.SLIDING_AGGREGATE

    def name(self):
        return "sliding_window"


class InstantAggregatingWindowFunc(_WindowAggregate):
    kind = ffi.INSTANT_AGGREGATE

    def name(self):
        return "instant_window"

    def _width_ns(self) -> int:
        c = self.config
        if int(c.width) != 0:
            raise ffi.ArroyoB200Error(ffi.INVALID_ARGUMENT, "the instant window has width 0")
        return int(getattr(c, "nested_width", 0)) if c.final_projection else 0


_WINDOW_FNS = {"row_number": ffi.FN_ROW_NUMBER, "rank": ffi.FN_RANK, "dense_rank": ffi.FN_DENSE_RANK}
_WINDOW_AGGS = {"count": ffi.AGG_COUNT_STAR, "sum": ffi.AGG_SUM_I64, "avg": ffi.AGG_AVG_I64, "min": ffi.AGG_MIN_I64,
                "max": ffi.AGG_MAX_I64}
_WINDOW_VALUES = {"lag": ffi.FN_LAG, "lead": ffi.FN_LEAD, "first_value": ffi.FN_FIRST_VALUE,
                  "last_value": ffi.FN_LAST_VALUE, "nth_value": ffi.FN_NTH_VALUE}
_WINDOW_DISTS = {"percent_rank": ffi.FN_PERCENT_RANK, "cume_dist": ffi.FN_CUME_DIST}


def flat_names(schema: pa.Schema) -> List[str]:
    return [name for name, _ in _flat_fields(schema)]


def _flat_fields(schema: pa.Schema):
    fields = []
    for f in schema:
        if pa.types.is_struct(f.type):
            fields += [(f"{f.name}_{c.name}", c.type) for c in f.type]
        else:
            fields.append((f.name, f.type))
    return fields


def _default_bits(value, arrow_type) -> int:
    if arrow_type is not None and pa.types.is_floating(arrow_type):
        return struct.unpack("<q", struct.pack("<d", float(value)))[0]
    return ((int(value) + (1 << 63)) % (1 << 64)) - (1 << 63)


class WindowFunction(_WindowAggregate):
    kind = ffi.WINDOW_FUNCTION

    def __init__(self, config, input_schema: Optional[pa.Schema] = None, **kw):
        _NativeOperator.__init__(self, **kw)
        self.config = config
        self._names: Optional[List[str]] = None
        if input_schema is not None:
            self._build(input_schema.names, input_schema)

    def name(self):
        return "window_function"

    def _build(self, names: List[str], schema: Optional[pa.Schema] = None):
        c = self.config
        agg, value = c.function in _WINDOW_AGGS, c.function in _WINDOW_VALUES
        codes = {**_WINDOW_FNS, **_WINDOW_VALUES, **_WINDOW_DISTS, **{f: ffi.FN_AGGREGATE for f in _WINDOW_AGGS}}
        if c.function not in codes:
            raise ffi.UnsupportedPlan(ffi.UNSUPPORTED, f"window function {c.function}")
        if c.function not in _WINDOW_FNS and c.top_n != 0:
            raise ffi.ArroyoB200Error(ffi.INVALID_ARGUMENT, f"{c.function} takes no top N filter")
        if c.default is not None and c.function not in ("lag", "lead"):
            raise ffi.ArroyoB200Error(ffi.INVALID_ARGUMENT, f"{c.function} takes no default")
        fields = [(n, None) for n in names] if schema is None else _flat_fields(schema)
        flat = [n for n, _ in fields]
        cfg = ffi.OpConfig()
        cfg.kind = self.kind
        cfg.window_fn = codes[c.function]
        cfg.n_cols = len(flat)
        cfg.timestamp_col = flat.index(TIMESTAMP)
        cfg.n_key_cols = 0 if c.partition_by is None else 1
        cfg.key_col = 0 if c.partition_by is None else flat.index(c.partition_by)
        if len(c.order_by) > ffi.MAX_ORDER_KEYS:
            raise ffi.ArroyoB200Error(ffi.INVALID_ARGUMENT, "more than 4 ORDER BY keys")
        first = 0
        if agg:
            cfg.aggs[0].kind = _WINDOW_AGGS[c.function]
            cfg.aggs[0].input_col = 0 if c.function == "count" else flat.index(c.argument)
            first = 1
        if value:
            cfg.aggs[0].kind = ffi.FN_ARGUMENT
            cfg.aggs[0].input_col = flat.index(c.argument)
            first = 1
            if c.function in ("lag", "lead", "nth_value"):
                cfg.width_ns = int(c.offset)
            if c.default is not None:
                cfg.flags |= ffi.FLAG_FN_DEFAULT
                cfg.gap_ns = _default_bits(c.default, fields[cfg.aggs[0].input_col][1])
        cfg.n_aggs = first + len(c.order_by)
        for i, (col, desc) in enumerate(c.order_by):
            cfg.aggs[first + i].kind = ffi.ORDER_DESC if desc else ffi.ORDER_ASC
            cfg.aggs[first + i].input_col = flat.index(col)
        cfg.slide_ns = int(c.top_n)
        self._create(cfg)
        self._names = list(names)
        if schema is not None:
            empty = pa.RecordBatch.from_arrays([pa.array([], f.type) for f in schema], schema=schema)
            self._process_batch(self._lib.arroyo_b200_op_process_batch, 0, 1, empty)

    def _ensure(self, schema: pa.Schema):
        if not self.created:
            self._build(schema.names, schema)

    def output_names(self) -> List[str]:
        return list(self._names) + [self.config.name]

    def state_names(self) -> List[str]:
        return list(self._names)

    def tables(self):
        return {"input": 0}

    def on_start(self, ctx: OperatorContext):
        wm = ctx.last_present_watermark()
        batches = [b for _, b in ctx.table("input", 0).all_batches_for_watermark(wm)]
        if not batches and not self.created:
            return
        if not self.created:
            self._ensure(batches[0].schema)
        self._on_start(batches, ffi.INT64_MIN if wm is None else clamp_watermark(wm), ffi.INT64_MIN)

    def process_batch(self, batch: pa.RecordBatch, ctx: OperatorContext, collector: Collector):
        self._ensure(batch.schema)
        self._process_batch(self._lib.arroyo_b200_op_process_batch, 0, 1, batch)

    def run_batches(self, exported: "ExportedBatches", watermarks, collector: Collector, first: int = 0,
                    count: Optional[int] = None, async_emit: bool = True):
        if not self.created:
            raise ffi.ArroyoB200Error(ffi.INVALID_ARGUMENT, "run_batches needs input_schema at construction")
        super().run_batches(exported, watermarks, collector, first, count, async_emit)

    def handle_checkpoint(self, barrier, ctx: OperatorContext, collector: Collector):
        if not self.created:
            return
        out = ffi.Batches()
        _check(self._lib, self._h, self._lib.arroyo_b200_op_handle_checkpoint(self._h, ffi.INT64_MIN, C.byref(out)))
        table = ctx.table("input", 0)
        names = self.state_names()
        for b in import_batches(self._lib, out):
            b = pa.RecordBatch.from_arrays(b.columns, names=names)
            table.insert(b.column(names.index(TIMESTAMP)).cast(pa.int64())[0].as_py(), b)


class SessionAggregatingWindowFunc(_NativeOperator):
    kind = ffi.SESSION_AGGREGATE

    def __init__(self, config, input_schema: Optional[pa.Schema] = None, **kw):
        super().__init__(**kw)
        self.config = config
        if input_schema is not None:
            self._build(input_schema.names)

    def name(self):
        return "session_window"

    def tables(self):
        return {"s": int(self.config.gap) * 100, "e": 0}

    def _build(self, names: List[str]):
        cfg = _agg_config(self.kind, self.config, names)
        cfg.gap_ns = int(self.config.gap)
        cfg.window_index = int(self.config.window_index)
        self._create(cfg)

    def output_names(self) -> List[str]:
        c = self.config
        names = list(c.key_names)
        names.insert(min(max(c.window_index, 0), len(names)), "window")
        return names + [a.name for a in c.aggs] + [TIMESTAMP]

    def _set_watermark(self, ctx: OperatorContext):
        wm = ctx.last_present_watermark()
        if wm is None or not self.created:
            return
        self._on_start([], clamp_watermark(wm), ffi.INT64_MIN)

    def process_batch(self, batch: pa.RecordBatch, ctx: OperatorContext, collector: Collector):
        if not self.created:
            self._build(batch.schema.names)
            self._set_watermark(ctx)
        wm = ctx.last_present_watermark()
        kept = batch
        if wm is not None:
            import pyarrow.compute as pc
            ts = batch.column(batch.schema.names.index(TIMESTAMP)).cast(pa.int64())
            kept = batch.filter(pc.greater_equal(ts, min(wm, (1 << 63) - 1)))
        if kept.num_rows:
            ts = kept.column(kept.schema.names.index(TIMESTAMP)).cast(pa.int64())
            import pyarrow.compute as pc
            ctx.table("s", int(self.config.gap) * 100).insert(int(pc.max(ts).as_py()), kept)
        self._process_batch(self._lib.arroyo_b200_op_process_batch, 0, 1, batch)

    def process_device_batch(self, cols: List[int], n_rows: int):
        arr = (C.c_uint64 * len(cols))(*cols)
        _check(self._lib, self._h, self._lib.arroyo_b200_op_process_device_batch(self._h, 0, 1, arr, len(cols), n_rows))

    def handle_checkpoint(self, barrier, ctx: OperatorContext, collector: Collector):
        wm = ctx.last_present_watermark()
        ctx.table("s", int(self.config.gap) * 100).flush(wm)
        earliest = None
        if self.created:
            out = ffi.Batches()
            st = self._lib.arroyo_b200_op_handle_checkpoint(self._h, ffi.INT64_MIN if wm is None else clamp_watermark(wm),
                                                            C.byref(out))
            _check(self._lib, self._h, st)
            for b in import_batches(self._lib, out):
                if b.num_rows:
                    earliest = int(b.column(0).cast(pa.int64())[0].as_py())
        ctx.global_table("e")[ctx.task_index] = earliest

    def on_start(self, ctx: OperatorContext):
        starts = [v for v in ctx.global_table("e").values() if v is not None]
        if not starts:
            self._set_watermark(ctx)
            return
        start_time = min(starts)
        table = ctx.table("s", int(self.config.gap) * 100)
        batches = [b for _, b in table.all_batches_for_watermark(start_time)]
        if not self.created:
            if not batches:
                return
            self._build(batches[0].schema.names)
        wm = ctx.last_present_watermark()
        self._on_start(batches, ffi.INT64_MIN if wm is None else clamp_watermark(wm), start_time)

    def handle_watermark(self, watermark, ctx: OperatorContext, collector: Collector):
        wm = ctx.last_present_watermark()
        if wm is None or not self.created:
            return watermark
        out = ffi.Batches()
        _check(self._lib, self._h, self._lib.arroyo_b200_op_handle_watermark(self._h, clamp_watermark(wm), C.byref(out)))
        self._collect(out, collector)
        return watermark

    def handle_watermark_device(self, wm: int, max_out: int = 4):
        return self._device_windows(
            functools.partial(self._lib.arroyo_b200_op_handle_watermark_device, self._h, clamp_watermark(wm)), max_out)


class UpdatingAggregatingFunc(_NativeOperator):
    kind = ffi.UPDATING_AGGREGATE
    IS_RETRACT = "_is_retract"
    DEFAULT_TTL_NS = 24 * 60 * 60 * 1_000_000_000

    def __init__(self, config, input_schema: Optional[pa.Schema] = None, updating_input: bool = False,
                 ttl: Optional[int] = None, clock=None, **kw):
        super().__init__(**kw)
        self.config = config
        self.updating_input = updating_input
        self.ttl = None if ttl is None else (int(ttl) or self.DEFAULT_TTL_NS)
        self.clock = clock or time.monotonic_ns
        self._key_type = None
        if input_schema is not None:
            self._build(input_schema.names)
            self._note_key_type(input_schema)

    def name(self):
        return "UpdatingAggregatingFunc"

    def _note_key_type(self, schema: pa.Schema):
        if self.config.key_names:
            self._key_type = schema.field(self.config.key_names[0]).type

    def tables(self):
        return {"a": 0, "b": 0}

    def state_names(self) -> List[str]:
        names = list(self.config.key_names)
        fields = {"count": ["count"], "sum": ["sum", "count"], "avg": ["count", "sum"], "min": ["min"], "max": ["max"]}
        for a in self.config.aggs:
            names += [f"{a.name}[{f}]" for f in fields[a.kind]]
        return names + [TIMESTAMP, "_generation"]

    def on_start(self, ctx: OperatorContext):
        batches = list(ctx.key_value_table("a").get_all())
        if not batches:
            return
        if not self.created:
            raise ffi.ArroyoB200Error(ffi.INVALID_ARGUMENT, "restore needs input_schema at construction")
        self._tick_clock()
        self._on_start(batches, ffi.INT64_MIN, ffi.INT64_MIN)

    def _build(self, names: List[str]):
        cfg = _agg_config(self.kind, self.config, names)
        cfg.gap_ns = self.ttl or 0
        if self.updating_input:
            self._flags |= ffi.FLAG_UPDATING_INPUT
        self._create(cfg)

    def _tick_clock(self):
        if self.ttl is not None and self.created:
            _check(self._lib, self._h, self._lib.arroyo_b200_op_set_clock(self._h, int(self.clock())))

    def output_names(self) -> List[str]:
        return list(self.config.key_names) + [a.name for a in self.config.aggs] + [TIMESTAMP, self.IS_RETRACT]

    def process_batch(self, batch: pa.RecordBatch, ctx: OperatorContext, collector: Collector):
        if not self.created:
            self._build(batch.schema.names)
        self._note_key_type(batch.schema)
        self._tick_clock()
        self._process_batch(self._lib.arroyo_b200_op_process_batch, 0, 1, batch)

    def process_device_batch(self, cols: List[int], n_rows: int):
        arr = (C.c_uint64 * len(cols))(*cols)
        self._tick_clock()
        _check(self._lib, self._h, self._lib.arroyo_b200_op_process_device_batch(self._h, 0, 1, arr, len(cols), n_rows))

    def process_device_batches(self, cols_flat, n_rows, n_cols: int):
        self._tick_clock()
        st = self._lib.arroyo_b200_op_process_device_batches(self._h, 0, 1, cols_flat, n_cols, n_rows, len(n_rows))
        _check(self._lib, self._h, st)

    def handle_watermark(self, watermark, ctx: OperatorContext, collector: Collector):
        return watermark

    def _typed(self, out, names) -> List[pa.RecordBatch]:
        res = []
        for b in import_batches(self._lib, out):
            cols = b.columns
            if self._key_type is not None and cols[0].type != self._key_type:
                cols = [cols[0].view(self._key_type)] + cols[1:]
            res.append(pa.RecordBatch.from_arrays(cols, names=names))
        return res

    def _emit(self, out, collector: Collector):
        for b in self._typed(out, self.output_names()):
            collector.collect(b)

    def handle_tick(self, tick, ctx: OperatorContext, collector: Collector):
        if not self.created:
            return
        out = ffi.Batches()
        self._tick_clock()
        _check(self._lib, self._h, self._lib.arroyo_b200_op_handle_tick(self._h, C.byref(out)))
        self._emit(out, collector)

    def handle_checkpoint(self, barrier, ctx: OperatorContext, collector: Collector):
        if not self.created:
            return
        out = ffi.Batches()
        self._tick_clock()
        _check(self._lib, self._h, self._lib.arroyo_b200_op_handle_checkpoint(self._h, ffi.INT64_MIN, C.byref(out)))
        self._emit(out, collector)
        if ctx is not None:
            self.checkpoint_state(ctx.key_value_table("a"))

    def checkpoint_state(self, table):
        out = ffi.Batches()
        _check(self._lib, self._h, self._lib.arroyo_b200_op_checkpoint_state(self._h, C.byref(out)))
        for b in self._typed(out, self.state_names()):
            table.insert_batch(b)

    def on_close(self, final_message, ctx: OperatorContext, collector: Collector):
        if not self.created:
            return
        out = ffi.Batches()
        self._tick_clock()
        _check(self._lib, self._h, self._lib.arroyo_b200_op_on_close(self._h, 1 if final_message == "end_of_data" else 0,
                                                                      C.byref(out)))
        self._emit(out, collector)


_JOIN_TYPES = {"inner": ffi.JOIN_INNER, "left": ffi.JOIN_LEFT, "right": ffi.JOIN_RIGHT, "full": ffi.JOIN_FULL}


class InstantJoin(_NativeOperator):
    kind = ffi.INSTANT_JOIN

    def __init__(self, config, left_schema: Optional[pa.Schema] = None, right_schema: Optional[pa.Schema] = None, **kw):
        super().__init__(**kw)
        self.config = config
        self._schemas = [left_schema, right_schema]
        self._buffered = []
        if left_schema is not None and right_schema is not None:
            self._build()

    def name(self):
        return "InstantJoin"

    def tables(self):
        return {"left": 0, "right": 0}

    def _side_layout(self, side: int):
        c = self.config
        names = self._schemas[side].names
        routing = c.left_routing_keys if side == 0 else c.right_routing_keys
        on = c.left_on if side == 0 else c.right_on
        if len(on) != 1:
            raise ffi.UnsupportedPlan(ffi.UNSUPPORTED, "only single-column equi-joins are supported")
        if list(names[:len(routing)]) != list(routing):
            raise ffi.ArroyoB200Error(ffi.INVALID_ARGUMENT, "routing key columns must lead the schema")
        return len(names), names.index(TIMESTAMP), names.index(on[0]), len(routing)

    def _build(self):
        cfg = ffi.OpConfig()
        cfg.kind = self.kind
        cfg.join_type = _JOIN_TYPES[self.config.join_type]
        cfg.n_cols, cfg.timestamp_col, cfg.left_key_col, cfg.left_n_routing = self._side_layout(0)
        cfg.right_n_cols, cfg.right_timestamp_col, cfg.right_key_col, cfg.right_n_routing = self._side_layout(1)
        self._create(cfg)
        for index, parts, batch in self._buffered:
            self._send(index, parts, batch)
        self._buffered = []

    def output_names(self):
        out = []
        for side in (0, 1):
            names = self._schemas[side].names
            routing = self.config.left_routing_keys if side == 0 else self.config.right_routing_keys
            for n in names[len(routing):]:
                if n == TIMESTAMP:
                    continue
                out.append(n if n not in out else n + "_right")
        return out + [TIMESTAMP]

    def _send(self, index, parts, batch):
        self._process_batch(self._lib.arroyo_b200_op_process_batch, index, parts, batch)

    def on_start(self, ctx: OperatorContext):
        wm = ctx.last_present_watermark()
        replay = []
        for side, name in enumerate(("left", "right")):
            replay.append([b for _, b in ctx.table(name, 0).all_batches_for_watermark(wm)])
        if self.created and wm is not None:
            self._on_start([], clamp_watermark(wm), ffi.INT64_MIN)
        for side, batches in enumerate(replay):
            for b in batches:
                self.process_batch_index(side, 2, b, ctx, None)

    def handle_checkpoint(self, barrier, ctx: OperatorContext, collector: Collector):
        wm = ctx.last_present_watermark()
        ctx.table("left", 0).flush(wm)
        ctx.table("right", 0).flush(wm)

    def process_batch_index(self, index: int, in_partitions: int, batch: pa.RecordBatch, ctx: OperatorContext,
                            collector: Collector):
        side = index // (in_partitions // 2)
        if batch.num_rows:
            import pyarrow.compute as pc
            ts = batch.column(batch.schema.names.index(TIMESTAMP)).cast(pa.int64())
            ctx.table("left" if side == 0 else "right", 0).insert(int(pc.max(ts).as_py()), batch)
        if self._schemas[side] is None:
            self._schemas[side] = batch.schema
        if not self.created:
            if self._schemas[0] is not None and self._schemas[1] is not None:
                self._build()
            else:
                self._buffered.append((index, in_partitions, batch))
                return
        self._send(index, in_partitions, batch)

    def handle_watermark(self, watermark, ctx: OperatorContext, collector: Collector):
        wm = ctx.last_present_watermark()
        if wm is None:
            return watermark
        if not self.created:
            if self.config.join_type == "inner":
                self._buffered = []
                return wm
            known = 0 if self._schemas[0] is not None else 1
            self._schemas[1 - known] = pa.schema([("__none", pa.int64()), (TIMESTAMP, pa.timestamp("ns"))])
            saved = (self.config.left_on, self.config.right_on)
            if known == 0:
                self.config.right_on = ["__none"]
            else:
                self.config.left_on = ["__none"]
            try:
                self._build()
            finally:
                self.config.left_on, self.config.right_on = saved
        out = ffi.Batches()
        _check(self._lib, self._h, self._lib.arroyo_b200_op_handle_watermark(self._h, clamp_watermark(wm), C.byref(out)))
        self._collect(out, collector)
        return wm


DAY_NS = 24 * 3600 * 10 ** 9


class JoinWithExpiration(InstantJoin):
    kind = ffi.TTL_JOIN

    def __init__(self, config, left_schema: Optional[pa.Schema] = None, right_schema: Optional[pa.Schema] = None, **kw):
        self._restore_pending = False
        self._restored = [[], []]
        super().__init__(config, left_schema, right_schema, **kw)

    def name(self):
        return "JoinWithExpiration"

    def ttl(self) -> int:
        return int(getattr(self.config, "ttl", 0) or 0) or DAY_NS

    def tables(self):
        return {"left": self.ttl(), "right": self.ttl()}

    def _table(self, ctx: OperatorContext, side: int):
        return ctx.table("left" if side == 0 else "right", self.ttl())

    def on_start(self, ctx: OperatorContext):
        self._restore_pending = True

    def _restore(self, ctx: OperatorContext):
        wm = ctx.last_present_watermark()
        for side in (0, 1):
            batches = [b for _, b in self._table(ctx, side).all_batches_for_watermark(wm)]
            if not batches:
                continue
            if self._schemas[side] is None:
                self._schemas[side] = batches[0].schema
            if self.created:
                self._restore_side(side, batches)
            else:
                self._restored[side] += batches
        if not self.created and self._schemas[0] is not None and self._schemas[1] is not None:
            self._build()

    def _restore_side(self, side: int, batches: List[pa.RecordBatch]):
        if batches:
            self._hand_over_state(
                lambda a, s, n: self._lib.arroyo_b200_op_restore_side(self._h, side, a, s, n), batches)

    def _build(self):
        buffered, self._buffered = self._buffered, []
        super()._build()
        restored, self._restored = self._restored, [[], []]
        for side in (0, 1):
            self._restore_side(side, restored[side])
        for index, parts, batch in buffered:
            self._send(index, parts, batch)

    def handle_checkpoint(self, barrier, ctx: OperatorContext, collector: Collector):
        wm = ctx.last_present_watermark()
        for side in (0, 1):
            self._table(ctx, side).flush(wm)

    def _send(self, index, parts, batch, collector=None):
        out = ffi.Batches()
        self._process_batch(self._lib.arroyo_b200_op_process_batch_emit, index, parts, batch, out)
        self._collect(out, collector)

    def process_batch_index(self, index: int, in_partitions: int, batch: pa.RecordBatch, ctx: OperatorContext,
                            collector: Collector):
        side = index // (in_partitions // 2)
        if self._restore_pending:
            self._restore_pending = False
            self._restore(ctx)
        if self._schemas[side] is None:
            self._schemas[side] = batch.schema
        if self.created or (self._schemas[0] is not None and self._schemas[1] is not None):
            if not self.created:
                self._build()
            self._send(index, in_partitions, batch, collector)
        else:
            self._buffered.append((index, in_partitions, batch))
        if batch.num_rows:
            import pyarrow.compute as pc
            ts = batch.column(batch.schema.names.index(TIMESTAMP)).cast(pa.int64())
            self._table(ctx, side).insert(int(pc.max(ts).as_py()), batch)

    def handle_watermark(self, watermark, ctx: OperatorContext, collector: Collector):
        return watermark
```

include/arroyo_b200.h:

```cpp
#ifndef ARROYO_B200_H
#define ARROYO_B200_H

#include <stdint.h>

#ifdef __cplusplus
extern "C" {
#endif

#ifndef ARROW_C_DATA_INTERFACE
#define ARROW_C_DATA_INTERFACE

#define ARROW_FLAG_DICTIONARY_ORDERED 1
#define ARROW_FLAG_NULLABLE 2
#define ARROW_FLAG_MAP_KEYS_SORTED 4

struct ArrowSchema {
  const char* format;
  const char* name;
  const char* metadata;
  int64_t flags;
  int64_t n_children;
  struct ArrowSchema** children;
  struct ArrowSchema* dictionary;
  void (*release)(struct ArrowSchema*);
  void* private_data;
};

struct ArrowArray {
  int64_t length;
  int64_t null_count;
  int64_t offset;
  int64_t n_buffers;
  int64_t n_children;
  const void** buffers;
  struct ArrowArray** children;
  struct ArrowArray* dictionary;
  void (*release)(struct ArrowArray*);
  void* private_data;
};
#endif

typedef enum ArroyoB200Status {
  ARROYO_B200_OK = 0,
  ARROYO_B200_INVALID_ARGUMENT = 1,
  ARROYO_B200_UNSUPPORTED = 2,
  ARROYO_B200_RUNTIME = 3,
  ARROYO_B200_FATAL = 4,
  ARROYO_B200_PANIC = 5
} ArroyoB200Status;

typedef enum ArroyoB200OpKind {
  ARROYO_B200_TUMBLING_AGGREGATE = 1,
  ARROYO_B200_SLIDING_AGGREGATE = 2,
  ARROYO_B200_SESSION_AGGREGATE = 3,
  ARROYO_B200_INSTANT_JOIN = 4,
  ARROYO_B200_UPDATING_AGGREGATE = 5,
  ARROYO_B200_TTL_JOIN = 6,
  ARROYO_B200_INSTANT_AGGREGATE = 7,
  ARROYO_B200_WINDOW_FUNCTION = 8
} ArroyoB200OpKind;

typedef enum ArroyoB200WindowFn {
  ARROYO_B200_FN_ROW_NUMBER = 1,
  ARROYO_B200_FN_RANK = 2,
  ARROYO_B200_FN_DENSE_RANK = 3,
  ARROYO_B200_FN_AGGREGATE = 4,
  ARROYO_B200_FN_LAG = 5,
  ARROYO_B200_FN_LEAD = 6,
  ARROYO_B200_FN_FIRST_VALUE = 7,
  ARROYO_B200_FN_LAST_VALUE = 8,
  ARROYO_B200_FN_NTH_VALUE = 9,
  ARROYO_B200_FN_PERCENT_RANK = 10,
  ARROYO_B200_FN_CUME_DIST = 11
} ArroyoB200WindowFn;
#define ARROYO_B200_ORDER_ASC 16
#define ARROYO_B200_ORDER_DESC 17
#define ARROYO_B200_FN_ARGUMENT 18
#define ARROYO_B200_MAX_ORDER_KEYS 4

typedef enum ArroyoB200AggKind {
  ARROYO_B200_AGG_COUNT_STAR = 1,
  ARROYO_B200_AGG_SUM_I64 = 2,
  ARROYO_B200_AGG_AVG_I64 = 3,
  ARROYO_B200_AGG_MIN_I64 = 4,
  ARROYO_B200_AGG_MAX_I64 = 5
} ArroyoB200AggKind;

typedef enum ArroyoB200JoinType {
  ARROYO_B200_JOIN_INNER = 0,
  ARROYO_B200_JOIN_LEFT = 1,
  ARROYO_B200_JOIN_RIGHT = 2,
  ARROYO_B200_JOIN_FULL = 3
} ArroyoB200JoinType;

#define ARROYO_B200_MAX_AGGS 8
#define ARROYO_B200_MAX_COLS 16

typedef struct ArroyoB200Agg {
  int32_t kind;
  int32_t input_col;
} ArroyoB200Agg;

typedef struct ArroyoB200OpConfig {
  int32_t kind;
  int32_t device;
  uint64_t stream;
  uint32_t task_index;
  uint32_t parallelism;

  int64_t width_ns;
  int64_t slide_ns;
  int64_t gap_ns;

  int32_t n_cols;
  int32_t timestamp_col;
  int32_t n_key_cols;
  int32_t key_col;
  int32_t n_aggs;
  ArroyoB200Agg aggs[ARROYO_B200_MAX_AGGS];

  int32_t final_projection;
  int32_t window_index;

  int32_t join_type;
  int32_t right_n_cols;
  int32_t right_timestamp_col;
  int32_t left_key_col;
  int32_t right_key_col;
  int32_t left_n_routing;
  int32_t right_n_routing;

  int32_t partial_count_col_plus1;
  int32_t window_fn;

  uint64_t expected_keys;
  uint32_t flags;
  uint32_t reserved;
} ArroyoB200OpConfig;

#define ARROYO_B200_FLAG_PROFILE 1u
#define ARROYO_B200_FLAG_REMERGE_ONLY 2u
#define ARROYO_B200_FLAG_AVG_F64 8u
#define ARROYO_B200_FLAG_COMBINE 4u
#define ARROYO_B200_FLAG_ZERO_COPY 32u
#define ARROYO_B200_FLAG_NO_COMBINE 16u
#define ARROYO_B200_FLAG_NO_DIRECT 64u
#define ARROYO_B200_FLAG_NO_TWO_PASS 128u
#define ARROYO_B200_FLAG_UPDATING_INPUT 512u
#define ARROYO_B200_FLAG_TWO_PASS_ALWAYS 256u
#define ARROYO_B200_FLAG_FN_DEFAULT 1024u

typedef struct ArroyoB200Op ArroyoB200Op;

typedef struct ArroyoB200Batches {
  int64_t n_batches;
  struct ArrowArray* arrays;
  struct ArrowSchema* schemas;
  void* private_data;
} ArroyoB200Batches;

typedef struct ArroyoB200DeviceBatch {
  int64_t n_rows;
  int32_t n_cols;
  int32_t reserved;
  uint64_t cols[ARROYO_B200_MAX_COLS];
} ArroyoB200DeviceBatch;

typedef struct ArroyoB200Stats {
  uint64_t rows_in;
  uint64_t rows_late;
  uint64_t rows_deferred;
  uint64_t rows_out;
  uint64_t windows_out;
  uint64_t n_keys;
  uint64_t kernel_launches;
  uint64_t ingest_launches;
  uint64_t emit_launches;
  uint64_t h2d_bytes;
  uint64_t d2h_bytes;
  double ingest_ms;
  double emit_ms;
  uint64_t ingest_rows_timed;
  uint64_t emit_rows_timed;
  double host_process_ms;
  double host_watermark_ms;
} ArroyoB200Stats;

int32_t arroyo_b200_abi_version(void);
int32_t arroyo_b200_device_count(void);
void* arroyo_b200_host_alloc(uint64_t bytes);
void arroyo_b200_host_free(void* p);


int32_t arroyo_b200_op_create(const ArroyoB200OpConfig* config, ArroyoB200Op** out, char* err,
                              uint64_t err_len);
void arroyo_b200_op_destroy(ArroyoB200Op* op);
const char* arroyo_b200_op_last_error(const ArroyoB200Op* op);
const char* arroyo_b200_op_name(const ArroyoB200Op* op);

int32_t arroyo_b200_op_on_start(ArroyoB200Op* op, struct ArrowArray* state, struct ArrowSchema* schemas,
                                int64_t n, int64_t watermark_ns, int64_t table_min_time_ns);

int32_t arroyo_b200_op_restore_side(ArroyoB200Op* op, uint32_t side, struct ArrowArray* batches,
                                    struct ArrowSchema* schemas, int64_t n);

int32_t arroyo_b200_op_process_batch(ArroyoB200Op* op, uint32_t input_index, uint32_t in_partitions,
                                     struct ArrowArray* batch, const struct ArrowSchema* schema);

int32_t arroyo_b200_op_process_batch_emit(ArroyoB200Op* op, uint32_t input_index, uint32_t in_partitions,
                                          struct ArrowArray* batch, const struct ArrowSchema* schema, ArroyoB200Batches* out);

int32_t arroyo_b200_op_process_device_batch(ArroyoB200Op* op, uint32_t input_index, uint32_t in_partitions,
                                            const uint64_t* cols, int32_t n_cols, int64_t n_rows);

int32_t arroyo_b200_op_process_device_batches(ArroyoB200Op* op, uint32_t input_index, uint32_t in_partitions,
                                              const uint64_t* cols, int32_t n_cols, const int64_t* n_rows,
                                              int64_t n_batches);

int32_t arroyo_b200_op_handle_watermark(ArroyoB200Op* op, int64_t watermark_ns, ArroyoB200Batches* out);

int32_t arroyo_b200_op_handle_tick(ArroyoB200Op* op, ArroyoB200Batches* out);

int32_t arroyo_b200_op_handle_watermark_begin(ArroyoB200Op* op, int64_t watermark_ns);
int32_t arroyo_b200_op_handle_watermark_poll(ArroyoB200Op* op, int32_t block, ArroyoB200Batches* out, int32_t* ready);

int32_t arroyo_b200_op_run_batches(ArroyoB200Op* op, struct ArrowArray* batches, const struct ArrowSchema* schema,
                                    int64_t n_batches, const int64_t* watermarks, int32_t async_emit,
                                    ArroyoB200Batches* out, int64_t* n_consumed);

int32_t arroyo_b200_op_handle_watermark_device(ArroyoB200Op* op, int64_t watermark_ns,
                                               ArroyoB200DeviceBatch* out, int64_t max_out, int64_t* n_out);

int32_t arroyo_b200_op_handle_watermark_device_begin(ArroyoB200Op* op, int64_t watermark_ns);
int32_t arroyo_b200_op_handle_watermark_device_poll(ArroyoB200Op* op, ArroyoB200DeviceBatch* out, int64_t max_out,
                                                    int64_t* n_out);

int32_t arroyo_b200_op_handle_checkpoint(ArroyoB200Op* op, int64_t watermark_ns, ArroyoB200Batches* state_out);

int32_t arroyo_b200_op_checkpoint_state(ArroyoB200Op* op, ArroyoB200Batches* state_out);

int32_t arroyo_b200_op_set_clock(ArroyoB200Op* op, int64_t now_ns);

int32_t arroyo_b200_op_on_close(ArroyoB200Op* op, int32_t end_of_data, ArroyoB200Batches* out);

int32_t arroyo_b200_op_flush(ArroyoB200Op* op);

int32_t arroyo_b200_op_submit(ArroyoB200Op* op);

void arroyo_b200_release_batches(ArroyoB200Batches* batches);

int32_t arroyo_b200_op_stats(ArroyoB200Op* op, ArroyoB200Stats* out);

typedef struct ArroyoB200Partitioner ArroyoB200Partitioner;
int32_t arroyo_b200_partitioner_create(int32_t device, uint64_t stream, int32_t n_dest, int32_t n_cols,
                                       int32_t key_col, int64_t max_rows, ArroyoB200Partitioner** out);
void arroyo_b200_partitioner_destroy(ArroyoB200Partitioner* p);
int32_t arroyo_b200_partition(ArroyoB200Partitioner* p, const uint64_t* in_cols, int64_t n_rows,
                              const uint64_t* out_cols, uint64_t counts_dev, uint64_t offsets_dev);
int32_t arroyo_b200_partition_packed(ArroyoB200Partitioner* p, const uint64_t* in_cols, int64_t n_rows,
                                     uint64_t packed_dev, uint64_t counts_dev, uint64_t offsets_dev);
int32_t arroyo_b200_ts_minmax(int32_t device, uint64_t stream, uint64_t ts_dev, int64_t n_rows, int64_t* out_min,
                               int64_t* out_max);
uint64_t arroyo_b200_hash_key(int64_t key);
uint32_t arroyo_b200_server_for_hash(uint64_t h, uint32_t n);

int64_t arroyo_b200_plan_sliding(int64_t width_ns, int64_t slide_ns, const int64_t* events, int64_t n_events,
                                 int64_t* out, int64_t out_cap);
int64_t arroyo_b200_plan_tumbling(int64_t width_ns, const int64_t* events, int64_t n_events, int64_t* out,
                                  int64_t out_cap);

int64_t arroyo_b200_bin_start(int64_t ts_ns, int64_t width_ns);

#ifdef __cplusplus
}
#endif
#endif
```

Measured before the change: 24.98 billion.

## Speculatively emit watermarks before last ingest launch completes, with device-gated rollback

The device watermark path no longer waits for the last in-flight ingest launch. It snapshots planner and pane state, launches a tiny check kernel that validates slot row counts and counters on the device, and plans and emits windows with the emit kernels gated on that check's flag. If the host later sees the check fail, it restores the snapshot and replans synchronously. Bookkeeping copies (counters, output counts) also move to a separate stream so they do not serialize the main stream. This removes a host sync per watermark at the cost of extra state copies, a small kernel, and rare redo work.

```diff
diff --git a/arroyo_b200/csrc/abi.cu b/arroyo_b200/csrc/abi.cu
--- a/arroyo_b200/csrc/abi.cu
+++ b/arroyo_b200/csrc/abi.cu
@@ -347,6 +347,13 @@
   });
 }
 
+int32_t arroyo_b200_op_watermark_counts(ArroyoB200Op* op, uint64_t* early, uint64_t* redone) {
+  return guarded(op, [&](OpBase* o) {
+    AB_REQUIRE(early != nullptr && redone != nullptr, ARROYO_B200_INVALID_ARGUMENT, "null out");
+    o->watermark_counts(early, redone);
+  });
+}
+
 int32_t arroyo_b200_op_handle_checkpoint(ArroyoB200Op* op, int64_t watermark_ns, ArroyoB200Batches* state_out) {
   return emit_batches(op, state_out, [&](OpBase* o, BatchesPriv* b) { o->handle_checkpoint(watermark_ns, b); });
 }
diff --git a/arroyo_b200/csrc/op.h b/arroyo_b200/csrc/op.h
--- a/arroyo_b200/csrc/op.h
+++ b/arroyo_b200/csrc/op.h
@@ -51,6 +51,10 @@
     pending_dev.clear();
   }
   virtual void stats(ArroyoB200Stats* out) = 0;
+  virtual void watermark_counts(uint64_t* early, uint64_t* redone) {
+    *early = 0;
+    *redone = 0;
+  }
 
  protected:
   int device_ = 0;
diff --git a/arroyo_b200/csrc/window_agg.cu b/arroyo_b200/csrc/window_agg.cu
--- a/arroyo_b200/csrc/window_agg.cu
+++ b/arroyo_b200/csrc/window_agg.cu
@@ -496,7 +496,30 @@
   int n_add;
   int partial;
   unsigned long long* out_state[MAX_ACC];
+  const unsigned int* spec_ok;
 };
+
+constexpr int SPEC_SLOTS = 64;
+struct SpecCheckParams {
+  const Counters* counters;
+  const unsigned long long* slot_rows;
+  unsigned int* ok;
+  unsigned int* out_count;
+  int n;
+  uint32_t slot[SPEC_SLOTS];
+  unsigned long long seen[SPEC_SLOTS];
+};
+
+__global__ void spec_check_kernel(const __grid_constant__ SpecCheckParams p) {
+  const int lane = threadIdx.x;
+  bool ok = true;
+  for (int i = lane; i < p.n; i += 32) ok = ok && p.slot_rows[p.slot[i]] == p.seen[i];
+  ok = __all_sync(0xffffffffu, ok);
+  if (lane == 0) {
+    *p.ok = ok && p.counters->deferred == 0 && p.counters->lost == 0 && p.counters->neg_ts == 0 ? 1u : 0u;
+    *p.out_count = 0;
+  }
+}
 
 constexpr int EMIT_THREADS = 256;
 
@@ -539,6 +562,7 @@
   __shared__ unsigned int s_base;
   const int tid = threadIdx.x;
   const int lane = tid & 31, w = tid >> 5;
+  if (p.spec_ok && *p.spec_ok == 0) return;
   const uint32_t n_pairs = (p.n_ids + 1) / 2;
   const uint32_t n_iter = (n_pairs + EMIT_THREADS - 1) / EMIT_THREADS;
   for (uint32_t it = blockIdx.x; it < n_iter; it += gridDim.x) {
@@ -637,6 +661,7 @@
 };
 
 struct LaunchRec {
+  cudaEvent_t end = nullptr;
   cudaEvent_t done = nullptr;
   cudaEvent_t t0 = nullptr, t1 = nullptr;
   Counters* h_counters = nullptr;
@@ -670,6 +695,7 @@
   void begin_watermark_device(int64_t wm) override;
   void poll_watermark_device(std::vector<ArroyoB200DeviceBatch>* out) override;
   void stats(ArroyoB200Stats* out) override;
+  void watermark_counts(uint64_t* early, uint64_t* redone) override;
 
  private:
   bool sliding_;
@@ -739,6 +765,16 @@
   DevBuf chunk_[NCHUNK];
   cudaEvent_t chunk_free_[NCHUNK] = {nullptr, nullptr, nullptr};
   cudaStream_t copy_stream_ = nullptr;
+  cudaStream_t book_stream_ = nullptr;
+  cudaEvent_t spec_ev_ = nullptr;
+  bool count_zeroed_ = false;
+  cudaEvent_t emit_ev_ = nullptr, count_copied_ = nullptr;
+  bool count_copy_pending_ = false;
+  void wait_count_copy() {
+    if (!count_copy_pending_) return;
+    AB_CUDA(cudaStreamWaitEvent(stream_, count_copied_, 0));
+    count_copy_pending_ = false;
+  }
   cudaEvent_t copied_ = nullptr;
   int cur_chunk_ = 0;
   int64_t cur_rows_ = 0;
@@ -781,9 +817,42 @@
   cudaEvent_t counts_done_ = nullptr;
   void resolve_deferred();
 
+  struct EarlyWatermark {
+    bool active = false;
+    int li = -1;
+    int64_t wm = 0;
+    std::vector<uint32_t> slots;
+    std::vector<unsigned long long> seen;
+    std::vector<unsigned long long*> releases;
+    std::unique_ptr<SlidingPlanner> sliding;
+    std::unique_ptr<TumblingPlanner> tumbling;
+    std::map<int64_t, Pane> panes, zombies;
+    std::set<int64_t> in_running;
+    int64_t late_bin = 0;
+    uint32_t ring = 0;
+    std::vector<long long> ring_bins;
+    std::vector<unsigned long long*> ring_ptrs;
+    bool ring_dirty = false;
+    std::vector<std::pair<unsigned long long*, uint64_t>> free_panes;
+    unsigned long long* running = nullptr;
+    size_t emit_events_used = 0;
+    uint64_t emit_rows_timed = 0;
+  };
+  EarlyWatermark early_;
+  bool hold_releases_ = false;
+  const unsigned int* spec_gate_ = nullptr;
+  DevBuf spec_ok_;
+  PinnedBuf h_spec_ok_;
+  cudaEvent_t spec_done_ = nullptr;
+  uint64_t watermarks_early_ = 0, watermarks_redone_ = 0;
+  bool begin_early(int64_t wm);
+  void resolve_early();
+  void plan_watermark(int64_t wm, BatchesPriv* out_host, std::vector<ArroyoB200DeviceBatch>* out_dev);
+
   ArroyoB200Stats st_{};
   std::vector<std::pair<cudaEvent_t, cudaEvent_t>> emit_events_;
   size_t emit_events_used_ = 0;
+  size_t emit_sets_ = 0;
 
   void preallocate();
   template <class Fill>
@@ -896,6 +965,7 @@
     launches_[i].h_counters = h_book_[i].as<Counters>();
     launches_[i].h_slot_rows = reinterpret_cast<unsigned long long*>((char*)h_book_[i].p + BOOK_SLOT_OFF);
     AB_CUDA(cudaEventCreateWithFlags(&launches_[i].done, cudaEventDisableTiming));
+    AB_CUDA(cudaEventCreateWithFlags(&launches_[i].end, cudaEventDisableTiming));
     if (profile_) {
       AB_CUDA(cudaEventCreate(&launches_[i].t0));
       AB_CUDA(cudaEventCreate(&launches_[i].t1));
@@ -909,6 +979,13 @@
   AB_CUDA(cudaMemsetAsync(d_out_count_.p, 0, sizeof(unsigned int), stream_));
   h_out_count_.alloc(sizeof(unsigned int));
   h_out_counts_.alloc(COUNT_SLOTS * sizeof(unsigned int));
+  spec_ok_.alloc(sizeof(unsigned int));
+  h_spec_ok_.alloc(sizeof(unsigned int));
+  AB_CUDA(cudaEventCreateWithFlags(&spec_done_, cudaEventDisableTiming));
+  AB_CUDA(cudaEventCreateWithFlags(&spec_ev_, cudaEventDisableTiming));
+  AB_CUDA(cudaEventCreateWithFlags(&emit_ev_, cudaEventDisableTiming));
+  AB_CUDA(cudaEventCreateWithFlags(&count_copied_, cudaEventDisableTiming));
+  AB_CUDA(cudaStreamCreateWithFlags(&book_stream_, cudaStreamNonBlocking));
   preallocate();
   AB_CUDA(cudaStreamSynchronize(stream_));
 }
@@ -932,6 +1009,11 @@
 WindowAggOp::~WindowAggOp() {
   cudaSetDevice(device_);
   if (counts_done_) cudaEventDestroy(counts_done_);
+  if (book_stream_) cudaStreamSynchronize(book_stream_);
+  if (spec_done_) cudaEventDestroy(spec_done_);
+  if (spec_ev_) cudaEventDestroy(spec_ev_);
+  if (emit_ev_) cudaEventDestroy(emit_ev_);
+  if (count_copied_) cudaEventDestroy(count_copied_);
   if (copy_stream_) cudaStreamSynchronize(copy_stream_);
   if (out_stream_) cudaStreamSynchronize(out_stream_);
   cudaStreamSynchronize(stream_);
@@ -954,6 +1036,7 @@
   }
   for (int i = 0; i < NLAUNCH; ++i) {
     if (launches_[i].done) cudaEventDestroy(launches_[i].done);
+    if (launches_[i].end) cudaEventDestroy(launches_[i].end);
     if (launches_[i].t0) cudaEventDestroy(launches_[i].t0);
     if (launches_[i].t1) cudaEventDestroy(launches_[i].t1);
   }
@@ -961,6 +1044,7 @@
     cudaEventDestroy(e.first);
     cudaEventDestroy(e.second);
   }
+  if (book_stream_) cudaStreamDestroy(book_stream_);
   if (out_stream_) {
     cudaStreamSynchronize(out_stream_);
     cudaStreamDestroy(out_stream_);
@@ -998,6 +1082,10 @@
 
 void WindowAggOp::release_block(unsigned long long* blk) {
   if (!blk) return;
+  if (hold_releases_) {
+    early_.releases.push_back(blk);
+    return;
+  }
   free_panes_.emplace_back(blk, std::min<uint64_t>(dict_.id_cap(), (uint64_t)dict_.n_ids() + 1));
 }
 
@@ -1277,6 +1365,7 @@
 
 void WindowAggOp::process_batch(uint32_t, uint32_t, ArrowArray* batch, const ArrowSchema* schema) {
   set_device();
+  resolve_early();
   int64_t n = 0;
   std::vector<InColumn> cols = import_batch(batch, schema, &n);
   AB_REQUIRE((int)cols.size() == cfg.n_cols, ARROYO_B200_INVALID_ARGUMENT, "batch has the wrong number of columns");
@@ -1486,6 +1575,15 @@
     tiles += (hs[i].n + TILE - 1) / TILE;
     rows += (uint64_t)hs[i].n;
   }
+  const bool two_pass = two_pass_eligible(rows);
+  long long t2 = 0;
+  if (two_pass) {
+    for (size_t i = 0; i < segs_in.size(); ++i) {
+      hs[i].tile_start = t2;
+      t2 += (hs[i].n + P1_TILE - 1) / P1_TILE;
+    }
+  }
+  if (!in_flight_.empty()) AB_CUDA(cudaStreamWaitEvent(stream_, launches_[in_flight_.back()].done, 0));
   AB_CUDA(cudaMemcpyAsync(d_segs_[li].p, hs, segs_in.size() * sizeof(Segment), cudaMemcpyHostToDevice, stream_));
   if (ring_ > RING_INLINE) upload_ring();
   if (!defer_[defer_cur_][0].p) {
@@ -1530,14 +1628,7 @@
   int grid = (int)std::min<long long>(tiles, (long long)num_sms_ * 8);
   if (grid < 1) grid = 1;
   if (profile_) AB_CUDA(cudaEventRecord(L.t0, stream_));
-  const bool two_pass = two_pass_eligible(rows);
   if (two_pass) {
-    long long t2 = 0;
-    for (size_t i = 0; i < segs_in.size(); ++i) {
-      hs[i].tile_start = t2;
-      t2 += (hs[i].n + P1_TILE - 1) / P1_TILE;
-    }
-    AB_CUDA(cudaMemcpyAsync(d_segs_[li].p, hs, segs_in.size() * sizeof(Segment), cudaMemcpyHostToDevice, stream_));
     p.n_tiles = t2;
     launch_two_pass(p, rows, t2);
   }
@@ -1563,9 +1654,11 @@
   if (profile_) AB_CUDA(cudaEventRecord(L.t1, stream_));
   ++st_.kernel_launches;
   ++st_.ingest_launches;
+  AB_CUDA(cudaEventRecord(L.end, stream_));
+  AB_CUDA(cudaStreamWaitEvent(book_stream_, L.end, 0));
   AB_CUDA(cudaMemcpyAsync(L.h_counters, book_.p, BOOK_SLOT_OFF + ring_ * sizeof(unsigned long long), cudaMemcpyDeviceToHost,
-                          stream_));
-  AB_CUDA(cudaEventRecord(L.done, stream_));
+                          book_stream_));
+  AB_CUDA(cudaEventRecord(L.done, book_stream_));
   if (chunk >= 0) AB_CUDA(cudaEventRecord(chunk_free_[chunk], stream_));
   L.rows = rows;
   L.in_flight = true;
@@ -1574,6 +1667,7 @@
 }
 
 void WindowAggOp::launch_pending() {
+  resolve_early();
   seal_release();
   if (segs_.empty()) return;
   std::vector<Segment> segs;
@@ -1710,6 +1804,7 @@
 
 void WindowAggOp::flush() {
   set_device();
+  resolve_early();
   resolve_deferred();
   launch_pending();
   sync_all();
@@ -1718,6 +1813,7 @@
 
 void WindowAggOp::submit() {
   set_device();
+  resolve_early();
   launch_pending();
 }
 
@@ -1745,8 +1841,9 @@
 }
 
 bool WindowAggOp::poll_watermark(bool block) {
+  set_device();
+  resolve_early();
   if (!out_inflight_) return true;
-  set_device();
   if (block) {
     wait_outputs();
     return true;
@@ -1822,14 +1919,17 @@
   p.ts = ts;
   p.out_count = d_out_count_.as<unsigned int>();
   const bool deferred = defer_counts_ && count_slots_used_ < COUNT_SLOTS;
+  wait_count_copy();
   if (defer_counts_) {
-    AB_CUDA(cudaMemsetAsync(d_out_count_.p, 0, sizeof(unsigned int), stream_));
+    if (!count_zeroed_) AB_CUDA(cudaMemsetAsync(d_out_count_.p, 0, sizeof(unsigned int), stream_));
+    count_zeroed_ = false;
     out_count_base_ = 0;
   }
   p.out_base = out_count_base_;
   p.running = use_running ? running_ : nullptr;
   p.n_add = n_add;
   p.partial = partial ? 1 : 0;
+  p.spec_ok = spec_gate_;
   if (partial) {
     for (int a = 0; a < plan_.n_acc; ++a) {
       if (!os->state[a].p) os->state[a].alloc(os->cap * 8);
@@ -1876,11 +1976,15 @@
   if (deferred) {
     const int slot = count_slots_used_++;
     last_count_slot_ = slot;
-    AB_CUDA(cudaMemcpyAsync(h_out_counts_.as<unsigned int>() + slot, d_out_count_.p, sizeof(unsigned int),
-                            cudaMemcpyDeviceToHost, stream_));
-    counts_pending_ = true;
     for (auto& d : dup_cols)
       if (n_ids) AB_CUDA(cudaMemcpyAsync(d.second, d.first, (size_t)n_ids * 8, cudaMemcpyDeviceToDevice, stream_));
+    AB_CUDA(cudaEventRecord(emit_ev_, stream_));
+    AB_CUDA(cudaStreamWaitEvent(book_stream_, emit_ev_, 0));
+    AB_CUDA(cudaMemcpyAsync(h_out_counts_.as<unsigned int>() + slot, d_out_count_.p, sizeof(unsigned int),
+                            cudaMemcpyDeviceToHost, book_stream_));
+    AB_CUDA(cudaEventRecord(count_copied_, book_stream_));
+    count_copy_pending_ = true;
+    counts_pending_ = true;
     return -(int64_t)(slot + 1);
   }
   AB_CUDA(cudaMemcpyAsync(h_out_count_.p, d_out_count_.p, sizeof(unsigned int), cudaMemcpyDeviceToHost, stream_));
@@ -2007,15 +2111,21 @@
 
 void WindowAggOp::handle_watermark(int64_t wm, BatchesPriv* out_host, std::vector<ArroyoB200DeviceBatch>* out_dev) {
   set_device();
+  resolve_early();
   if (!defer_counts_) resolve_deferred();
   wait_outputs();
   launch_pending();
   sync_all();
   poll_releases(false);
+  plan_watermark(wm, out_host, out_dev);
+}
+
+void WindowAggOp::plan_watermark(int64_t wm, BatchesPriv* out_host, std::vector<ArroyoB200DeviceBatch>* out_dev) {
   std::vector<PlanStep> steps;
   if (sliding_) sliding_planner_->watermark(wm, steps);
   else tumbling_->watermark(wm, steps);
   size_t out_index = 0;
+  emit_sets_ = 0;
   for (const PlanStep& s : steps) {
     switch (s.kind) {
       case PlanStep::JOIN: {
@@ -2030,9 +2140,11 @@
           AB_REQUIRE(it != panes_.end(), ARROYO_B200_RUNTIME, "emitting a pane that is not resident");
           it->second.in_tier = true;
           emit_window(s.a, s.b, out_index++, out_host, out_dev);
+          emit_sets_ = out_index;
           drop_pane(s.c);
         } else {
           emit_window(s.a, s.b, out_index++, out_host, out_dev);
+          emit_sets_ = out_index;
         }
         break;
       }
@@ -2090,12 +2202,173 @@
   } flag(defer_counts_);
   count_slots_used_ = 0;
   try {
-    handle_watermark(wm, nullptr, &pending_dev);
+    if (!begin_early(wm)) handle_watermark(wm, nullptr, &pending_dev);
   } catch (...) {
-    if (counts_pending_) cudaEventRecord(counts_done_, stream_);
+    if (counts_pending_) cudaEventRecord(counts_done_, book_stream_);
     throw;
   }
-  if (counts_pending_) AB_CUDA(cudaEventRecord(counts_done_, stream_));
+  if (counts_pending_) AB_CUDA(cudaEventRecord(counts_done_, book_stream_));
+}
+
+bool WindowAggOp::begin_early(int64_t wm) {
+  if ((cfg.flags & ARROYO_B200_FLAG_SYNC_WATERMARK) || wm == INT64_MAX || rows_slot_ >= 0) return false;
+  wait_outputs();
+  launch_pending();
+  while (in_flight_.size() > 1) absorb(in_flight_.front());
+  if (in_flight_.size() != 1) return false;
+  if (!have_counters_ || last_counters_.deferred != 0 || (need_promote_ && avg_exact_)) return false;
+  const int li = in_flight_.front();
+  const LaunchRec& L = launches_[li];
+  const int64_t wbin = bin_start(wm, slide_);
+  if (sliding_) {
+    if (sliding_planner_->state() != SlidingPlanner::IN_MEMORY) return false;
+    SlidingPlanner dry(*sliding_planner_);
+    std::vector<PlanStep> steps;
+    while (dry.should_advance(wm)) {
+      dry.advance(steps);
+      if (dry.state() != SlidingPlanner::IN_MEMORY) return false;
+    }
+  }
+  if (avg_exact_) {
+    uint64_t total = L.rows;
+    for (const auto& kv : panes_) {
+      if (kv.second.rows + L.rows >= (1ull << 31)) return false;
+      total += kv.second.rows;
+    }
+    if (guard_vals_ && total >= (1ull << 32)) return false;
+  }
+  EarlyWatermark& e = early_;
+  e.slots.clear();
+  e.seen.clear();
+  for (uint32_t s = 0; s < ring_; ++s) {
+    if (h_pane_bins_[s] == FREE_BIN || h_pane_bins_[s] >= wbin) continue;
+    if (e.slots.size() == (size_t)SPEC_SLOTS) return false;
+    e.slots.push_back(s);
+    e.seen.push_back(slot_rows_seen_[s]);
+  }
+
+  if (sliding_) e.sliding.reset(new SlidingPlanner(*sliding_planner_));
+  else e.tumbling.reset(new TumblingPlanner(*tumbling_));
+  e.panes = panes_;
+  e.zombies = zombies_;
+  e.in_running = in_running_;
+  e.late_bin = late_bin_;
+  e.ring = ring_;
+  e.ring_bins.assign(h_pane_bins_.begin(), h_pane_bins_.begin() + ring_);
+  e.ring_ptrs.assign(h_pane_ptrs_.begin(), h_pane_ptrs_.begin() + ring_);
+  e.ring_dirty = ring_dirty_;
+  e.free_panes = free_panes_;
+  e.running = running_;
+  e.emit_events_used = emit_events_used_;
+  e.emit_rows_timed = st_.emit_rows_timed;
+  e.releases.clear();
+  e.li = li;
+  e.wm = wm;
+
+  SpecCheckParams sp{};
+  sp.counters = d_counters();
+  sp.slot_rows = d_slot_rows();
+  sp.ok = spec_ok_.as<unsigned int>();
+  sp.n = (int)e.slots.size();
+  for (size_t i = 0; i < e.slots.size(); ++i) {
+    sp.slot[i] = e.slots[i];
+    sp.seen[i] = e.seen[i];
+  }
+  sp.out_count = d_out_count_.as<unsigned int>();
+  wait_count_copy();
+  spec_check_kernel<<<1, 32, 0, stream_>>>(sp);
+  AB_CUDA(cudaGetLastError());
+  ++st_.kernel_launches;
+  count_zeroed_ = true;
+  AB_CUDA(cudaEventRecord(spec_ev_, stream_));
+  AB_CUDA(cudaStreamWaitEvent(book_stream_, spec_ev_, 0));
+  AB_CUDA(cudaMemcpyAsync(h_spec_ok_.p, spec_ok_.p, sizeof(unsigned int), cudaMemcpyDeviceToHost, book_stream_));
+  AB_CUDA(cudaEventRecord(spec_done_, book_stream_));
+
+  e.active = true;
+  ++watermarks_early_;
+  struct Hold {
+    WindowAggOp* o;
+    ~Hold() {
+      o->hold_releases_ = false;
+      o->spec_gate_ = nullptr;
+      o->count_zeroed_ = false;
+    }
+  } hold{this};
+  hold_releases_ = true;
+  spec_gate_ = spec_ok_.as<unsigned int>();
+  plan_watermark(wm, nullptr, &pending_dev);
+  return true;
+}
+
+void WindowAggOp::resolve_early() {
+  if (!early_.active) return;
+  EarlyWatermark& e = early_;
+  e.active = false;
+  AB_CUDA(cudaEventSynchronize(spec_done_));
+  const LaunchRec& L = launches_[e.li];
+  const Counters& c = *L.h_counters;
+  bool ok = c.deferred == 0 && c.lost == 0 && c.neg_ts == 0;
+  for (size_t i = 0; i < e.slots.size(); ++i) ok = ok && L.h_slot_rows[e.slots[i]] == e.seen[i];
+  AB_REQUIRE(ok == (*h_spec_ok_.as<unsigned int>() != 0), ARROYO_B200_RUNTIME,
+             "early watermark: the device's check and the host's disagree");
+  std::vector<unsigned long long*> held;
+  held.swap(e.releases);
+  if (ok) {
+    for (unsigned long long* b : held) release_block(b);
+    absorb(e.li);
+    e.sliding.reset();
+    e.tumbling.reset();
+    e.panes.clear();
+    e.zombies.clear();
+    return;
+  }
+  ++watermarks_redone_;
+  if (sliding_) *sliding_planner_ = *e.sliding;
+  else *tumbling_ = *e.tumbling;
+  panes_.swap(e.panes);
+  zombies_.swap(e.zombies);
+  in_running_.swap(e.in_running);
+  late_bin_ = e.late_bin;
+  AB_REQUIRE(ring_ == e.ring, ARROYO_B200_RUNTIME, "early watermark: the ring grew");
+  std::copy(e.ring_bins.begin(), e.ring_bins.end(), h_pane_bins_.begin());
+  std::copy(e.ring_ptrs.begin(), e.ring_ptrs.end(), h_pane_ptrs_.begin());
+  ring_dirty_ = true;
+  free_panes_.swap(e.free_panes);
+  running_ = e.running;
+  emit_events_used_ = e.emit_events_used;
+  st_.emit_rows_timed = e.emit_rows_timed;
+  e.sliding.reset();
+  e.tumbling.reset();
+  e.panes.clear();
+  e.zombies.clear();
+  pending_dev.clear();
+  counts_pending_ = false;
+  count_slots_used_ = 0;
+  last_count_slot_ = -1;
+  struct Flag {
+    bool& f;
+    const bool was;
+    explicit Flag(bool& x) : f(x), was(x) { f = true; }
+    ~Flag() { f = was; }
+  } flag(defer_counts_);
+  try {
+    wait_outputs();
+    sync_all();
+    poll_releases(false);
+    plan_watermark(e.wm, nullptr, &pending_dev);
+  } catch (...) {
+    if (counts_pending_) cudaEventRecord(counts_done_, book_stream_);
+    throw;
+  }
+  if (counts_pending_) AB_CUDA(cudaEventRecord(counts_done_, book_stream_));
+}
+
+void WindowAggOp::watermark_counts(uint64_t* early, uint64_t* redone) {
+  set_device();
+  resolve_early();
+  *early = watermarks_early_;
+  *redone = watermarks_redone_;
 }
 
 void WindowAggOp::resolve_deferred() {
@@ -2124,6 +2397,7 @@
 
 void WindowAggOp::poll_watermark_device(std::vector<ArroyoB200DeviceBatch>* out) {
   set_device();
+  resolve_early();
   resolve_deferred();
   out->swap(pending_dev);
   pending_dev.clear();
@@ -2142,6 +2416,7 @@
 
 void WindowAggOp::handle_checkpoint(int64_t wm, BatchesPriv* out) {
   set_device();
+  resolve_early();
   resolve_deferred();
   wait_outputs();
   launch_pending();
@@ -2149,12 +2424,13 @@
   std::vector<PlanStep> steps;
   if (sliding_) sliding_planner_->checkpoint(wm != INT64_MIN, wm, steps);
   else tumbling_->checkpoint(steps);
+  const size_t ck_set = pending_dev.empty() ? 0 : emit_sets_;
   for (const PlanStep& s : steps) {
     if (s.kind != PlanStep::CHECKPOINT_PANE) continue;
     auto it = panes_.find(s.a);
     AB_REQUIRE(it != panes_.end(), ARROYO_B200_RUNTIME, "checkpointing a pane that is not resident");
     Pane& p = it->second;
-    OutSet* os = out_set(0, std::max<uint64_t>(dict_.n_ids(), 1));
+    OutSet* os = out_set(ck_set, std::max<uint64_t>(dict_.n_ids(), 1));
     int64_t n = run_emit({p.dev}, 1, false, true, 0, 0, s.a, os);
     if (n > 0) export_partial(os, n, out);
     p.delta_exported = true;
@@ -2176,7 +2452,7 @@
     if (!p.in_tier || p.exported) continue;
     std::vector<const unsigned long long*> blocks{p.dev};
     if (p.frozen && !p.delta_exported) blocks.push_back(p.frozen);
-    OutSet* os = out_set(0, std::max<uint64_t>(dict_.n_ids(), 1));
+    OutSet* os = out_set(ck_set, std::max<uint64_t>(dict_.n_ids(), 1));
     int64_t n = run_emit(blocks, (int)blocks.size(), false, true, 0, 0, kv.first, os);
     if (n > 0) export_partial(os, n, out);
     p.exported = true;
@@ -2187,6 +2463,7 @@
 
 void WindowAggOp::on_start(ArrowArray* state, ArrowSchema* schemas, int64_t n, int64_t watermark, int64_t table_min) {
   set_device();
+  resolve_early();
   const StateBatches sb(plan_, false, state, schemas, n);
   const bool has_wm = watermark != INT64_MIN;
   if (has_wm) late_bin_ = std::max<int64_t>(late_bin_, bin_start(watermark, slide_));
@@ -2257,6 +2534,7 @@
 
 void WindowAggOp::stats(ArroyoB200Stats* out) {
   set_device();
+  resolve_early();
   resolve_deferred();
   st_.n_keys = plan_.keyed ? total_keys_host_ : 0;
   st_.rows_late = last_counters_.late_rows;
diff --git a/arroyo_b200/ffi.py b/arroyo_b200/ffi.py
--- a/arroyo_b200/ffi.py
+++ b/arroyo_b200/ffi.py
@@ -24,6 +24,7 @@
 FLAG_TWO_PASS_ALWAYS = 256
 FLAG_UPDATING_INPUT = 512
 FLAG_FN_DEFAULT = 1024
+FLAG_SYNC_WATERMARK = 2048
 NO_WATERMARK = -(1 << 63)
 INT64_MIN = -(1 << 63)
 INT64_MAX = (1 << 63) - 1
@@ -122,6 +123,7 @@
     ("arroyo_b200_op_handle_watermark_device_begin", C.c_int32, [_VP, C.c_int64]),
     ("arroyo_b200_op_handle_watermark_device_poll", C.c_int32, [_VP, C.POINTER(DeviceBatch), C.c_int64,
                                                                 C.POINTER(C.c_int64)]),
+    ("arroyo_b200_op_watermark_counts", C.c_int32, [_VP, C.POINTER(C.c_uint64), C.POINTER(C.c_uint64)]),
     ("arroyo_b200_op_handle_checkpoint", C.c_int32, [_VP, C.c_int64, C.POINTER(Batches)]),
     ("arroyo_b200_op_checkpoint_state", C.c_int32, [_VP, C.POINTER(Batches)]),
     ("arroyo_b200_op_set_clock", C.c_int32, [_VP, C.c_int64]),
diff --git a/arroyo_b200/operators.py b/arroyo_b200/operators.py
--- a/arroyo_b200/operators.py
+++ b/arroyo_b200/operators.py
@@ -150,6 +150,11 @@
         s = ffi.Stats()
         _check(self._lib, self._h, self._lib.arroyo_b200_op_stats(self._h, C.byref(s)))
         return s.as_dict()
+
+    def watermark_counts(self) -> dict:
+        early, redone = C.c_uint64(0), C.c_uint64(0)
+        _check(self._lib, self._h, self._lib.arroyo_b200_op_watermark_counts(self._h, C.byref(early), C.byref(redone)))
+        return {"early": early.value, "redone": redone.value}
 
     def _process_batch(self, entry, index: int, parts: int, batch: pa.RecordBatch, out: Optional[ffi.Batches] = None):
         arr, sch = export_batch(batch)
diff --git a/include/arroyo_b200.h b/include/arroyo_b200.h
--- a/include/arroyo_b200.h
+++ b/include/arroyo_b200.h
@@ -149,6 +149,7 @@
 #define ARROYO_B200_FLAG_UPDATING_INPUT 512u
 #define ARROYO_B200_FLAG_TWO_PASS_ALWAYS 256u
 #define ARROYO_B200_FLAG_FN_DEFAULT 1024u
+#define ARROYO_B200_FLAG_SYNC_WATERMARK 2048u
 
 typedef struct ArroyoB200Op ArroyoB200Op;
 
@@ -235,6 +236,8 @@
 int32_t arroyo_b200_op_handle_watermark_device_poll(ArroyoB200Op* op, ArroyoB200DeviceBatch* out, int64_t max_out,
                                                     int64_t* n_out);
 
+int32_t arroyo_b200_op_watermark_counts(ArroyoB200Op* op, uint64_t* early, uint64_t* redone);
+
 int32_t arroyo_b200_op_handle_checkpoint(ArroyoB200Op* op, int64_t watermark_ns, ArroyoB200Batches* state_out);
 
 int32_t arroyo_b200_op_checkpoint_state(ArroyoB200Op* op, ArroyoB200Batches* state_out);
```

Result: faster. 27.32 billion (median of 6 runs) (+9.4%).
